# jsourati/nn-active-learning

Measured on AMD Instinct MI355X. Metric: patches/sec Fisher-scored (32^3, 2-class), higher is better.
Workload: dtype f32 (fp32 operands split into 16-bit pieces on the 16-bit MFMA, fp32 accumulate: fp16 pairs - 22-23 bits kept per operand, three products - in the conv under the head (forward + backward), in dec1's forward launch and in the other backward launches; bf16 triples - all 24 bits, exact, six products -

## Files before the change

include/alq.h:

```cpp
#ifndef ALQ_H
#define ALQ_H

#include <stddef.h>
#include <stdint.h>

#ifdef __cplusplus
extern "C" {
#endif

typedef struct alq_ctx alq_ctx;
typedef struct alq_model alq_model;

enum { ALQ_OK = 0, ALQ_EINVAL = -1, ALQ_EHIP = -2, ALQ_ENOMEM = -3, ALQ_EUNSUPPORTED = -4 };

enum { ALQ_CONV = 0, ALQ_CONVT = 1, ALQ_POOL = 2, ALQ_FC = 3 };

typedef struct {
    int32_t type;
    int32_t cout;
    int32_t k[3];
    int32_t s[3];
    int32_t relu;
    int32_t skip_src;
} alq_layer_t;
// ... 164 lines not shown
int alq_segment_min(alq_ctx *ctx, const int32_t *d_labels, const int64_t dims[3], int32_t n_labels, const int64_t *d_inds,
                    const double *d_scores, int64_t n, double *d_table);

size_t alq_cc_work_bytes(const int64_t dims[3]);
int alq_cc_label(alq_ctx *ctx, const uint8_t *d_seg, const int64_t dims[3], int connectivity, int select_zero, int32_t *d_labels);
int alq_cc_keep_largest(alq_ctx *ctx, const uint8_t *d_seg, const int64_t dims[3], int connectivity, int skip_origin, uint8_t *d_out,
                        int64_t *d_info, void *d_work);
int alq_fill_holes(alq_ctx *ctx, const uint8_t *d_seg, const int64_t dims[3], uint8_t *d_out, int64_t *d_info, void *d_work);

typedef struct alq_dcrf_params {
    float sdims_smooth[2];
    float sdims_app[2];
    float schan;
    float compat_smooth, compat_app;
    int32_t niter;
} alq_dcrf_params;
size_t alq_dcrf_work_bytes(const int64_t dims[3]);
int alq_dcrf2d(alq_ctx *ctx, const float *d_post, const float *d_img, const int64_t dims[3], const alq_dcrf_params *par,
               float *d_q1, uint8_t *d_map, void *d_work);

int alq_llfc_grads(alq_ctx *ctx, const float *d_feat, const float *d_post, const int32_t *d_labels, int n, int d, int c,
                   float *d_out);
size_t alq_llfc_hess_max_bytes(void);
int alq_llfc_hess(alq_ctx *ctx, const float *d_feat_one, const float *d_post_one, int d, int c, double *d_H);
int alq_llfc_if_path(int d, int c);
size_t alq_llfc_if_work_bytes(int n_pool, int c);
int alq_llfc_stoch_if(alq_ctx *ctx, const float *d_pool_feat, const float *d_pool_post, const int32_t *d_pool_labels, int n_pool,
                      const float *d_tr_feat, const float *d_tr_post, int n_tr, const int32_t *d_draws, int T, double scale, int d,
                      int c, int path, float *d_V, void *d_work);

int alq_aopt_tile(void);
int alq_aopt_max_workgroups(void);
size_t alq_aopt_work_bytes(int64_t n, int L);
int alq_aopt_svec(alq_ctx *ctx, const double *d_A, int64_t n, int L, double *d_V);
int alq_aopt_stats(alq_ctx *ctx, const double *d_V, const double *d_q, int64_t n, int m, const double *h_kvec,
                   const double *h_R, double mu, double obj, double *d_out, void *d_work);
int alq_aopt_direction(alq_ctx *ctx, const double *d_V, const double *d_q, int64_t n, int m, const double *h_kvec,
                       const double *h_R, const double *h_c_r, const double *h_c_1, double ratio, double mu, double obj,
                       double *d_dq, double *d_out, void *d_work);
int alq_aopt_linesearch(alq_ctx *ctx, const double *d_q, const double *d_dq, int64_t n, const double *h_alpha, int J,
                        double *d_out, void *d_work);
int alq_aopt_update(alq_ctx *ctx, double *d_q, const double *d_dq, const double *d_V, int64_t n, int m, double alpha,
                    double *d_out, void *d_work);

typedef struct {
    int32_t layer;
    int32_t pad;
    int64_t idx;
    double delta;
} alq_flip_t;
int alq_ref64_scores(alq_ctx *ctx, const alq_layer_t *layers, int n_layers, const int32_t in_dims[4],
                     const double *const *h_dW, const double *const *h_db, const float *d_x, const int64_t *d_rows, int N,
                     const alq_flip_t *d_flips, int flips_per_sample, double eps, int cand_cap,
                     double *d_logits, double *d_S, double *d_rms, alq_flip_t *d_cand, double *d_cand_key, int32_t *d_cand_count);

int alq_prof_enable(alq_ctx *ctx, int on);
int alq_prof_reset(alq_ctx *ctx);
int alq_prof_num_classes(void);
const char *alq_prof_class_name(int cls);
int alq_prof_read(alq_ctx *ctx, int cls, double *ms, int64_t *launches, double *flops);

int alq_model_debug_copy(alq_model *m, int layer_idx, int what, int N, float *d_out,
                         int64_t *elems_out);

int alq_debug_set_stamp_buffer(void *d_buf);
int alq_debug_set(int key, int value);
enum {
    ALQ_INFO_SUBNORMALS_OK = 0,
    ALQ_INFO_C3D_FWD = 1,
    ALQ_INFO_C3D_BWD = 2,
    ALQ_INFO_C3D_ONE_ACC = 3,
    ALQ_INFO_FLIP_OVERFLOW = 5,
    ALQ_INFO_F16_DERIVED = 6,
    ALQ_INFO_T3D_FWD = 7,
    ALQ_INFO_T3D_BWD = 8,
    ALQ_INFO_E3D_BWD = 9,
    ALQ_INFO_D3D_FWD = 10,
    ALQ_INFO_D3D_BWD = 11,
    ALQ_INFO_F3D_FWD = 12,
    ALQ_INFO_C3D_BWD_FORM = 13,
    ALQ_INFO_HOST_PACK_ELEMS = 14,
    ALQ_INFO_LSUM = 15,
    ALQ_INFO_DCP_FORM = 16,
    ALQ_INFO_E3D_BWD_FORM = 17
};
int alq_model_engine_info(alq_model *m, int what);

int alq_synth_patches(alq_ctx *ctx, uint64_t seed, int64_t first_id, int64_t n,
                      int64_t elems_per_patch, float *d_out);

#ifdef __cplusplus
}
#endif
#endif
```

nn-active-learning_amd/csrc/alq_internal.h:

```cpp
#pragma once
#include <hip/hip_runtime.h>

#include <cstdint>
#include <cstdio>
#include <memory>
#include <string>
#include <vector>

#include "alq.h"
#include "engine_switches.h"

namespace alq {

void set_error(const char *fmt, ...);

#define ALQ_HIP(expr)                                                                     \
    do {                                                                                  \
        hipError_t e_ = (expr);                                                           \
        if (e_ != hipSuccess) {                                                           \
            ::alq::set_error("%s:%d: %s -> %s", __FILE__, __LINE__, #expr,               \
                             hipGetErrorString(e_));                                      \
            return ALQ_EHIP;                                                              \
        }                                                                                 \
    } while (0)
// ... 142 lines not shown
int igemm_launch(alq_ctx *ctx, const IgemmPlan &plan, const View &in, const View &out,
                 const float *bias, int relu, int accumulate, int N, int prof_cls);

struct Igemm2Args {
    const float *in;
    float *out;
    const float *W;
    const float *bias;
    const float *mask;
    float *osumA, *osumB;
    int mask_cs, mask_c0, mask_from, split;
    int in_cs, in_c0, Ci, ID, IH, IW;
    int out_cs, out_c0, Co, OD, OH, OW;
    int MD, MH, MW;
    int sm, so, ooffz, ooffy, ooffx;
    int PT, TZ, TY, TX, HZ, HY, HX, rows;
    int minz, miny, minx;
    int ntaps, nchunks;
    int tilesZ, tilesY, tilesX;
    int N, relu, accumulate;
    int t0, tsz, tsy, tsx, tnx, tny;
    int dbg_repeat, dbg_flags;
    unsigned long long *dbg;
    const int *tdesc;
    const int *sdesc;
    int tpg;
    int in_bytes;
    int in_pstride, out_pstride;
    float f16_sc = 0.f, f16_inv = 0.f, f16_bias_sc = 0.f;
    const unsigned *f16_bound = nullptr;
    int f16_wexp = 0;
};

struct Igemm2Plan {
    Igemm2Args a;
    bool ok = false;
    bool wres = false;
    int NTW = 1;
    int wgs_per_cu = 1;
    size_t lds_bytes = 0;
    double flops_per_patch = 0;
    std::vector<float> h_W;
    float *d_W = nullptr;
    std::vector<int> h_tdesc, h_sdesc;
    int *d_tdesc = nullptr, *d_sdesc = nullptr;
};

struct Igemm2Fuse {
    const float *mask = nullptr;
    int mask_cs = 0, mask_c0 = 0, mask_from = 0;
    int mask_to = 1 << 30;
    float *osumA = nullptr, *osumB = nullptr;
    int split = 0;
    int store_from = 0;
    int mask_split = 0;
    long long mask_delta = 0;
    const unsigned char *mask_bits = nullptr;
    unsigned char *sign_out = nullptr;
    const unsigned *in_bits = nullptr;
    const float *in_vec = nullptr;
    float in_vec_amax = 0.f;
    const unsigned *in_vec16 = nullptr;
    unsigned *out_amax = nullptr;
    int amax_from = 0;
    const unsigned *in_amax = nullptr, *in_amax2 = nullptr;
    float in_bound = 0.f;
    const float *fc_W = nullptr;
    long long fc_F = 0;
    float *fc_part = nullptr;
    unsigned *fc_bits = nullptr;
    unsigned *flip_cnt = nullptr, *flip_list = nullptr;
    int flip_cap = 0;
    float flip_l1 = 0.f;
    bool flip_bias_nonzero = false;
};

extern unsigned long long *g_igemm2_dbg;
extern int g_dbg_knobs[ALQ_NKNOBS];
inline bool two_slot_allowed() { return !g_dbg_knobs[KNOB_NO_V3] && !g_dbg_knobs[KNOB_NO_V4]; }
extern int g_dcp_last_form;
extern int g_no_f16x2;
extern int g_no_fixed;
extern int g_no_xcd_order;
int igemm2_build_plan(const IgemmPlan &p1, Igemm2Plan *p2);
void igemm2_pack_weights(Igemm2Plan *p2, const std::vector<float> &Bmat);
int igemm2_launch(alq_ctx *ctx, const Igemm2Plan &plan, const View &in, const View &out, const float *bias,
                  int relu, int accumulate, int N, int prof_cls, const Igemm2Fuse *fuse);

struct Igemm3Plan {
    bool ok = false;
    bool wres = false;
    int NTW = 1;
    int wgs_per_cu = 1;
    size_t lds_bytes = 0;
    std::vector<unsigned short> h_W;
    void *d_W = nullptr;
    std::vector<unsigned short> h_W16;
    void *d_W16 = nullptr;
    int w16_exp = 0;
};
int igemm3_build_plan(const Igemm2Plan &p2, Igemm3Plan *p3);
void igemm3_pack_weights(const Igemm2Plan &p2, Igemm3Plan *p3, const std::vector<float> &Bmat);
void igemm3_pack_weights_f16(const Igemm2Plan &p2, Igemm3Plan *p3, const std::vector<float> &Bmat);
int igemm3_launch(alq_ctx *ctx, const Igemm2Plan &p2, const Igemm3Plan &plan, const View &in, const View &out,
                  const float *bias, int relu, int accumulate, int N, int prof_cls, const Igemm2Fuse *fuse);

struct Igemm4Args {
    const float *in;
    float *out;
    const void *W;
    const float *bias;
    const float *mask;
    float *osumA, *osumB;
    const int *tdesc;
    const int *sdesc;
    const int *pdesc;
    const int *ttab;
    const int *vdesc;
    int in_cs, in_c0, out_cs, out_c0, Co;
    int mask_cs, mask_c0, mask_from, mask_to, split;
    int N, PT, tpg, rows;
    int PX, PYX, PZ;
    int smz, smy, smx;
    int soz, soy, sox, OD, OH, OW;
    int MD, MH, MW;
    int nph, ngr, NP;
    int nslots, plane_bytes;
    int in_pstride, out_pstride, in_bytes;
    int relu, accumulate, pair, store_from;
    int cls_ok;
    int in_split_ch, in_delta, out_split, out_delta, mask_split, mask_delta;
    int tt_ints, pd_off, td_off, wbytes, abytes;
    int dbg_repeat;
    unsigned long long *dbg;
    const unsigned *src_bits;
    int bits_pstride, bits_bytes;
    const float *fc_W;
    float *fc_part;
    unsigned char *fc_bits;
    int fc_F;
    int f16_ein;
    int f16_ew;
    const unsigned *in_amax, *in_amax2;
    unsigned *out_amax;
    int amax_from;
    int wp;
    int src_presplit;
    int xcd_order;
    int zreuse;
    float flip_tau;
    int flip_cap;
    unsigned *flip_cnt;
    unsigned *flip_list;
    const unsigned char *mask_bits;
    unsigned char *sign_out;
};

struct G4Geom {
    int kind = 0;
    int cls[3] = {0, 0, 0};
    int ID = 1, IH = 1, IW = 1, Ci = 0;
    int OD = 1, OH = 1, OW = 1, Co = 0;
    int k[3] = {1, 1, 1}, s[3] = {1, 1, 1}, lo[3] = {0, 0, 0};
    bool flipped = false;
    double flops_per_patch = 0;
};
// ... 350 lines not shown
```

nn-active-learning_amd/csrc/d3d.hip:

```cpp
#include "f16_pair.h"
#include "sweep_common.h"

#include <algorithm>
#include <cmath>
#include <cstdlib>
#include <cstring>
#include <vector>

namespace alq {

struct D3Args {
    const float *inA, *inB;
    const unsigned *amaxA, *amaxB;
    const unsigned short *Whi;
    const unsigned short *Wlo;
    const float *bias;
    float *out;
    unsigned char *sg;
    float *osum;
    int e_w;
    int relu;
    int N;
};

constexpr int D3_KG = 18 * 16;
constexpr int D3_ROWB = 4 * D3_KG;
constexpr int D3_SLOT = 2 * D3_ROWB;
constexpr int D3_PLANE = 18 * D3_SLOT;
constexpr int D3_STRIP = 2 * D3_PLANE;

#ifndef D3_PIPE
#define D3_PIPE 2
#endif
#ifndef D3_START
#define D3_START 1
#endif

struct D3Row { f32x4 a, b; };

__global__ __launch_bounds__(256) __attribute__((amdgpu_waves_per_eu(1, 1))) void d3d_fwd_kernel(const D3Args a) {
    extern __shared__ __attribute__((aligned(16))) char d3lds[];
    const int lane = threadIdx.x & 63, wave = __builtin_amdgcn_readfirstlane((int)(threadIdx.x >> 6));
    char *strip = d3lds;
    for (int i = threadIdx.x; i < D3_STRIP / 16; i += 256) reinterpret_cast<i32x4 *>(strip)[i] = i32x4{0, 0, 0, 0};
    __syncthreads();
    const int n = lane & 15, kg = lane >> 4;
    f16x8 wh[27], wl[27];
#pragma unroll
    for (int c = 0; c < 27; ++c) {
        wh[c] = *reinterpret_cast<const f16x8 *>(a.Whi + ((size_t)c * 64 + lane) * 8);
        wl[c] = *reinterpret_cast<const f16x8 *>(a.Wlo + ((size_t)c * 64 + lane) * 8);
    }
#pragma unroll
    for (int c = 0; c < 27; ++c) asm volatile("" : "+a"(wh[c]), "+a"(wl[c]));
    f32x4 bias4 = *reinterpret_cast<const f32x4 *>(a.bias + 4 * kg);
    asm volatile("" : "+v"(bias4));
    const float relu_floor = a.relu ? 0.f : -__builtin_inff();

    typedef const unsigned __attribute__((address_space(4))) *cu32p;
    const cu32p amaxA_c = (cu32p)(unsigned long long)a.amaxA, amaxB_c = (cu32p)(unsigned long long)a.amaxB;
    auto patch_exp = [&](int p) __attribute__((always_inline)) {
        const unsigned fa = amaxA_c[p], fb = amaxB_c[p];
        return sw_patch_exp(fa > fb ? fa : fb);
    };

    const __amdgpu_buffer_rsrc_t ia_rsrc = sw_rsrc(a.inA, (unsigned long long)a.N * 4096 * 64);
    const __amdgpu_buffer_rsrc_t ib_rsrc = sw_rsrc(a.inB, (unsigned long long)a.N * 4096 * 64);
    const __amdgpu_buffer_rsrc_t o_rsrc = sw_rsrc(a.out, (unsigned long long)a.N * 4096 * 64);
    const __amdgpu_buffer_rsrc_t s_rsrc = sw_rsrc(a.sg, a.sg ? (unsigned long long)a.N * 4096 * 4 : 0ull);
    const __amdgpu_buffer_rsrc_t u_rsrc = sw_rsrc(a.osum, a.osum ? (unsigned long long)a.N * 4096 * 4 : 0ull);

    const int sx = lane >> 2, cq = lane & 3;
    char *const w_base = strip + (4 * wave + 1) * D3_SLOT + (cq >> 1) * D3_KG + (sx + 1) * 16 + (cq & 1) * 8;
    const unsigned ldA = (unsigned)lane * 16u;
    const char *const f_base = strip + 4 * wave * D3_SLOT + kg * D3_KG + n * 16;
    const unsigned e_out = (unsigned)n * 64u + (unsigned)kg * 16u, e_sg = (unsigned)n * 4u + (unsigned)kg;
    const unsigned e_sum = kg == 0 ? (unsigned)n * 4u : SW_OOB;

    SW_PATCH_ORDER(a.N);

    D3Row RA[4];
    auto fetch = [&](int q) __attribute__((always_inline)) {
        const unsigned row0 = ((unsigned)patch_of(q >> 4) * 16u + (unsigned)(q & 15)) * 16u + 4u * (unsigned)wave;
#pragma unroll
        for (int r = 0; r < 4; ++r) {
            RA[r].a = __builtin_bit_cast(f32x4, __builtin_amdgcn_raw_buffer_load_b128(ia_rsrc, (int)ldA, sw_s((row0 + r) * 1024u), 0));
            RA[r].b = __builtin_bit_cast(f32x4, __builtin_amdgcn_raw_buffer_load_b128(ib_rsrc, (int)ldA, sw_s((row0 + r) * 1024u), 0));
        }
    };
    auto stage_unit = [&](auto U, int img, float sc, float sc11) __attribute__((always_inline)) {
        constexpr int u = decltype(U)::value, r = u >> 1, h = u & 1;
        char *dst = w_base + img * D3_PLANE + r * D3_SLOT + h * 2 * D3_KG;
        const f32x4 g = h ? RA[r].b : RA[r].a;
        const f16x2 h01 = __builtin_convertvector(f32x2{g.x * sc, g.y * sc}, f16x2), h23 = __builtin_convertvector(f32x2{g.z * sc, g.w * sc}, f16x2);
        const f16x2 l01 = __builtin_convertvector(f32x2{__builtin_fmaf((float)h01.x, -2048.f, g.x * sc11), __builtin_fmaf((float)h01.y, -2048.f, g.y * sc11)}, f16x2);
        const f16x2 l23 = __builtin_convertvector(f32x2{__builtin_fmaf((float)h23.x, -2048.f, g.z * sc11), __builtin_fmaf((float)h23.y, -2048.f, g.w * sc11)}, f16x2);
        *reinterpret_cast<i32x2 *>(dst) = i32x2{__builtin_bit_cast(int, h01), __builtin_bit_cast(int, h23)};
        *reinterpret_cast<i32x2 *>(dst + D3_ROWB) = i32x2{__builtin_bit_cast(int, l01), __builtin_bit_cast(int, l23)};
    };

    f32x4 acc[3][4], acx[3][4];
#pragma unroll
    for (int st = 0; st < 3; ++st)
#pragma unroll
        for (int ry = 0; ry < 4; ++ry) { acc[st][ry] = f32x4{0.f, 0.f, 0.f, 0.f}; acx[st][ry] = f32x4{0.f, 0.f, 0.f, 0.f}; }
    f32x4 okeep[2];
    okeep[0] = okeep[1] = f32x4{0.f, 0.f, 0.f, 0.f};

    auto epi_row = [&](auto ST, auto RY, int p, int zo, bool tv, float inv) __attribute__((always_inline)) {
        constexpr int st = decltype(ST)::value, ry = decltype(RY)::value;
        const unsigned vrow = (unsigned)sw_s((((unsigned)p * 16u + (unsigned)(tv ? zo : 0)) * 16u + (unsigned)(4 * wave + ry)) * 16u);
        const f32x4 c = acc[st][ry], cx = acx[st][ry];
        if (!D3_START) { acc[st][ry] = f32x4{0.f, 0.f, 0.f, 0.f}; acx[st][ry] = f32x4{0.f, 0.f, 0.f, 0.f}; }
        const float v0 = __builtin_fmaxf(__builtin_fmaf(__builtin_fmaf(cx.x, 0x1p-11f, c.x), inv, bias4.x), relu_floor);
        const float v1 = __builtin_fmaxf(__builtin_fmaf(__builtin_fmaf(cx.y, 0x1p-11f, c.y), inv, bias4.y), relu_floor);
        const float v2 = __builtin_fmaxf(__builtin_fmaf(__builtin_fmaf(cx.z, 0x1p-11f, c.z), inv, bias4.z), relu_floor);
        const float v3 = __builtin_fmaxf(__builtin_fmaf(__builtin_fmaf(cx.w, 0x1p-11f, c.w), inv, bias4.w), relu_floor);
        const f32x4 o = f32x4{v0, v1, v2, v3};
        okeep[ry & 1] = o;
        __builtin_amdgcn_raw_buffer_store_b128(__builtin_bit_cast(i32x4, o), o_rsrc, (int)(tv ? e_out : SW_OOB), (int)(vrow * 64u), 0);
        ALQ_STORE_HOLD("v"(o));
        const unsigned bits = (v0 > 0.f ? 1u : 0u) | (v1 > 0.f ? 2u : 0u) | (v2 > 0.f ? 4u : 0u) | (v3 > 0.f ? 8u : 0u);
        __builtin_amdgcn_raw_buffer_store_b8((unsigned char)bits, s_rsrc, (int)(tv ? e_sg : SW_OOB), (int)(vrow * 4u), 0);
        float s_ = (v0 + v1) + (v2 + v3);
        s_ += __shfl_xor(s_, 16, 64);
        s_ += __shfl_xor(s_, 32, 64);
        __builtin_amdgcn_raw_buffer_store_b32(__builtin_bit_cast(int, s_), u_rsrc, (int)(tv ? e_sum : SW_OOB), (int)(vrow * 4u), 0);
    };

    auto step = [&](auto JJ, int i, int s) __attribute__((always_inline)) {
        constexpr int J = decltype(JJ)::value;
        constexpr int S0 = (J + 1) % 3, S1 = J, S2 = (J + 2) % 3;
        __builtin_amdgcn_sched_barrier(0);
        const int q = 16 * i + s;
        const int p = patch_of(i);
        const float inv = __builtin_ldexpf(1.f, -(patch_exp(p) + a.e_w));
        const int pn = patch_of((q + 1) >> 4);
        const int cen = patch_exp(pn);
        const bool nv = ((q + 1) >> 4) < npw;
        const float sc = nv ? __builtin_ldexpf(1.f, cen) : 0.f, sc11 = nv ? __builtin_ldexpf(1.f, cen + 11) : 0.f;
        const int img = q & 1;
        asm volatile("s_waitcnt lgkmcnt(0)\n\ts_barrier" ::: "memory");
        const char *fb = f_base + img * D3_PLANE;
        f16x8 Fh[2][3], Fl[2][3];
        auto frag = [&](auto R, f16x8 *fh, f16x8 *fl) __attribute__((always_inline)) {
            constexpr int r = decltype(R)::value;
#pragma unroll
            for (int dx = 0; dx < 3; ++dx) {
                fh[dx] = *reinterpret_cast<const f16x8 *>(fb + r * D3_SLOT + dx * 16);
                fl[dx] = *reinterpret_cast<const f16x8 *>(fb + r * D3_SLOT + dx * 16 + D3_ROWB);
            }
        };
        frag(IC<0>{}, Fh[0], Fl[0]);
        auto block = [&](auto R) __attribute__((always_inline)) {
            constexpr int r = decltype(R)::value;
            __builtin_amdgcn_sched_barrier(0);
            if constexpr (r + 1 < 6) frag(IC<r + 1>{}, Fh[(r + 1) % 2], Fl[(r + 1) % 2]);
            if constexpr (r == 0) epi_row(IC<S0>{}, IC<3>{}, p, s - 2, s >= 2, inv);
            if constexpr (r == 1) { stage_unit(IC<0>{}, img ^ 1, sc, sc11); stage_unit(IC<1>{}, img ^ 1, sc, sc11); stage_unit(IC<2>{}, img ^ 1, sc, sc11); stage_unit(IC<3>{}, img ^ 1, sc, sc11); }
            if constexpr (r == 2) { stage_unit(IC<4>{}, img ^ 1, sc, sc11); stage_unit(IC<5>{}, img ^ 1, sc, sc11); stage_unit(IC<6>{}, img ^ 1, sc, sc11); stage_unit(IC<7>{}, img ^ 1, sc, sc11); }
            if constexpr (r == 3) {
                fetch(q + 2);
                epi_row(IC<S2>{}, IC<0>{}, p, s - 1, s >= 1, inv);
            }
            if constexpr (r == 4) epi_row(IC<S2>{}, IC<1>{}, p, s - 1, s >= 1, inv);
            if constexpr (r == 5) epi_row(IC<S2>{}, IC<2>{}, p, s - 1, s >= 1, inv);
            int nm = 0;
#pragma unroll
            for (int dx = 0; dx < 3; ++dx) {
                const f16x8 xh = Fh[r % 2][dx], xl = Fl[r % 2][dx];
#pragma unroll
                for (int dy = 0; dy < 3; ++dy) {
                    const int ry = r - dy;
                    if (ry < 0 || ry > 3) continue;
#pragma unroll
                    for (int dz = 0; dz < 3; ++dz) {
                        const int st = dz == 0 ? S0 : (dz == 1 ? S1 : S2);
                        const int tap = (dz * 3 + dy) * 3 + dx;
                        const bool first = D3_START && dz == 0 && dy == 0 && dx == 0;
                        const f32x4 zero = f32x4{0.f, 0.f, 0.f, 0.f};
                        acx[st][ry] = __builtin_amdgcn_mfma_f32_16x16x32_f16(wl[tap], xh, first ? zero : acx[st][ry], 0, 0, 0);
                        acc[st][ry] = __builtin_amdgcn_mfma_f32_16x16x32_f16(wh[tap], xh, first ? zero : acc[st][ry], 0, 0, 0);
                        acx[st][ry] = __builtin_amdgcn_mfma_f32_16x16x32_f16(wh[tap], xl, acx[st][ry], 0, 0, 0);
                        nm += 3;
                    }
                }
            }
            (void)nm;
#pragma unroll
            for (int m = 0; m < 27 * ((r == 0 || r == 5) ? 1 : ((r == 1 || r == 4) ? 2 : 3)); ++m) {
                __builtin_amdgcn_sched_group_barrier(0x008, 1, 0);
                __builtin_amdgcn_sched_group_barrier(SW_FILL_MASK, D3_PIPE, 0);
            }
        };
        block(IC<0>{}); block(IC<1>{}); block(IC<2>{}); block(IC<3>{}); block(IC<4>{}); block(IC<5>{});
        __builtin_amdgcn_sched_barrier(0);
        const f32x4 k0 = okeep[0], k1 = okeep[1];
        asm volatile("" :: "v"(k0), "v"(k1));
    };

    if (npw > 0) {
        {
            fetch(0);
            const int ce = patch_exp(patch_of(0));
            const float sc = __builtin_ldexpf(1.f, ce), sc11 = __builtin_ldexpf(1.f, ce + 11);
            stage_unit(IC<0>{}, 0, sc, sc11); stage_unit(IC<1>{}, 0, sc, sc11); stage_unit(IC<2>{}, 0, sc, sc11); stage_unit(IC<3>{}, 0, sc, sc11);
            stage_unit(IC<4>{}, 0, sc, sc11); stage_unit(IC<5>{}, 0, sc, sc11); stage_unit(IC<6>{}, 0, sc, sc11); stage_unit(IC<7>{}, 0, sc, sc11);
            __builtin_amdgcn_sched_barrier(0);
            fetch(1);
        }
        for (int i = 0; i < npw; ++i) {
            for (int k = 0; k < 5; ++k) {
                step(IC<0>{}, i, 3 * k);
                step(IC<1>{}, i, 3 * k + 1);
                step(IC<2>{}, i, 3 * k + 2);
            }
            step(IC<0>{}, i, 15);
            __builtin_amdgcn_sched_barrier(0);
            const int p = patch_of(i);
            const float inv = __builtin_ldexpf(1.f, -(patch_exp(p) + a.e_w));
            epi_row(IC<2>{}, IC<3>{}, p, 14, true, inv);
            epi_row(IC<0>{}, IC<0>{}, p, 15, true, inv);
            epi_row(IC<0>{}, IC<1>{}, p, 15, true, inv);
            epi_row(IC<0>{}, IC<2>{}, p, 15, true, inv);
            epi_row(IC<0>{}, IC<3>{}, p, 15, true, inv);
#pragma unroll
            for (int ry = 0; ry < 4; ++ry) { acc[0][ry] = f32x4{0.f, 0.f, 0.f, 0.f}; acx[0][ry] = f32x4{0.f, 0.f, 0.f, 0.f}; }
            __builtin_amdgcn_sched_barrier(0);
            asm volatile("s_nop 7" :: "v"(okeep[0]), "v"(okeep[1]) : "memory");
        }
    }
}

struct D3BArgs {
    const float *dout;
    const unsigned short *Whi;
    const unsigned short *Wlo;
    float *dinA, *dinB;
    float *sumB;
    float scale, scale11, inv;
    int N;
};
constexpr int DB_KG = 18 * 16;
constexpr int DB_ROWB = 2 * DB_KG;
constexpr int DB_SLOT = 2 * DB_ROWB;
constexpr int DB_PLANE = 19 * DB_SLOT;
constexpr int DB_STRIP = 2 * DB_PLANE;

__global__ __launch_bounds__(256) __attribute__((amdgpu_waves_per_eu(1, 1))) void d3d_bwd_kernel(const D3BArgs a) {
    extern __shared__ __attribute__((aligned(16))) char d3lds[];
    const int lane = threadIdx.x & 63, wave = __builtin_amdgcn_readfirstlane((int)(threadIdx.x >> 6));
    const int cb = wave & 1, rg = wave >> 1;
    char *strip = d3lds;
    for (int i = threadIdx.x; i < DB_STRIP / 16; i += 256) reinterpret_cast<i32x4 *>(strip)[i] = i32x4{0, 0, 0, 0};
    __syncthreads();
    const int n = lane & 15, kg = lane >> 4;
    f16x8 wh[15], wl[15];
#pragma unroll
    for (int c = 0; c < 15; ++c) {
        wh[c] = *reinterpret_cast<const f16x8 *>(a.Whi + ((size_t)(cb * 15 + c) * 64 + lane) * 8);
        wl[c] = *reinterpret_cast<const f16x8 *>(a.Wlo + ((size_t)(cb * 15 + c) * 64 + lane) * 8);
    }
#pragma unroll
    for (int c = 0; c < 15; ++c) asm volatile("" : "+a"(wh[c]), "+a"(wl[c]));

    const __amdgpu_buffer_rsrc_t i_rsrc = sw_rsrc(a.dout, (unsigned long long)a.N * 4096 * 64);
    const __amdgpu_buffer_rsrc_t o_rsrc = sw_rsrc(cb ? a.dinB : a.dinA, (unsigned long long)a.N * 4096 * 64);
    const __amdgpu_buffer_rsrc_t u_rsrc = sw_rsrc(a.sumB, a.sumB ? (unsigned long long)a.N * 4096 * 4 : 0ull);

    const int sx = lane >> 2, cq = lane & 3;
    char *const w_base = strip + (4 * wave + 1) * DB_SLOT + (cq >> 1) * DB_KG + (sx + 1) * 16 + (cq & 1) * 8;
    const unsigned ldA = (unsigned)lane * 16u;
    const char *const f01 = strip + 8 * rg * DB_SLOT + (kg & 1) * DB_KG + (n + (kg >> 1)) * 16;
    const char *const f22 = strip + 8 * rg * DB_SLOT + (kg >> 1) * DB_SLOT + (kg & 1) * DB_KG + (n + 2) * 16;
    const unsigned e_out = (unsigned)n * 64u + (unsigned)kg * 16u;
    const unsigned e_sum = (kg == 0 && cb == 1) ? (unsigned)n * 4u : SW_OOB;

    SW_PATCH_ORDER(a.N);

    f32x4 RA[4];
    auto fetch = [&](int q) __attribute__((always_inline)) {
        const unsigned row0 = ((unsigned)patch_of(q >> 4) * 16u + (unsigned)(q & 15)) * 16u + 4u * (unsigned)wave;
#pragma unroll
        for (int r = 0; r < 4; ++r)
            RA[r] = __builtin_bit_cast(f32x4, __builtin_amdgcn_raw_buffer_load_b128(i_rsrc, (int)ldA, sw_s((row0 + r) * 1024u), 0));
    };
    auto stage_unit = [&](auto U, int img, float sc, float sc11) __attribute__((always_inline)) {
        constexpr int r = decltype(U)::value;
        char *dst = w_base + img * DB_PLANE + r * DB_SLOT;
        const f32x4 g = RA[r];
        const f16x2 h01 = __builtin_convertvector(f32x2{g.x * sc, g.y * sc}, f16x2), h23 = __builtin_convertvector(f32x2{g.z * sc, g.w * sc}, f16x2);
        const f16x2 l01 = __builtin_convertvector(f32x2{__builtin_fmaf((float)h01.x, -2048.f, g.x * sc11), __builtin_fmaf((float)h01.y, -2048.f, g.y * sc11)}, f16x2);
        const f16x2 l23 = __builtin_convertvector(f32x2{__builtin_fmaf((float)h23.x, -2048.f, g.z * sc11), __builtin_fmaf((float)h23.y, -2048.f, g.w * sc11)}, f16x2);
        *reinterpret_cast<i32x2 *>(dst) = i32x2{__builtin_bit_cast(int, h01), __builtin_bit_cast(int, h23)};
        *reinterpret_cast<i32x2 *>(dst + DB_ROWB) = i32x2{__builtin_bit_cast(int, l01), __builtin_bit_cast(int, l23)};
    };

    f32x4 acc[3][8], acx[3][8];
#pragma unroll
    for (int st = 0; st < 3; ++st)
#pragma unroll
        for (int ry = 0; ry < 8; ++ry) { acc[st][ry] = f32x4{0.f, 0.f, 0.f, 0.f}; acx[st][ry] = f32x4{0.f, 0.f, 0.f, 0.f}; }
    f32x4 okeep[2];
    okeep[0] = okeep[1] = f32x4{0.f, 0.f, 0.f, 0.f};

    auto epi_row = [&](auto ST, auto RY, int p, int zo, bool tv) __attribute__((always_inline)) {
        constexpr int st = decltype(ST)::value, ry = decltype(RY)::value;
        const unsigned vrow = (unsigned)sw_s((((unsigned)p * 16u + (unsigned)(tv ? zo : 0)) * 16u + (unsigned)(8 * rg + ry)) * 16u);
        const f32x4 c = acc[st][ry], cx = acx[st][ry];
        if (!D3_START) { acc[st][ry] = f32x4{0.f, 0.f, 0.f, 0.f}; acx[st][ry] = f32x4{0.f, 0.f, 0.f, 0.f}; }
        const float v0 = __builtin_fmaf(cx.x, 0x1p-11f, c.x) * a.inv, v1 = __builtin_fmaf(cx.y, 0x1p-11f, c.y) * a.inv;
        const float v2 = __builtin_fmaf(cx.z, 0x1p-11f, c.z) * a.inv, v3 = __builtin_fmaf(cx.w, 0x1p-11f, c.w) * a.inv;
        const f32x4 o = f32x4{v0, v1, v2, v3};
        okeep[ry & 1] = o;
        __builtin_amdgcn_raw_buffer_store_b128(__builtin_bit_cast(i32x4, o), o_rsrc, (int)(tv ? e_out : SW_OOB), (int)(vrow * 64u), 0);
        ALQ_STORE_HOLD("v"(o));
        float s_ = (v0 + v1) + (v2 + v3);
        s_ += __shfl_xor(s_, 16, 64);
        s_ += __shfl_xor(s_, 32, 64);
        __builtin_amdgcn_raw_buffer_store_b32(__builtin_bit_cast(int, s_), u_rsrc, (int)(tv ? e_sum : SW_OOB), (int)(vrow * 4u), 0);
    };

    auto step = [&](auto JJ, int i, int s) __attribute__((always_inline)) {
        constexpr int J = decltype(JJ)::value;
        constexpr int S0 = (J + 1) % 3, S1 = J, S2 = (J + 2) % 3;
        __builtin_amdgcn_sched_barrier(0);
        const int q = 16 * i + s;
        const int p = patch_of(i);
        const bool nv = ((q + 1) >> 4) < npw;
        const float sc = nv ? a.scale : 0.f, sc11 = nv ? a.scale11 : 0.f;
        const int img = q & 1;
        asm volatile("s_waitcnt lgkmcnt(0)\n\ts_barrier" ::: "memory");
        const char *fa = f01 + img * DB_PLANE, *fb = f22 + img * DB_PLANE;
        f16x8 Fh[2][2], Fl[2][2];
        auto frag = [&](auto R, f16x8 *fh, f16x8 *fl) __attribute__((always_inline)) {
            constexpr int r = decltype(R)::value;
            fh[0] = *reinterpret_cast<const f16x8 *>(fa + r * DB_SLOT);
            fl[0] = *reinterpret_cast<const f16x8 *>(fa + r * DB_SLOT + DB_ROWB);
            fh[1] = *reinterpret_cast<const f16x8 *>(fb + r * DB_SLOT);
            fl[1] = *reinterpret_cast<const f16x8 *>(fb + r * DB_SLOT + DB_ROWB);
        };
        frag(IC<0>{}, Fh[0], Fl[0]);
        auto mm = [&](auto ST, auto RY, auto KS, const f16x8 &xh, const f16x8 &xl) __attribute__((always_inline)) {
            constexpr int st = decltype(ST)::value, ry = decltype(RY)::value, ks = decltype(KS)::value;
            constexpr bool first = D3_START && ks == 0;
            const f32x4 zero = f32x4{0.f, 0.f, 0.f, 0.f};
            acx[st][ry] = __builtin_amdgcn_mfma_f32_16x16x32_f16(wl[ks], xh, first ? zero : acx[st][ry], 0, 0, 0);
            acc[st][ry] = __builtin_amdgcn_mfma_f32_16x16x32_f16(wh[ks], xh, first ? zero : acc[st][ry], 0, 0, 0);
            acx[st][ry] = __builtin_amdgcn_mfma_f32_16x16x32_f16(wh[ks], xl, acx[st][ry], 0, 0, 0);
        };
        auto block = [&](auto R) __attribute__((always_inline)) {
            constexpr int r = decltype(R)::value;
            __builtin_amdgcn_sched_barrier(0);
            if constexpr (r + 1 < 10) frag(IC<r + 1>{}, Fh[(r + 1) % 2], Fl[(r + 1) % 2]);
            if constexpr (r == 0) epi_row(IC<S0>{}, IC<7>{}, p, s - 2, s >= 2);
            if constexpr (r == 2) { stage_unit(IC<0>{}, img ^ 1, sc, sc11); stage_unit(IC<1>{}, img ^ 1, sc, sc11); }
            if constexpr (r == 3) { stage_unit(IC<2>{}, img ^ 1, sc, sc11); stage_unit(IC<3>{}, img ^ 1, sc, sc11); }
            if constexpr (r == 4) fetch(q + 2);
            if constexpr (r >= 3) epi_row(IC<S2>{}, IC<r - 3>{}, p, s - 1, s >= 1);
            const f16x8 ph = Fh[r % 2][0], pl = Fl[r % 2][0], qh = Fh[r % 2][1], ql = Fl[r % 2][1];
#define D3B_ALLDZ(RYV, PIV, XH, XL)                                                   \
            mm(IC<S0>{}, IC<RYV>{}, IC<0 * 5 + PIV>{}, XH, XL);                 \
            mm(IC<S1>{}, IC<RYV>{}, IC<1 * 5 + PIV>{}, XH, XL);                 \
            mm(IC<S2>{}, IC<RYV>{}, IC<2 * 5 + PIV>{}, XH, XL);
            if constexpr (r <= 7) { D3B_ALLDZ((r <= 7 ? r : 0), 0, ph, pl) }
            if constexpr (r >= 1 && r <= 8) { D3B_ALLDZ((r >= 1 && r <= 8 ? r - 1 : 0), 1, ph, pl) }
            if constexpr (r >= 2) { D3B_ALLDZ((r >= 2 ? r - 2 : 0), 2, ph, pl) }
            if constexpr (r <= 7) { D3B_ALLDZ((r <= 7 ? r : 0), 3, qh, ql) }
            if constexpr (r >= 2) { D3B_ALLDZ((r >= 2 ? r - 2 : 0), 4, qh, ql) }
#undef D3B_ALLDZ
#pragma unroll
            for (int m = 0; m < 9 * ((r == 0 || r == 9) ? 2 : ((r == 1 || r == 8) ? 3 : 5)); ++m) {
                __builtin_amdgcn_sched_group_barrier(0x008, 1, 0);
                __builtin_amdgcn_sched_group_barrier(SW_FILL_MASK, D3_PIPE, 0);
            }
        };
        block(IC<0>{}); block(IC<1>{}); block(IC<2>{}); block(IC<3>{}); block(IC<4>{});
        block(IC<5>{}); block(IC<6>{}); block(IC<7>{}); block(IC<8>{}); block(IC<9>{});
        __builtin_amdgcn_sched_barrier(0);
        const f32x4 k0 = okeep[0], k1 = okeep[1];
        asm volatile("" :: "v"(k0), "v"(k1));
    };

    if (npw > 0) {
        {
            fetch(0);
            stage_unit(IC<0>{}, 0, a.scale, a.scale11); stage_unit(IC<1>{}, 0, a.scale, a.scale11);
            stage_unit(IC<2>{}, 0, a.scale, a.scale11); stage_unit(IC<3>{}, 0, a.scale, a.scale11);
            __builtin_amdgcn_sched_barrier(0);
            fetch(1);
        }
        for (int i = 0; i < npw; ++i) {
            for (int k = 0; k < 5; ++k) {
                step(IC<0>{}, i, 3 * k);
                step(IC<1>{}, i, 3 * k + 1);
                step(IC<2>{}, i, 3 * k + 2);
            }
            step(IC<0>{}, i, 15);
            __builtin_amdgcn_sched_barrier(0);
            const int p = patch_of(i);
            epi_row(IC<2>{}, IC<7>{}, p, 14, true);
            epi_row(IC<0>{}, IC<0>{}, p, 15, true); epi_row(IC<0>{}, IC<1>{}, p, 15, true);
            epi_row(IC<0>{}, IC<2>{}, p, 15, true); epi_row(IC<0>{}, IC<3>{}, p, 15, true);
            epi_row(IC<0>{}, IC<4>{}, p, 15, true); epi_row(IC<0>{}, IC<5>{}, p, 15, true);
            epi_row(IC<0>{}, IC<6>{}, p, 15, true); epi_row(IC<0>{}, IC<7>{}, p, 15, true);
#pragma unroll
            for (int ry = 0; ry < 8; ++ry) { acc[0][ry] = f32x4{0.f, 0.f, 0.f, 0.f}; acx[0][ry] = f32x4{0.f, 0.f, 0.f, 0.f}; }
            __builtin_amdgcn_sched_barrier(0);
            asm volatile("s_nop 7" :: "v"(okeep[0]), "v"(okeep[1]) : "memory");
        }
    }
}

int d3d_build(const View &in, const View &out, const int k[3], const int lo[3], const int s[3], D3dPlan *plan) {
    plan->ok = false;
    if (getenv("ALQ_NO_D3D")) return ALQ_OK;
    if (!is_conv3_same(k, lo, s)) return ALQ_OK;
    if (!(in.D == 16 && in.H == 16 && in.W == 16 && out.D == 16 && out.H == 16 && out.W == 16 && in.C == 32 && in.split == 16 && in.cs == 16 && in.c0 == 0 &&
          out.C == 16 && out.cs == 16 && out.c0 == 0 && out.split == 0)) return ALQ_OK;
    plan->flops_per_patch = 2.0 * 27 * 32 * 16 * 4096.0;
    plan->ok = true;
    return ALQ_OK;
}

void d3d_pack(D3dPlan *plan, const float *W) {
    plan->w_exp = f16_pair_exp(W, (size_t)27 * 32 * 16);
    plan->h_Whi.assign((size_t)27 * 64 * 8, 0);
    plan->h_Wlo.assign((size_t)27 * 64 * 8, 0);
    for (int tap = 0; tap < 27; ++tap)
        for (int lane = 0; lane < 64; ++lane) {
            const int co = lane & 15, kg = lane >> 4;
            for (int c = 0; c < 8; ++c) {
                const float w = W[((size_t)tap * 32 + 8 * kg + c) * 16 + co];
                const size_t o = ((size_t)tap * 64 + lane) * 8 + c;
                f16_pair_split(w, plan->w_exp, 11, &plan->h_Whi[o], &plan->h_Wlo[o]);
            }
        }
}

void d3d_bwd_pack(D3dPlan *plan, const float *W) {
    plan->h_Bhi.assign((size_t)2 * 15 * 64 * 8, 0);
    plan->h_Blo.assign((size_t)2 * 15 * 64 * 8, 0);
    for (int cb = 0; cb < 2; ++cb)
        for (int dz = 0; dz < 3; ++dz)
            for (int pi = 0; pi < 5; ++pi)
                for (int lane = 0; lane < 64; ++lane) {
                    const int r = lane & 15, kg = lane >> 4, h = kg >> 1;
                    int dy, dx;
                    bool any = true;
                    if (pi < 3) { dy = pi; dx = h; } else if (pi == 3) { dy = h; dx = 2; } else { dy = 2; dx = 2; any = h == 0; }
                    for (int c = 0; c < 8; ++c) {
                        const int co = 8 * (kg & 1) + c, ci = 16 * cb + r;
                        const int tap = ((2 - dz) * 3 + (2 - dy)) * 3 + (2 - dx);
                        const float w = any ? W[((size_t)tap * 32 + ci) * 16 + co] : 0.f;
                        const size_t o = ((size_t)((cb * 3 + dz) * 5 + pi) * 64 + lane) * 8 + c;
                        f16_pair_split(w, plan->w_exp, 11, &plan->h_Bhi[o], &plan->h_Blo[o]);
                    }
                }
}

int d3d_bwd_launch(alq_ctx *ctx, const D3dPlan &plan, int N, const float *dout, float in_bound, float *dinA, float *dinB, float *sumB) {
    ALQ_REQUIRE(plan.ok && plan.d_Bhi && plan.d_Blo, ALQ_EINVAL, "d3d: backward weights not set");
    ALQ_REQUIRE(dout && dinA && dinB && in_bound > 0.f, ALQ_EINVAL, "d3d: missing argument");
    SWEEP_REQUIRE_PATCHES(N, "d3d");
    if (N <= 0) return ALQ_OK;
    const int e_in = f16_pair_exp(&in_bound, 1);
    D3BArgs a;
    a.dout = dout; a.Whi = reinterpret_cast<const unsigned short *>(plan.d_Bhi); a.Wlo = reinterpret_cast<const unsigned short *>(plan.d_Blo);
    a.dinA = dinA; a.dinB = dinB; a.sumB = sumB;
    a.scale = std::ldexp(1.f, e_in); a.scale11 = std::ldexp(1.f, e_in + 11); a.inv = std::ldexp(1.f, -(e_in + plan.w_exp)); a.N = N;
    ProfScope ps(ctx, PROF_IGEMM_F16, plan.flops_per_patch * N);
    return sweep_launch(ctx, d3d_bwd_kernel, sweep_grid(ctx, N, 1), 256, DB_STRIP, a);
}

int d3d_fwd_launch(alq_ctx *ctx, const D3dPlan &plan, int N, const float *inA, const float *inB, const unsigned *amaxA, const unsigned *amaxB,
                   const float *bias, int relu, float *out, unsigned char *sg, float *osum) {
    ALQ_REQUIRE(plan.ok && plan.d_Whi && plan.d_Wlo, ALQ_EINVAL, "d3d: weights not set");
    ALQ_REQUIRE(inA && inB && amaxA && amaxB && bias && out, ALQ_EINVAL, "d3d: missing argument");
    SWEEP_REQUIRE_PATCHES(N, "d3d");
    if (N <= 0) return ALQ_OK;
    D3Args a;
    a.inA = inA; a.inB = inB; a.amaxA = amaxA; a.amaxB = amaxB;
    a.Whi = reinterpret_cast<const unsigned short *>(plan.d_Whi); a.Wlo = reinterpret_cast<const unsigned short *>(plan.d_Wlo);
    a.bias = bias; a.out = out; a.sg = sg; a.osum = osum; a.e_w = plan.w_exp; a.relu = relu; a.N = N;
    ProfScope ps(ctx, PROF_IGEMM_F16, plan.flops_per_patch * N);
    return sweep_launch(ctx, d3d_fwd_kernel, sweep_grid(ctx, N, 1), 256, D3_STRIP, a);
}

}
```

nn-active-learning_amd/csrc/e3d.hip:

```cpp
#include "f16_pair.h"
#include "sweep_common.h"

#include <algorithm>
#include <cmath>
#include <cstdlib>
#include <cstring>
#include <vector>

namespace alq {

struct E3Args {
    const float *skip;
    const float *dpool;
    const unsigned char *am2;
    const unsigned char *sg2;
    const unsigned short *Whi;
    const unsigned short *Wlo;
    const unsigned char *am1;
    const unsigned char *sg1;
    float *dsum2;
    float *dsum1;
    float scale, inv;
    int N;
};
// ... 131 lines not shown
                const E3RowB &rb = RB[r];
                const int i = 3 * wave + r, pi = i >> 1;
                const int zz = z0 - 1 + pi, yy = 2 * t - 1 + (i & 1);
                const bool rv = live && zz >= 0 && zz < 16 && yy >= 0 && yy < 16;
                const float scr = rv ? a.scale : 0.f;
                const unsigned x4 = rb.am ^ (lanepar4 ^ ((unsigned)((((zz & 1) * 2 + (yy & 1)) * 2)) * 0x01010101u));
                float g0 = ra.sk.x + (((x4 & 0xffu) == 0u) ? rb.dp.x : 0.f);
                float g1 = ra.sk.y + (((x4 & 0xff00u) == 0u) ? rb.dp.y : 0.f);
                float g2 = ra.sk.z + (((x4 & 0xff0000u) == 0u) ? rb.dp.z : 0.f);
                float g3 = ra.sk.w + (((x4 & 0xff000000u) == 0u) ? rb.dp.w : 0.f);
                unsigned k0 = (unsigned)__builtin_amdgcn_sbfe((int)ra.sg, 0, 1), k1 = (unsigned)__builtin_amdgcn_sbfe((int)ra.sg, 1, 1);
                unsigned k2 = (unsigned)__builtin_amdgcn_sbfe((int)ra.sg, 2, 1), k3 = (unsigned)__builtin_amdgcn_sbfe((int)ra.sg, 3, 1);
                asm("" : "+v"(k0), "+v"(k1), "+v"(k2), "+v"(k3));
                g0 = __builtin_bit_cast(float, __builtin_bit_cast(unsigned, g0) & k0); g1 = __builtin_bit_cast(float, __builtin_bit_cast(unsigned, g1) & k1);
                g2 = __builtin_bit_cast(float, __builtin_bit_cast(unsigned, g2) & k2); g3 = __builtin_bit_cast(float, __builtin_bit_cast(unsigned, g3) & k3);
                {
                    float s_ = (g0 + g1) + (g2 + g3);
                    s_ += __builtin_bit_cast(float, __builtin_amdgcn_mov_dpp(__builtin_bit_cast(int, s_), 0xB1, 0xf, 0xf, true));
                    s_ += __builtin_bit_cast(float, __builtin_amdgcn_mov_dpp(__builtin_bit_cast(int, s_), 0x4E, 0xf, 0xf, true));
                    const bool own = rv && pi >= 1 && pi <= 4;
                    const unsigned row = ((unsigned)p * 16u + (unsigned)clampi(zz)) * 16u + (unsigned)clampi(yy);
                    __builtin_amdgcn_raw_buffer_store_b32(__builtin_bit_cast(int, s_), d2_rsrc, (int)(own ? st2 : SW_OOB), sw_s(row * 64u), 0);
                }
                const float x0 = g0 * scr, x1 = g1 * scr, x2 = g2 * scr, x3 = g3 * scr;
                const f16x2 h01 = __builtin_convertvector(f32x2{x0, x1}, f16x2), h23 = __builtin_convertvector(f32x2{x2, x3}, f16x2);
                const float sc11 = scr * 2048.f;
                const f16x2 l01 = __builtin_convertvector(f32x2{__builtin_fmaf((float)h01.x, -2048.f, g0 * sc11), __builtin_fmaf((float)h01.y, -2048.f, g1 * sc11)}, f16x2);
                const f16x2 l23 = __builtin_convertvector(f32x2{__builtin_fmaf((float)h23.x, -2048.f, g2 * sc11), __builtin_fmaf((float)h23.y, -2048.f, g3 * sc11)}, f16x2);
                char *dst = strip + (live ? pi * E3_PLANE + ((yy + 6) % 6) * E3_SLOT : E3_STRIP) + w_off;
                *reinterpret_cast<i32x2 *>(dst) = i32x2{__builtin_bit_cast(int, h01), __builtin_bit_cast(int, h23)};
                *reinterpret_cast<i32x2 *>(dst + E3_ROWB) = i32x2{__builtin_bit_cast(int, l01), __builtin_bit_cast(int, l23)};
            }
            fetchB(S + 1, RB);
            fetchA(S + 2, RA[b]);
            asm volatile("s_waitcnt lgkmcnt(0)\n\ts_barrier" ::: "memory");
            f32x4 c = f32x4{0.f, 0.f, 0.f, 0.f}, cl = f32x4{0.f, 0.f, 0.f, 0.f};
#pragma unroll
            for (int dy = 0; dy < 3; ++dy) {
                const int s0 = ((2 * t + 3 + dy) % 6) * E3_SLOT, s1 = ((2 * t + 4 + dy) % 6) * E3_SLOT;
                const int rowo = (ry ? s1 : s0) + f_off;
#pragma unroll
                for (int dz = 0; dz < 3; ++dz) {
                    const char *src = strip + dz * E3_PLANE + rowo;
#pragma unroll
                    for (int s = 0; s < 2; ++s) {
                        const f16x8 xh = *reinterpret_cast<const f16x8 *>(src + s * 64);
                        const f16x8 xl = *reinterpret_cast<const f16x8 *>(src + s * 64 + E3_ROWB);
                        const f16x8 wlo = *reinterpret_cast<const f16x8 *>(wl + ((dz * 3 + dy) * 2 + s) * 1024);
                        const f16x8 whi = wh[dz * 3 + dy][s];
                        cl = __builtin_amdgcn_mfma_f32_16x16x32_f16(wlo, xh, cl, 0, 0, 0);
                        cl = __builtin_amdgcn_mfma_f32_16x16x32_f16(whi, xl, cl, 0, 0, 0);
                        c = __builtin_amdgcn_mfma_f32_16x16x32_f16(whi, xh, c, 0, 0, 0);
                    }
                }
            }
            const float r0 = __builtin_fmaf(cl.x, 0x1p-11f, c.x) * a.inv, r1 = __builtin_fmaf(cl.y, 0x1p-11f, c.y) * a.inv;
            const float r2 = __builtin_fmaf(cl.z, 0x1p-11f, c.z) * a.inv, r3 = __builtin_fmaf(cl.w, 0x1p-11f, c.w) * a.inv;
            unsigned m0 = (unsigned)__builtin_amdgcn_sbfe((int)sg1b, 0, 1), m1 = (unsigned)__builtin_amdgcn_sbfe((int)sg1b, 1, 1);
            unsigned m2 = (unsigned)__builtin_amdgcn_sbfe((int)sg1b, 2, 1), m3 = (unsigned)__builtin_amdgcn_sbfe((int)sg1b, 3, 1);
            asm("" : "+v"(m0), "+v"(m1), "+v"(m2), "+v"(m3));
            const float v0 = __builtin_bit_cast(float, __builtin_bit_cast(unsigned, r0) & m0), v1 = __builtin_bit_cast(float, __builtin_bit_cast(unsigned, r1) & m1);
            const float v2 = __builtin_bit_cast(float, __builtin_bit_cast(unsigned, r2) & m2), v3 = __builtin_bit_cast(float, __builtin_bit_cast(unsigned, r3) & m3);
            float sw[8];
#pragma unroll
            for (int w = 0; w < 8; ++w)
                sw[w] = ((((am1w & 255u) == (unsigned)w) ? v0 : 0.f) + ((((am1w >> 8) & 255u) == (unsigned)w) ? v1 : 0.f)) +
                        (((((am1w >> 16) & 255u) == (unsigned)w) ? v2 : 0.f) + (((am1w >> 24) == (unsigned)w) ? v3 : 0.f));
            f32x4 mine;
            {
                const float g0 = __shfl_xor(hi ? sw[0] : sw[4], 16, 64), g1 = __shfl_xor(hi ? sw[1] : sw[5], 16, 64);
                const float g2 = __shfl_xor(hi ? sw[2] : sw[6], 16, 64), g3 = __shfl_xor(hi ? sw[3] : sw[7], 16, 64);
                mine = f32x4{(hi ? sw[4] : sw[0]) + g0, (hi ? sw[5] : sw[1]) + g1, (hi ? sw[6] : sw[2]) + g2, (hi ? sw[7] : sw[3]) + g3};
            }
            const f32x2 n0 = f32x2{old0.x + mine.x, old0.y + mine.y}, n1 = f32x2{old1.x + mine.z, old1.y + mine.w};
            __builtin_amdgcn_raw_buffer_store_b64(__builtin_bit_cast(i32x2, n0), d1_rsrc, (int)(tv ? e_d1 : SW_OOB), (int)d1row, 0);
            __builtin_amdgcn_raw_buffer_store_b64(__builtin_bit_cast(i32x2, n1), d1_rsrc, (int)(tv ? e_d1 + 128u : SW_OOB), (int)d1row, 0);
        }
    }
}

constexpr int E3Z_IMG = 18 * E3_SLOT;
constexpr int E3Z_ZERO = 4 * E3Z_IMG;
constexpr int E3Z_SINK = 5 * E3Z_IMG;
constexpr int E3Z_LDS = E3_WLO + E3Z_SINK + E3_SLOT;
static_assert(E3Z_IMG % 16 == 0 && E3Z_LDS <= 160 * 1024, "e3d plane sweep: LDS layout");

struct E3ZRowB { f32x4 dp; unsigned am; };

__global__ __launch_bounds__(512) void e3d_bwdz_kernel(const E3Args a) {
    extern __shared__ __attribute__((aligned(16))) char e3lds[];
    {
        const i32x4 *src = reinterpret_cast<const i32x4 *>(a.Wlo);
        i32x4 *dst = reinterpret_cast<i32x4 *>(e3lds);
        for (int i = threadIdx.x; i < E3_WLO / 16; i += 512) dst[i] = src[i];
        for (int i = threadIdx.x; i < (E3Z_LDS - E3_WLO) / 16; i += 512) dst[E3_WLO / 16 + i] = i32x4{0, 0, 0, 0};
    }
    __syncthreads();
    const int lane = threadIdx.x & 63, wave = __builtin_amdgcn_readfirstlane((int)(threadIdx.x >> 6));
    char *strip = e3lds + E3_WLO;
    const int n = lane & 15, kg = lane >> 4, ry = n >> 3, j = n & 7;
    f16x8 wh[9][2];
#pragma unroll
    for (int c = 0; c < 9; ++c)
#pragma unroll
        for (int s = 0; s < 2; ++s) wh[c][s] = *reinterpret_cast<const f16x8 *>(a.Whi + ((size_t)(c * 2 + s) * 64 + lane) * 8);
#pragma unroll
    for (int c = 0; c < 9; ++c)
#pragma unroll
        for (int s = 0; s < 2; ++s) asm volatile("" : "+v"(wh[c][s]));
    const char *wl = e3lds + lane * 16;

    const __amdgpu_buffer_rsrc_t sk_rsrc = sw_rsrc(a.skip, (unsigned long long)a.N * 4096 * 64);
    const __amdgpu_buffer_rsrc_t dp_rsrc = sw_rsrc(a.dpool, (unsigned long long)a.N * 512 * 64);
    const __amdgpu_buffer_rsrc_t a2_rsrc = sw_rsrc(a.am2, (unsigned long long)a.N * 512 * 16);
    const __amdgpu_buffer_rsrc_t s2_rsrc = sw_rsrc(a.sg2, (unsigned long long)a.N * 4096 * 4);
    const __amdgpu_buffer_rsrc_t a1_rsrc = sw_rsrc(a.am1, (unsigned long long)a.N * 4096 * 8);
    const __amdgpu_buffer_rsrc_t s1_rsrc = sw_rsrc(a.sg1, (unsigned long long)a.N * 4096 * 2);
    const __amdgpu_buffer_rsrc_t d2_rsrc = sw_rsrc(a.dsum2, (unsigned long long)a.N * 4096 * 4);
    const __amdgpu_buffer_rsrc_t d1_rsrc = sw_rsrc(a.dsum1, (unsigned long long)a.N * 32768 * 4);

    const int sx = lane >> 2, cq = lane & 3;
    const int w_off = (sx + 1) * 32 + cq * 8 + (2 * wave + 1) * E3_SLOT;
    const unsigned ldA = (unsigned)lane * 16u, ldS = (unsigned)lane;
    const unsigned ldP = (unsigned)(sx >> 1) * 64u + (unsigned)cq * 16u, ldM = (unsigned)(sx >> 1) * 16u + (unsigned)cq * 4u;
    const unsigned lanepar4 = (unsigned)(sx & 1) * 0x01010101u;
    const unsigned st2 = cq == 0 ? (unsigned)sx * 4u : SW_OOB;
    const int f_off = (2 * j + (kg >> 1)) * 32 + (kg & 1) * 16 + (2 * wave + ry) * E3_SLOT;
    const bool hi = (kg & 1) != 0;
    const unsigned e_am = (unsigned)(ry * 16 + 2 * j + (kg >> 1)) * 8u + (unsigned)(kg & 1) * 4u;
    const unsigned e_sg = (unsigned)(ry * 16 + 2 * j + (kg >> 1)) * 2u + (unsigned)(kg & 1);
    const unsigned e_d1 = (unsigned)(hi ? 32 * 128 : 0) + (unsigned)(2 * ry) * 128u + (unsigned)(2 * (2 * j + (kg >> 1))) * 4u;

    const int G = (int)gridDim.x, b0 = (int)blockIdx.x;
    const int nunits = a.N > b0 ? (a.N - b0 + G - 1) / G : 0;
    const int T = nunits * 16;

    auto plane = [&](int m, int *p, int *z) __attribute__((always_inline)) {
        const int mc = m < 0 ? 0 : (m < T ? m : T - 1);
        *p = b0 + (mc >> 4) * G;
        *z = mc & 15;
    };
    auto fetchA = [&](int m, E3RowA *R) __attribute__((always_inline)) {
        int p, z;
        plane(m, &p, &z);
        const unsigned row = ((unsigned)p * 16u + (unsigned)z) * 16u + (unsigned)(2 * wave);
        const int so_sk = sw_s(row * 1024u), so_sg = sw_s(row * 64u);
#pragma unroll
        for (int r = 0; r < 2; ++r) {
            R[r].sk = __builtin_bit_cast(f32x4, __builtin_amdgcn_raw_buffer_load_b128(sk_rsrc, (int)(ldA + (unsigned)r * 1024u), so_sk, 0));
            R[r].sg = (unsigned)(unsigned char)__builtin_amdgcn_raw_buffer_load_b8(s2_rsrc, (int)(ldS + (unsigned)r * 64u), so_sg, 0);
        }
    };
    auto fetchB = [&](int m, E3ZRowB *R) __attribute__((always_inline)) {
        int p, z;
        plane(m, &p, &z);
        const unsigned prow = ((unsigned)p * 8u + (unsigned)(z >> 1)) * 8u + (unsigned)wave;
        R->dp = __builtin_bit_cast(f32x4, __builtin_amdgcn_raw_buffer_load_b128(dp_rsrc, (int)ldP, sw_s(prow * 512u), 0));
        R->am = (unsigned)__builtin_amdgcn_raw_buffer_load_b32(a2_rsrc, (int)ldM, sw_s(prow * 128u), 0);
    };

    E3RowA RA[2][2];
    E3ZRowB RB;
    RB.dp = f32x4{0.f, 0.f, 0.f, 0.f}; RB.am = 0u;
#pragma unroll
    for (int i = 0; i < 2; ++i)
#pragma unroll
        for (int b = 0; b < 2; ++b) { RA[b][i].sk = f32x4{0.f, 0.f, 0.f, 0.f}; RA[b][i].sg = 0u; }

    if (T > 0)
    for (int s0 = -2; s0 < T + 2; s0 += 2) {
#pragma unroll
        for (int b = 0; b < 2; ++b) {
            __builtin_amdgcn_sched_barrier(0);
            const int s = s0 + b;
            const bool live = s0 >= 0 && s < T;
            const bool tv = s >= 2;
            int p, z, po, zo;
            plane(s, &p, &z);
            plane(s - 2, &po, &zo);
            asm volatile("s_waitcnt lgkmcnt(0)\n\ts_barrier" ::: "memory");
            const unsigned trow = ((unsigned)po * 16u + (unsigned)zo) * 16u + (unsigned)(2 * wave);
            const unsigned am1w = (unsigned)__builtin_amdgcn_raw_buffer_load_b32(a1_rsrc, (int)e_am, sw_s(trow * 128u), 0);
            const unsigned sg1b = (unsigned)(unsigned char)__builtin_amdgcn_raw_buffer_load_b8(s1_rsrc, (int)e_sg, sw_s(trow * 32u), 0);
            const unsigned d1row = (unsigned)sw_s((((unsigned)po * 32u + (unsigned)(2 * zo)) * 32u + (unsigned)(4 * wave)) * 128u);
            const f32x2 old0 = __builtin_bit_cast(f32x2, __builtin_amdgcn_raw_buffer_load_b64(d1_rsrc, (int)e_d1, (int)d1row, 0));
            const f32x2 old1 = __builtin_bit_cast(f32x2, __builtin_amdgcn_raw_buffer_load_b64(d1_rsrc, (int)(e_d1 + 128u), (int)d1row, 0));
            const unsigned srow = ((unsigned)p * 16u + (unsigned)z) * 16u + (unsigned)(2 * wave);
            const int so_d2 = sw_s(srow * 64u);
            char *img = strip + sw_s(live ? (unsigned)(s & 3) * (unsigned)E3Z_IMG : (unsigned)(E3Z_SINK - (2 * wave + 1) * E3_SLOT)) + w_off;
            const float scr = a.scale;
#pragma unroll
            for (int r = 0; r < 2; ++r) {
                const E3RowA &ra = RA[b][r];
                const unsigned x4 = RB.am ^ (lanepar4 ^ ((unsigned)((((z & 1) * 2 + r) * 2)) * 0x01010101u));
                float g0 = ra.sk.x + (((x4 & 0xffu) == 0u) ? RB.dp.x : 0.f);
                float g1 = ra.sk.y + (((x4 & 0xff00u) == 0u) ? RB.dp.y : 0.f);
                float g2 = ra.sk.z + (((x4 & 0xff0000u) == 0u) ? RB.dp.z : 0.f);
                float g3 = ra.sk.w + (((x4 & 0xff000000u) == 0u) ? RB.dp.w : 0.f);
                unsigned k0 = (unsigned)__builtin_amdgcn_sbfe((int)ra.sg, 0, 1), k1 = (unsigned)__builtin_amdgcn_sbfe((int)ra.sg, 1, 1);
                unsigned k2 = (unsigned)__builtin_amdgcn_sbfe((int)ra.sg, 2, 1), k3 = (unsigned)__builtin_amdgcn_sbfe((int)ra.sg, 3, 1);
                asm("" : "+v"(k0), "+v"(k1), "+v"(k2), "+v"(k3));
                g0 = __builtin_bit_cast(float, __builtin_bit_cast(unsigned, g0) & k0); g1 = __builtin_bit_cast(float, __builtin_bit_cast(unsigned, g1) & k1);
                g2 = __builtin_bit_cast(float, __builtin_bit_cast(unsigned, g2) & k2); g3 = __builtin_bit_cast(float, __builtin_bit_cast(unsigned, g3) & k3);
                {
                    float s_ = (g0 + g1) + (g2 + g3);
                    s_ += __builtin_bit_cast(float, __builtin_amdgcn_mov_dpp(__builtin_bit_cast(int, s_), 0xB1, 0xf, 0xf, true));
                    s_ += __builtin_bit_cast(float, __builtin_amdgcn_mov_dpp(__builtin_bit_cast(int, s_), 0x4E, 0xf, 0xf, true));
                    __builtin_amdgcn_raw_buffer_store_b32(__builtin_bit_cast(int, s_), d2_rsrc, (int)(live ? st2 + (unsigned)r * 64u : SW_OOB), so_d2, 0);
                }
                const float x0 = g0 * scr, x1 = g1 * scr, x2 = g2 * scr, x3 = g3 * scr;
                const f16x2 h01 = __builtin_convertvector(f32x2{x0, x1}, f16x2), h23 = __builtin_convertvector(f32x2{x2, x3}, f16x2);
                const float sc11 = scr * 2048.f;
                const f16x2 l01 = __builtin_convertvector(f32x2{__builtin_fmaf((float)h01.x, -2048.f, g0 * sc11), __builtin_fmaf((float)h01.y, -2048.f, g1 * sc11)}, f16x2);
                const f16x2 l23 = __builtin_convertvector(f32x2{__builtin_fmaf((float)h23.x, -2048.f, g2 * sc11), __builtin_fmaf((float)h23.y, -2048.f, g3 * sc11)}, f16x2);
                char *dst = img + (live ? r * E3_SLOT : 0);
                *reinterpret_cast<i32x2 *>(dst) = i32x2{__builtin_bit_cast(int, h01), __builtin_bit_cast(int, h23)};
                *reinterpret_cast<i32x2 *>(dst + E3_ROWB) = i32x2{__builtin_bit_cast(int, l01), __builtin_bit_cast(int, l23)};
            }
            fetchB(s + 1, &RB);
            fetchA(s + 2, RA[b]);
            const int io[3] = {sw_s(zo == 0 ? (unsigned)E3Z_ZERO : (unsigned)((s + 1) & 3) * (unsigned)E3Z_IMG), sw_s((unsigned)((s + 2) & 3) * (unsigned)E3Z_IMG),
                               sw_s(zo == 15 ? (unsigned)E3Z_ZERO : (unsigned)((s + 3) & 3) * (unsigned)E3Z_IMG)};
            f32x4 c = f32x4{0.f, 0.f, 0.f, 0.f}, cl = f32x4{0.f, 0.f, 0.f, 0.f};
#pragma unroll
            for (int dy = 0; dy < 3; ++dy) {
#pragma unroll
                for (int dz = 0; dz < 3; ++dz) {
                    const char *src = strip + io[dz] + f_off + dy * E3_SLOT;
#pragma unroll
                    for (int s2 = 0; s2 < 2; ++s2) {
                        const f16x8 xh = *reinterpret_cast<const f16x8 *>(src + s2 * 64);
                        const f16x8 xl = *reinterpret_cast<const f16x8 *>(src + s2 * 64 + E3_ROWB);
                        const f16x8 wlo = *reinterpret_cast<const f16x8 *>(wl + ((dz * 3 + dy) * 2 + s2) * 1024);
                        const f16x8 whi = wh[dz * 3 + dy][s2];
                        cl = __builtin_amdgcn_mfma_f32_16x16x32_f16(wlo, xh, cl, 0, 0, 0);
                        cl = __builtin_amdgcn_mfma_f32_16x16x32_f16(whi, xl, cl, 0, 0, 0);
                        c = __builtin_amdgcn_mfma_f32_16x16x32_f16(whi, xh, c, 0, 0, 0);
                    }
                }
            }
            const float r0 = __builtin_fmaf(cl.x, 0x1p-11f, c.x) * a.inv, r1 = __builtin_fmaf(cl.y, 0x1p-11f, c.y) * a.inv;
            const float r2 = __builtin_fmaf(cl.z, 0x1p-11f, c.z) * a.inv, r3 = __builtin_fmaf(cl.w, 0x1p-11f, c.w) * a.inv;
            unsigned m0 = (unsigned)__builtin_amdgcn_sbfe((int)sg1b, 0, 1), m1 = (unsigned)__builtin_amdgcn_sbfe((int)sg1b, 1, 1);
            unsigned m2 = (unsigned)__builtin_amdgcn_sbfe((int)sg1b, 2, 1), m3 = (unsigned)__builtin_amdgcn_sbfe((int)sg1b, 3, 1);
            asm("" : "+v"(m0), "+v"(m1), "+v"(m2), "+v"(m3));
            const float v0 = __builtin_bit_cast(float, __builtin_bit_cast(unsigned, r0) & m0), v1 = __builtin_bit_cast(float, __builtin_bit_cast(unsigned, r1) & m1);
            const float v2 = __builtin_bit_cast(float, __builtin_bit_cast(unsigned, r2) & m2), v3 = __builtin_bit_cast(float, __builtin_bit_cast(unsigned, r3) & m3);
            float sw[8];
#pragma unroll
            for (int w = 0; w < 8; ++w)
                sw[w] = ((((am1w & 255u) == (unsigned)w) ? v0 : 0.f) + ((((am1w >> 8) & 255u) == (unsigned)w) ? v1 : 0.f)) +
                        (((((am1w >> 16) & 255u) == (unsigned)w) ? v2 : 0.f) + (((am1w >> 24) == (unsigned)w) ? v3 : 0.f));
            f32x4 mine;
            {
                const float g0 = __shfl_xor(hi ? sw[0] : sw[4], 16, 64), g1 = __shfl_xor(hi ? sw[1] : sw[5], 16, 64);
                const float g2 = __shfl_xor(hi ? sw[2] : sw[6], 16, 64), g3 = __shfl_xor(hi ? sw[3] : sw[7], 16, 64);
                mine = f32x4{(hi ? sw[4] : sw[0]) + g0, (hi ? sw[5] : sw[1]) + g1, (hi ? sw[6] : sw[2]) + g2, (hi ? sw[7] : sw[3]) + g3};
            }
            const f32x2 n0 = f32x2{old0.x + mine.x, old0.y + mine.y}, n1 = f32x2{old1.x + mine.z, old1.y + mine.w};
            __builtin_amdgcn_raw_buffer_store_b64(__builtin_bit_cast(i32x2, n0), d1_rsrc, (int)(tv ? e_d1 : SW_OOB), (int)d1row, 0);
            __builtin_amdgcn_raw_buffer_store_b64(__builtin_bit_cast(i32x2, n1), d1_rsrc, (int)(tv ? e_d1 + 128u : SW_OOB), (int)d1row, 0);
        }
    }
}

int e3d_build(const View &in, const View &out, const int k[3], const int lo[3], const int s[3], E3dPlan *plan) {
    plan->ok = false;
    if (getenv("ALQ_NO_E3D")) return ALQ_OK;
    if (!is_conv3_same(k, lo, s)) return ALQ_OK;
    if (!(in.D == 16 && in.H == 16 && in.W == 16 && out.D == 16 && out.H == 16 && out.W == 16 && in.C == 8 && out.C == 16 && in.split == 0 && out.split == 0)) return ALQ_OK;
    plan->flops_per_patch = 2.0 * 27 * 8 * 16 * 4096.0;
    plan->ok = true;
    return ALQ_OK;
}

void e3d_pack(E3dPlan *plan, const float *W) {
    plan->w_exp = f16_pair_exp(W, (size_t)27 * 8 * 16);
    plan->h_Whi.assign((size_t)9 * 2 * 64 * 8, 0);
    plan->h_Wlo.assign((size_t)9 * 2 * 64 * 8, 0);
    for (int dz = 0; dz < 3; ++dz)
        for (int dy = 0; dy < 3; ++dy)
            for (int s = 0; s < 2; ++s)
                for (int lane = 0; lane < 64; ++lane) {
                    const int r = lane & 15, kg = lane >> 4, px = r >> 3, ci = r & 7, q = 2 * s + (kg >> 1);
                    const int tz = 2 - dz, ty = 2 - dy, tx = 2 - q + px;
                    for (int c = 0; c < 8; ++c) {
                        const int co = 8 * (kg & 1) + c;
                        const float w = (tx >= 0 && tx <= 2) ? W[((size_t)((tz * 3 + ty) * 3 + tx) * 8 + ci) * 16 + co] : 0.f;
                        const size_t o = ((size_t)((dz * 3 + dy) * 2 + s) * 64 + lane) * 8 + c;
                        f16_pair_split(w, plan->w_exp, 11, &plan->h_Whi[o], &plan->h_Wlo[o]);
                    }
                }
}

int e3d_bwd_launch(alq_ctx *ctx, const E3dPlan &plan, int N, const float *skip, const float *dpool, const unsigned char *am2, const unsigned char *sg2,
                   const unsigned char *am1, const unsigned char *sg1, float *dsum2, float *dsum1, float in_bound, bool rows) {
    ALQ_REQUIRE(plan.ok && plan.d_Whi && plan.d_Wlo, ALQ_EINVAL, "e3d: weights not set");
    ALQ_REQUIRE(skip && dpool && am2 && sg2 && am1 && sg1 && dsum2 && dsum1 && in_bound > 0.f, ALQ_EINVAL, "e3d: missing argument");
    SWEEP_REQUIRE_PATCHES(N, "e3d");
    if (N <= 0) return ALQ_OK;
    const int e_in = f16_pair_exp(&in_bound, 1);
    E3Args a;
    a.skip = skip; a.dpool = dpool; a.am2 = am2; a.sg2 = sg2; a.Whi = reinterpret_cast<const unsigned short *>(plan.d_Whi);
    a.Wlo = reinterpret_cast<const unsigned short *>(plan.d_Wlo); a.am1 = am1; a.sg1 = sg1; a.dsum2 = dsum2; a.dsum1 = dsum1;
    a.scale = std::ldexp(1.f, e_in); a.inv = std::ldexp(1.f, -(e_in + plan.w_exp)); a.N = N;
    ProfScope ps(ctx, PROF_IGEMM_F16, plan.flops_per_patch * N);
    if (!rows) {
        unsigned g = sweep_grid(ctx, N, 1);
        if (g_dbg_knobs[KNOB_E3D_GRID_CAP] > 0) g = std::min<unsigned>(g, (unsigned)g_dbg_knobs[KNOB_E3D_GRID_CAP]);
        return sweep_launch(ctx, e3d_bwdz_kernel, g, 512, E3Z_LDS, a);
    }
    return sweep_launch(ctx, e3d_bwd_kernel, sweep_grid(ctx, (long long)N * 4, 2), 256, E3_WLO + E3_STRIP + E3_SINK, a);
}

}
```

nn-active-learning_amd/csrc/engine_switches.h:

```cpp
#ifndef ALQ_ENGINE_SWITCHES_H
#define ALQ_ENGINE_SWITCHES_H
#include <cstddef>
#include <cstdlib>

namespace alq {

enum Knob {
    KNOB_REPEAT = 0,
    KNOB_FLAGS = 1,
    KNOB_NO_BWD_FUSE = 2,
    KNOB_NO_FWD_FUSE = 3,
    KNOB_NO_V3 = 4,
    KNOB_NO_V4 = 5,
    KNOB_NO_POOL_FIRST = 6,
    KNOB_NO_CONV_POOL = 7,
    KNOB_DCP_NARROW = 8,
    KNOB_E3D_GRID_CAP = 9,
    ALQ_NKNOBS = 10
};

struct EngineSwitches {
    int knobs[ALQ_NKNOBS] = {0, 0, 0, 0, 0, 0, 0, 0, 0, 0};
    int disable_v2 = 0;
    int disable_v3 = 0;
    int disable_v4 = 0;
    int no_fcgemm = 0;
    int no_split = 0;
    int no_wide2d_rule = 0;
    int no_v3_f16 = 0;
    int no_v3_f16_fwd = 0;
    int no_co_split = 0;
    int no_co_split_f16 = 0;
    int no_class_tiles = 0;
    int no_fc_bits = 0;
    int no_fc_fuse = 0;
    int no_fc_f16 = 0;
    int no_fc_f16_fwd = 0;
    int f16_derived_mask = 0;
    int has_f16_derived_mask = 0;
    int no_f16x2 = 0;
    int no_xcd_order = 0;
    int no_fixed = 0;
    int no_bound16 = 0;
    int no_flipfix = 0;
    int no_presplit = 0;
    int no_signs = 0;
    int no_signs0 = 0;
    int f16_fwd_mask = -1;
    int no_f16_derived = 0;
    int no_light_kernels = 0;
    int no_c3d = 0;
    int c3_bwd_rows = 7;
    int no_e3d = 0;
    int e3d_rows = 0;
    int no_d3d = 0;
    int no_d3b = 0;
    int no_f3d = 0;
    int no_t3d = 0;
};

enum SwitchRule {
    SW_PRESENT,
    SW_FIRST_IS_1,
    SW_ATOI_EQ,
    SW_INT,
    SW_ROWS
};

struct SwitchRow {
    const char *env;
    size_t member;
    SwitchRule rule;
    int arg;
};

#define ALQ_SW(env, member, rule, arg) {env, offsetof(EngineSwitches, member), rule, arg}
inline const SwitchRow kSwitchTable[] = {
    ALQ_SW("ALQ_DEBUG_REPEAT", knobs[KNOB_REPEAT], SW_INT, 0),
    ALQ_SW("ALQ_DEBUG_FLAGS", knobs[KNOB_FLAGS], SW_INT, 0),
    ALQ_SW("ALQ_NO_BWD_FUSE", knobs[KNOB_NO_BWD_FUSE], SW_INT, 0),
    ALQ_SW("ALQ_NO_FWD_FUSE", knobs[KNOB_NO_FWD_FUSE], SW_INT, 0),
    ALQ_SW("ALQ_NO_V3", knobs[KNOB_NO_V3], SW_INT, 0),
    ALQ_SW("ALQ_NO_V4", knobs[KNOB_NO_V4], SW_INT, 0),
    ALQ_SW("ALQ_NO_POOL_FIRST", knobs[KNOB_NO_POOL_FIRST], SW_INT, 0),
    ALQ_SW("ALQ_NO_CONV_POOL", knobs[KNOB_NO_CONV_POOL], SW_INT, 0),
    ALQ_SW("ALQ_DCP_NARROW", knobs[KNOB_DCP_NARROW], SW_INT, 0),
    ALQ_SW("ALQ_E3D_GRID_CAP", knobs[KNOB_E3D_GRID_CAP], SW_INT, 0),
    ALQ_SW("ALQ_DISABLE_V2", disable_v2, SW_FIRST_IS_1, 0),
    ALQ_SW("ALQ_DISABLE_V3", disable_v3, SW_FIRST_IS_1, 0),
    ALQ_SW("ALQ_DISABLE_V4", disable_v4, SW_PRESENT, 0),
    ALQ_SW("ALQ_NO_FCGEMM", no_fcgemm, SW_PRESENT, 0),
    ALQ_SW("ALQ_NO_SPLIT", no_split, SW_PRESENT, 0),
    ALQ_SW("ALQ_NO_WIDE2D_RULE", no_wide2d_rule, SW_PRESENT, 0),
    ALQ_SW("ALQ_NO_V3_F16", no_v3_f16, SW_PRESENT, 0),
    ALQ_SW("ALQ_NO_V3_F16_FWD", no_v3_f16_fwd, SW_PRESENT, 0),
    ALQ_SW("ALQ_NO_CO_SPLIT", no_co_split, SW_PRESENT, 0),
    ALQ_SW("ALQ_NO_CO_SPLIT_F16", no_co_split_f16, SW_PRESENT, 0),
    ALQ_SW("ALQ_NO_CLASS_TILES", no_class_tiles, SW_PRESENT, 0),
    ALQ_SW("ALQ_NO_FC_BITS", no_fc_bits, SW_PRESENT, 0),
    ALQ_SW("ALQ_NO_FC_FUSE", no_fc_fuse, SW_PRESENT, 0),
    ALQ_SW("ALQ_NO_FC_F16", no_fc_f16, SW_PRESENT, 0),
    ALQ_SW("ALQ_NO_FC_F16_FWD", no_fc_f16_fwd, SW_PRESENT, 0),
    ALQ_SW("ALQ_F16_DERIVED_MASK", f16_derived_mask, SW_INT, 0),
    ALQ_SW("ALQ_F16_DERIVED_MASK", has_f16_derived_mask, SW_PRESENT, 0),
    ALQ_SW("ALQ_NO_F16X2", no_f16x2, SW_PRESENT, 0),
    ALQ_SW("ALQ_NO_XCD_ORDER", no_xcd_order, SW_PRESENT, 0),
    ALQ_SW("ALQ_NO_FIXED", no_fixed, SW_PRESENT, 0),
    ALQ_SW("ALQ_NO_BOUND16", no_bound16, SW_PRESENT, 0),
    ALQ_SW("ALQ_NO_FLIPFIX", no_flipfix, SW_PRESENT, 0),
    ALQ_SW("ALQ_NO_PRESPLIT", no_presplit, SW_PRESENT, 0),
    ALQ_SW("ALQ_NO_SIGNS", no_signs, SW_PRESENT, 0),
    ALQ_SW("ALQ_NO_SIGNS0", no_signs0, SW_PRESENT, 0),
    ALQ_SW("ALQ_F16_FWD_MASK", f16_fwd_mask, SW_INT, 0),
    ALQ_SW("ALQ_F16_DERIVED", no_f16_derived, SW_ATOI_EQ, 0),
    ALQ_SW("ALQ_NO_F16_DERIVED", no_f16_derived, SW_ATOI_EQ, 1),
    ALQ_SW("ALQ_NO_LIGHT_KERNELS", no_light_kernels, SW_PRESENT, 0),
    ALQ_SW("ALQ_NO_C3D", no_c3d, SW_PRESENT, 0),
    ALQ_SW("ALQ_C3D_BWD_ROWS", c3_bwd_rows, SW_ROWS, 0),
    ALQ_SW("ALQ_NO_E3D", no_e3d, SW_PRESENT, 0),
    ALQ_SW("ALQ_E3D_ROWS", e3d_rows, SW_ATOI_EQ, 1),
    ALQ_SW("ALQ_NO_D3D", no_d3d, SW_PRESENT, 0),
    ALQ_SW("ALQ_NO_D3D_BWD", no_d3b, SW_PRESENT, 0),
    ALQ_SW("ALQ_NO_F3D", no_f3d, SW_PRESENT, 0),
    ALQ_SW("ALQ_NO_T3D", no_t3d, SW_PRESENT, 0),
};
#undef ALQ_SW
inline const int kNumSwitchRows = (int)(sizeof(kSwitchTable) / sizeof(kSwitchTable[0]));

inline int &switch_member(EngineSwitches &sw, const SwitchRow &row) {
    return *reinterpret_cast<int *>(reinterpret_cast<char *>(&sw) + row.member);
}

inline EngineSwitches read_engine_switches() {
    EngineSwitches sw;
    for (const SwitchRow &row : kSwitchTable) {
        const char *v = std::getenv(row.env);
        int &dst = switch_member(sw, row);
        switch (row.rule) {
            case SW_PRESENT:    if (v) dst = 1; break;
            case SW_FIRST_IS_1: if (v && v[0] == '1') dst = 1; break;
            case SW_ATOI_EQ:    if (v && std::atoi(v) == row.arg) dst = 1; break;
            case SW_INT:        if (v) dst = std::atoi(v); break;
            case SW_ROWS:       dst = (v && std::atoi(v) == 4) ? 4 : ((v && std::atoi(v) == 8) ? 8 : 7); break;
        }
    }
    return sw;
}

}
#endif
```

nn-active-learning_amd/csrc/igemm2.hip:

```cpp
#include "alq_internal.h"

#include <algorithm>
#include <cmath>
#include <cstring>

namespace alq {

typedef float f32x4 __attribute__((ext_vector_type(4)));
typedef float f32x2 __attribute__((ext_vector_type(2)));

#ifdef ALQ_STAMPS
#define STAMP(var) asm volatile("s_memtime %0\n\ts_waitcnt lgkmcnt(0)" : "=s"(var)::"memory")
#define PHASE_END(idx)                         \
    do {                                       \
        unsigned long long t_now_;             \
        STAMP(t_now_);                         \
        ph[idx] += t_now_ - t_last;            \
        t_last = t_now_;                       \
    } while (0)
#else
#define PHASE_END(idx) do {} while (0)
#endif

constexpr int I2_CBP = 12;
// ... 400 lines not shown
    a.split = 1 << 30;
    {
        const int dimsI[3] = {a.ID, a.IH, a.IW}, dimsM[3] = {a.MD, a.MH, a.MW};
        const int T[3] = {a.TZ, a.TY, a.TX}, tiles[3] = {a.tilesZ, a.tilesY, a.tilesX};
        const int mins[3] = {a.minz, a.miny, a.minx}, H[3] = {a.HZ, a.HY, a.HX};
        auto cls_of = [&](int d, int t) { return (t == 0 ? 1 : 0) | (t == tiles[d] - 1 ? 2 : 0); };
        auto valid1 = [&](int d, int t, int h) {
            const int c = t * T[d] * a.sm + mins[d] + h;
            return c >= 0 && c < dimsI[d];
        };
        for (int d = 0; d < 3; ++d)
            for (int t = 1; t + 1 < tiles[d]; ++t)
                for (int h = 0; h < H[d]; ++h)
                    if (!valid1(d, t, h)) return ALQ_OK;
        a.tpg = a.tilesZ * a.tilesY * a.tilesX;
        a.in_pstride = a.PT * a.ID * a.IH * a.IW;
        a.out_pstride = a.PT * a.OD * a.OH * a.OW;
        p2->h_tdesc.assign((size_t)a.tpg * 8, 0);
        for (int tz = 0; tz < a.tilesZ; ++tz)
            for (int ty = 0; ty < a.tilesY; ++ty)
                for (int tx = 0; tx < a.tilesX; ++tx) {
                    int *td = &p2->h_tdesc[(((size_t)tz * a.tilesY + ty) * a.tilesX + tx) * 8];
                    const int mz0 = tz * a.TZ, my0 = ty * a.TY, mx0 = tx * a.TX;
                    const int z0 = mz0 * a.sm + a.minz, y0 = my0 * a.sm + a.miny, x0 = mx0 * a.sm + a.minx;
                    td[0] = (z0 * a.IH + y0) * a.IW + x0;
                    td[1] = ((mz0 * a.so + a.ooffz) * a.OH + my0 * a.so + a.ooffy) * a.OW + mx0 * a.so + a.ooffx;
                    const int cls = cls_of(0, tz) | (cls_of(1, ty) << 2) | (cls_of(2, tx) << 4);
                    const bool full = a.rows == 256 && mz0 + a.TZ <= a.MD && my0 + a.TY <= a.MH && mx0 + a.TX <= a.MW;
                    td[2] = cls | (full ? 256 : 0);
                    td[3] = mz0; td[4] = my0; td[5] = mx0;
                }
        (void)dimsM;
        auto rep = [&](int d, int c) { return (c & 1) ? 0 : ((c & 2) ? tiles[d] - 1 : (tiles[d] > 2 ? 1 : 0)); };
        p2->h_sdesc.assign((size_t)nhv * 4, 0);
        for (int pt = 0; pt < a.PT; ++pt)
            for (int hz = 0; hz < a.HZ; ++hz)
                for (int hy = 0; hy < a.HY; ++hy)
                    for (int hx = 0; hx < a.HX; ++hx) {
                        const int hv = ((pt * a.HZ + hz) * a.HY + hy) * a.HX + hx;
                        int *sd = &p2->h_sdesc[(size_t)hv * 4];
                        sd[0] = ((pt * a.ID + hz) * a.IH + hy) * a.IW + hx;
                        unsigned long long m = 0;
                        for (int c = 0; c < 64; ++c) {
                            const int cz = c & 3, cy = (c >> 2) & 3, cx = (c >> 4) & 3;
                            if (valid1(0, rep(0, cz), hz) && valid1(1, rep(1, cy), hy) && valid1(2, rep(2, cx), hx))
                                m |= 1ull << c;
                        }
                        sd[1] = (int)(unsigned)(m & 0xffffffffull);
                        sd[2] = (int)(unsigned)(m >> 32);
                        sd[3] = (pt << 24) | (hz << 16) | (hy << 8) | hx;
                    }
    }
    p2->NTW = p1.NTW;
    p2->wres = wres;
    p2->lds_bytes = lds;
    int max_wgs = 2;
    if (const char *e = getenv("ALQ_MAX_WGS")) max_wgs = atoi(e);
    p2->wgs_per_cu = std::max<int>(1, std::min<int>(max_wgs, (int)((160 * 1024) / (lds + 512))));
    p2->flops_per_patch = p1.flops_per_patch;
    p2->ok = true;
    return ALQ_OK;
}

void igemm2_pack_weights(Igemm2Plan *p2, const std::vector<float> &Bmat) {
    const Igemm2Args &a = p2->a;
    const int NTW = p2->NTW, Ci = a.Ci, Co = a.Co;
    p2->h_W.assign((size_t)a.nchunks * a.ntaps * NTW * 128, 0.f);
    for (int ch = 0; ch < a.nchunks; ++ch)
        for (int tp = 0; tp < a.ntaps; ++tp)
            for (int nt = 0; nt < NTW; ++nt)
                for (int lane = 0; lane < 64; ++lane)
                    for (int s = 0; s < 2; ++s) {
                        const int c = ch * 8 + 2 * (lane >> 4) + s;
                        const int co = nt * 16 + (lane & 15);
                        if (co < Co)
                            p2->h_W[((((size_t)ch * a.ntaps + tp) * NTW + nt) * 64 + lane) * 2 + s] =
                                Bmat[((size_t)tp * Ci + c) * Co + co];
                    }
}

unsigned long long *g_igemm2_dbg = nullptr;
int g_no_f16x2 = 0;
int g_no_xcd_order = 0;
int g_no_fixed = 0;
int g_dbg_knobs[ALQ_NKNOBS] = {0, 0, 0, 0, 0, 0, 0, 0, 0, 0};

template <int NTW, bool WRES, int GEO, bool SUMS>
static int launch2_s(alq_ctx *ctx, const Igemm2Plan &plan, const Igemm2Args &a, unsigned grid) {
    auto kfn = igemm2_kernel<NTW, WRES, GEO, SUMS>;
    if (plan.lds_bytes > 64 * 1024)
        ALQ_HIP(hipFuncSetAttribute(reinterpret_cast<const void *>(kfn), hipFuncAttributeMaxDynamicSharedMemorySize,
                                    (int)plan.lds_bytes));
    hipLaunchKernelGGL(kfn, dim3(grid), dim3(256), plan.lds_bytes, ctx->stream, a);
    ALQ_HIP(hipGetLastError());
    return ALQ_OK;
}

template <int NTW, bool WRES, int GEO>
static int launch2_t(alq_ctx *ctx, const Igemm2Plan &plan, const Igemm2Args &a, unsigned grid) {
    return (a.osumA || a.osumB) ? launch2_s<NTW, WRES, GEO, true>(ctx, plan, a, grid)
                                : launch2_s<NTW, WRES, GEO, false>(ctx, plan, a, grid);
}

int igemm2_launch(alq_ctx *ctx, const Igemm2Plan &plan, const View &in, const View &out, const float *bias, int relu,
                  int accumulate, int N, int prof_cls, const Igemm2Fuse *fuse) {
    Igemm2Args a = plan.a;
    ALQ_REQUIRE(in.C == a.Ci && in.D == a.ID && in.H == a.IH && in.W == a.IW, ALQ_EINVAL,
                "igemm2: input view does not match plan");
    ALQ_REQUIRE(out.C == a.Co && out.D == a.OD && out.H == a.OH && out.W == a.OW, ALQ_EINVAL,
                "igemm2: output view does not match plan");
    ALQ_REQUIRE(plan.d_W != nullptr, ALQ_EINVAL, "igemm2: weights not set");
    ALQ_REQUIRE((long long)N * in.vox() * in.cs < (1LL << 29) && (long long)N * out.vox() * out.cs < (1LL << 29),
                ALQ_EUNSUPPORTED, "igemm2: tensor exceeds the 32-bit byte-offset range (lower the batch)");
    ALQ_REQUIRE(in.cs % 4 == 0 && in.c0 % 4 == 0 && out.cs % 4 == 0 && out.c0 % 4 == 0, ALQ_EUNSUPPORTED,
                "igemm2: channel slice not 16-byte aligned");
    if (fuse) ALQ_REQUIRE(fuse->split % 4 == 0 && fuse->mask_cs % 4 == 0 && fuse->mask_c0 % 4 == 0 && fuse->mask_from % 4 == 0, ALQ_EUNSUPPORTED,
                          "igemm2: fused epilogue needs 4-channel aligned slices");
    a.in = in.p; a.in_cs = in.cs; a.in_c0 = in.c0;
    a.out = out.p; a.out_cs = out.cs; a.out_c0 = out.c0;
    a.W = plan.d_W; a.bias = bias; a.relu = relu; a.accumulate = accumulate; a.N = N;
    a.in_bytes = (int)((long long)N * in.vox() * in.cs * 4);
    a.dbg = nullptr;
    if (g_igemm2_dbg) {
        static int want = -2;
        if (want == -2) { const char *e = getenv("ALQ_STAMP_ONLY"); want = e ? atoi(e) : -1; }
        static int ordinal = 0;
        static unsigned long long *last = nullptr;
        if (last != g_igemm2_dbg) { last = g_igemm2_dbg; ordinal = 0; }
        if (want < 0 || ordinal == want) a.dbg = g_igemm2_dbg;
        ++ordinal;
    }
    a.dbg_repeat = g_dbg_knobs[KNOB_REPEAT];
    a.dbg_flags = g_dbg_knobs[KNOB_FLAGS];
    if (fuse) {
        a.mask = fuse->mask; a.mask_cs = fuse->mask_cs; a.mask_c0 = fuse->mask_c0; a.mask_from = fuse->mask_from;
        a.osumA = fuse->osumA; a.osumB = fuse->osumB;
        a.split = fuse->split > 0 ? fuse->split : (1 << 30);
    }
    const int pgroups = (N + a.PT - 1) / a.PT;
    const long long total = (long long)pgroups * a.tilesZ * a.tilesY * a.tilesX;
    const unsigned grid = (unsigned)std::min<long long>(total, 256LL * plan.wgs_per_cu);
    ProfScope ps(ctx, prof_cls, plan.flops_per_patch * N);
    int geo = 0;
    if (a.ntaps == 27 && a.tnx == 3 && a.tny == 3 && a.HY == 6 && a.HX == 18) {
        const int SX = I2_CBP, SY = 18 * I2_CBP, SZ = 6 * 18 * I2_CBP;
        if (a.t0 == 0 && a.tsx == SX && a.tsy == SY && a.tsz == SZ) geo = 1;
        if (a.t0 == 2 * (SX + SY + SZ) && a.tsx == -SX && a.tsy == -SY && a.tsz == -SZ) geo = 2;
    }
#define ALQ_L2(NT)                                                                                       \
    case NT:                                                                                             \
        if (geo == 1) return plan.wres ? launch2_t<NT, true, 1>(ctx, plan, a, grid) : launch2_t<NT, false, 1>(ctx, plan, a, grid); \
        if (geo == 2) return plan.wres ? launch2_t<NT, true, 2>(ctx, plan, a, grid) : launch2_t<NT, false, 2>(ctx, plan, a, grid); \
        return plan.wres ? launch2_t<NT, true, 0>(ctx, plan, a, grid) : launch2_t<NT, false, 0>(ctx, plan, a, grid)
    switch (plan.NTW) { ALQ_L2(1); ALQ_L2(2); ALQ_L2(3); }
#undef ALQ_L2
    set_error("igemm2: NTW=%d unsupported", plan.NTW);
    return ALQ_EUNSUPPORTED;
}

}
```

nn-active-learning_amd/csrc/model.hip:

```cpp
#include <algorithm>
#include <cmath>
#include <cstring>
#include <string>

#include "model_types.h"

namespace alq {

static void same_pads(int in, int k, int s, int *out, int *lo) {
    *out = (in + s - 1) / s;
    int total = (*out - 1) * s + k - in;
    if (total < 0) total = 0;
    *lo = total / 2;
}

}

using namespace alq;

static int g_knob_override[ALQ_NKNOBS] = {-1, -1, -1, -1, -1, -1, -1, -1, -1, -1};

static void apply_knobs(const alq_model *m) {
    for (int k = 0; k < ALQ_NKNOBS; ++k) g_dbg_knobs[k] = g_knob_override[k] >= 0 ? g_knob_override[k] : m->sw.knobs[k];
    g_no_f16x2 = m->sw.no_f16x2;
    g_no_xcd_order = m->sw.no_xcd_order;
    g_no_fixed = m->sw.no_fixed;
}

static int gemm_build(const EngineSwitches &sw, const ConvDesc &d, int max_batch, Gemm *g, const G4Geom *g4 = nullptr) {
    ALQ_TRY(igemm_build_plan(d, max_batch, &g->p1));
    if (g4 && !sw.disable_v4) {
        G4Geom gg = *g4;
        gg.flops_per_patch = g->p1.flops_per_patch;
        ALQ_TRY(igemm4_build_plan(gg, max_batch, &g->p4));
    }
    ALQ_TRY(igemm2_build_plan(g->p1, &g->p2));
    ALQ_TRY(direct_build_plan(g->p1, &g->pd));
    if (sw.disable_v2) { g->p2.ok = false; g->pd.ok = false; }
    ALQ_TRY(igemm3_build_plan(g->p2, &g->p3));
    if (d.ID == 1 && d.IH == 1 && d.IW == 1 && d.tz.size() == 1 && d.sm == 1 && d.so == 1 && !sw.no_fcgemm)
        ALQ_TRY(fcgemm_build_plan(d.Ci, d.Co, &g->pfc));
    if (sw.disable_v3) g->p3.ok = false;
    return ALQ_OK;
}

int prepare_call(alq_model *m, bool fisher) {
    m->last.call_fisher = fisher;
    apply_knobs(m);
    if (!two_slot_allowed()) ALQ_TRY(refresh_fallback_forms(m));
    return ALQ_OK;
}

enum GemmRoute { ROUTE_DIRECT, ROUTE_FCGEMM, ROUTE_IGEMM4, ROUTE_IGEMM3, ROUTE_IGEMM2, ROUTE_IGEMM };
static GemmRoute gemm_route(const Gemm &g, const View &in, const View &out, int accumulate, const Igemm2Fuse *fuse) {
    if (g.pd.ok && !accumulate && !(fuse && (fuse->mask || fuse->osumB || fuse->split))) return ROUTE_DIRECT;
    if (g.pfc.ok && !accumulate && !fuse && two_slot_allowed()) return ROUTE_FCGEMM;
    const bool split_view = in.split != 0 || out.split != 0;
    if (g.p4.ok && (two_slot_allowed() || split_view)) return ROUTE_IGEMM4;
    if (g.p3.ok && !g_dbg_knobs[KNOB_NO_V3]) return ROUTE_IGEMM3;
    return g.p2.ok ? ROUTE_IGEMM2 : ROUTE_IGEMM;
}

int gemm_launch(alq_ctx *ctx, const Gemm &g, const View &in, const View &out, const float *bias, int relu,
                int accumulate, int N, int cls, const Igemm2Fuse *fuse, bool *fused, float fc_in_bound) {
    const GemmRoute route = gemm_route(g, in, out, accumulate, fuse);
    ALQ_REQUIRE(route <= ROUTE_FCGEMM || g.p4.ok || (in.split == 0 && out.split == 0), ALQ_EUNSUPPORTED, "split concat view without a two-slot plan");
    if (fused) *fused = fuse != nullptr && route != ROUTE_FCGEMM && route != ROUTE_IGEMM;
    const int cls3 = cls == PROF_IGEMM_BWD ? PROF_IGEMM3_BWD : PROF_IGEMM3_FWD;
    switch (route) {
        case ROUTE_DIRECT: return direct_launch(ctx, g.pd, in, out, bias, relu, N, fuse ? fuse->osumA : nullptr, PROF_DIRECT);
        case ROUTE_FCGEMM:
            return fcgemm_launch(ctx, g.pfc, in, out, bias, relu, N, cls3, (g_no_f16x2 || bias || relu) ? 0.f : fc_in_bound,
                                 (cls == PROF_IGEMM_FWD && !g_no_f16x2) ? g.fc_row_amax : nullptr);
        case ROUTE_IGEMM4: return igemm4_launch(ctx, g.p4, in, out, bias, relu, accumulate, N, cls3, fuse);
        case ROUTE_IGEMM3: return igemm3_launch(ctx, g.p2, g.p3, in, out, bias, relu, accumulate, N, cls3, fuse);
        case ROUTE_IGEMM2: return igemm2_launch(ctx, g.p2, in, out, bias, relu, accumulate, N, cls, fuse);
        case ROUTE_IGEMM: break;
    }
    return igemm_launch(ctx, g.p1, in, out, bias, relu, accumulate, N, cls);
}

static void enum_taps(const int k[3], std::vector<int> *tz, std::vector<int> *ty, std::vector<int> *tx) {
    for (int z = 0; z < k[0]; ++z)
        for (int y = 0; y < k[1]; ++y)
            for (int x = 0; x < k[2]; ++x) {
                tz->push_back(z); ty->push_back(y); tx->push_back(x);
            }
}

static int build_model(alq_model *m, const alq_layer_t *specs, int n_layers) {
    const EngineSwitches &sw = m->sw;
    m->layers.resize(n_layers);
    struct Shp { int D, H, W, C; };
    std::vector<Shp> outs(n_layers);
    Shp cur = {m->in_dims[0], m->in_dims[1], m->in_dims[2], m->in_dims[3]};
    bool flat = false;
    int pidx = 0;
    std::vector<int> src_of(n_layers, -1);
    std::vector<int> dest_of(n_layers, -1);
    for (int i = 0; i < n_layers; ++i) {
        Layer &ly = m->layers[i];
        ly.spec = specs[i];
        const alq_layer_t &sp = ly.spec;
        Shp in = cur;
        if (sp.skip_src >= 0) {
            ALQ_REQUIRE(sp.skip_src < i - 1, ALQ_EUNSUPPORTED, "layer %d: skip source %d must be an earlier, non-adjacent layer", i, sp.skip_src);
            ALQ_REQUIRE(dest_of[sp.skip_src] < 0, ALQ_EUNSUPPORTED, "layer %d feeds more than one concat", sp.skip_src);
            const Shp &s = outs[sp.skip_src];
            ALQ_REQUIRE(!flat && s.D == cur.D && s.H == cur.H && s.W == cur.W, ALQ_EUNSUPPORTED,
// ... 411 lines not shown
    const int nl = (int)m->layers.size();
    ALQ_TRY(m->dalloc(&m->bound_all, (size_t)nl * m->max_batch));
    for (int k = 0; k < nl; ++k) m->layers[k].bound_fwd = m->bound_all + (size_t)k * m->max_batch;
    return ALQ_OK;
}

static int ensure_amax_tiles(alq_model *m, size_t len) {
    if (len <= m->amax_tiles_len) return ALQ_OK;
    ALQ_TRY(m->dalloc(&m->amax_tiles, (size_t)m->max_batch * len));
    m->amax_tiles_len = len;
    return ALQ_OK;
}

static FwdBoundsArgs fwd_bounds_args(const alq_model *m) {
    const int nl = (int)m->layers.size();
    FwdBoundsArgs ba;
    ba.nl = nl;
    for (int k = 0; k < nl && k < 16; ++k) {
        const Layer &lk = m->layers[k];
        const bool par = lk.pidx >= 0 && lk.spec.type != ALQ_FC;
        ba.L[k] = par ? lk.out_l1 : 1.f;
        ba.B[k] = par ? lk.out_bmax : 0.f;
        ba.src2[k] = lk.spec.skip_src;
    }
    return ba;
}


static bool dcp_applies(const alq_model *m, int i, const DropSpec *drop) {
    if (i != 0 || m->layers.size() < 2) return false;
    const Layer &ly = m->layers[0], &nx = m->layers[1];
    const alq_layer_t &sp = ly.spec;
    const View &in = ly.in;
    return ly.spec.type == ALQ_CONV && nx.spec.type == ALQ_POOL && ly.fwd[0].pd.ok && ly.fwd[0].pd.d_W && in.C == 1 && in.cs == 1 &&
           sp.cout == 8 && sp.k[0] == 3 && sp.k[1] == 3 && sp.k[2] == 3 && ly.lo[0] == 1 && ly.lo[1] == 1 && ly.lo[2] == 1 &&
           nx.spec.k[0] == 2 && nx.spec.k[1] == 2 && nx.spec.k[2] == 2 && nx.lo[0] == 0 && nx.lo[1] == 0 && nx.lo[2] == 0 &&
           in.D % 2 == 0 && in.H % 2 == 0 && in.W % 2 == 0 && nx.out.D * 2 == in.D && nx.out.H * 2 == in.H &&
           nx.out.W * 2 == in.W && ((ly.out.cs | ly.out.c0 | nx.out.cs | nx.out.c0) & 3) == 0 && !g_dbg_knobs[KNOB_NO_CONV_POOL] &&
           !(drop && (drop->on(0) || drop->on(1)));
}

static bool flipfix_applies(const alq_model *m, const Layer &ly, const Layer &nx, const View &in, const Igemm2Fuse &fz, bool with_sums) {
    const alq_layer_t &sp = ly.spec;
    return with_sums && fz.fc_bits && fz.in_amax && !g_no_f16x2 && !m->sw.no_flipfix && ly.d_W32 && ly.fwd_l1 > 0.f &&
           sp.s[0] == 1 && sp.s[1] == 1 && sp.s[2] == 1 && in.c0 == 0 && nx.F % 64 == 0 &&
           ((in.split == 0 && in.cs == in.C) || (in.split > 0 && in.cs == in.split && in.C == 2 * in.split));
}

static bool c3d_fwd_applies(const alq_model *m, const Layer &ly, const Layer &nx, const Igemm2Fuse &fz) {
    return ly.c3f.ok && ly.c3f.d_W && nx.c3_part && fz.in_amax && fz.in_amax2 && !g_no_f16x2 && !m->sw.no_c3d;
}

static bool d3d_fwd_applies(const alq_model *m, int i, const View &in, const Igemm2Fuse *fuse, const std::vector<char> &prod, bool with_sums,
                            bool light, const DropSpec *drop) {
    const Layer &ly = m->layers[i];
    return fuse && ly.d3f.ok && ly.d3f.d_Whi && !m->sw.no_d3d && fuse->in_amax && fuse->in_amax2 && !prod[i] && !g_no_f16x2 && two_slot_allowed() &&
           ((with_sums && fuse->osumA) || (light && !m->sw.no_light_kernels)) && in.split == 16 && !(drop && drop->on(i));
}

static bool f3d_fwd_applies(const alq_model *m, int i, const View &in, const Igemm2Fuse *fuse, const std::vector<char> &prod,
                            const std::vector<char> &cons, bool with_sums, bool light, const DropSpec *drop) {
    const Layer &ly = m->layers[i];
    const Layer *nx = i + 1 < (int)m->layers.size() ? &m->layers[i + 1] : nullptr;
    return fuse && ly.f3f.ok && ly.f3f.d_Whi && !m->sw.no_f3d && cons[i] == 2 && fuse->in_amax && !fuse->in_amax2 && !prod[i] && !g_no_f16x2 && two_slot_allowed() &&
           ((with_sums && fuse->osumA) || (light && !m->sw.no_light_kernels)) && ly.spec.relu && in.split == 0 && !(drop && (drop->on(i) || drop->on(i + 1))) && nx && nx->spec.type == ALQ_POOL &&
           nx->spec.k[0] == 2 && nx->spec.k[1] == 2 && nx->spec.k[2] == 2 && nx->lo[0] == 0 && nx->lo[1] == 0 && nx->lo[2] == 0 && nx->out.D == 8 && nx->out.H == 8 &&
           nx->out.W == 8 && nx->out.C == 16 && nx->out.cs == 16 && nx->out.c0 == 0 && !nx->out.split && nx->argmax && !prod[i + 1];
}

static bool t3d_fwd_applies(const alq_model *m, int i, const std::vector<char> &prod, const std::vector<char> &cons, bool with_sums,
                            const DropSpec *drop) {
    const Layer &ly = m->layers[i];
    return ly.t3f.ok && ly.t3f.d_W && !m->sw.no_t3d && !g_dbg_knobs[KNOB_NO_FWD_FUSE] && two_slot_allowed() && !cons[i] && !ly.spec.relu &&
           !(drop && drop->on(i)) && (!with_sums || ly.osum) && !(ly.t3f.kind == 8 && prod[i]);
}

int run_forward(alq_model *m, const float *d_x, int N, bool with_sums, bool keep_all, const DropSpec *drop) {
    alq_ctx *ctx = m->ctx;
    const int nl = (int)m->layers.size();
    bool skip_next = false;
    bool fc_head_fused = false;
    bool c3_head = false;
    m->last.fwd = {};
    const bool no16 = g_no_f16x2 != 0;
    std::vector<char> prod(nl, 0), cons(nl, 0);
    const bool light = !with_sums && !keep_all;
    if ((with_sums || light) && !no16 && !g_dbg_knobs[KNOB_NO_FWD_FUSE] && two_slot_allowed()) {
        auto prod_ok = [&](int p) {
            if (p < 0) return false;
            const Layer &l = m->layers[p];
            if (p == 0 && dcp_applies(m, 0, drop)) return true;
            if (!l.osum) return false;
            if (l.spec.type == ALQ_CONV) return l.fwd[0].p4.ok && !l.fwd[0].pd.ok && !l.fwd[0].pfc.ok && l.fwd[0].p4.a.PT == 1;
            if (l.spec.type == ALQ_CONVT) return l.fwd_all.ok && l.fwd_all.a.PT == 1;
            return false;
        };
        size_t need = 0;
        for (int j = 1; j < nl; ++j) {
            const Layer &l = m->layers[j];
            if (l.dense_head) continue;
            const Igemm4Plan *pl = l.spec.type == ALQ_CONV ? &l.fwd[0].p4 : (l.spec.type == ALQ_CONVT ? &l.fwd_all : nullptr);
            if (!pl || !pl->ok || !pl->d_W16 || pl->multi || pl->a.PT != 1 || !l.osum) continue;
            if (l.spec.type == ALQ_CONV && (l.fwd[0].pd.ok || l.fwd[0].pfc.ok)) continue;
            const int s_ = l.spec.skip_src;
            if (m->sw.f16_fwd_mask < 0 && !m->sw.no_f16_derived && nl <= 16 && ((m->f16_fwd_derived >> j) & 1) && l.spec.type == ALQ_CONV && dcp_applies(m, 0, drop) &&
                (s_ >= 0) == (l.in.split != 0) && !(drop && drop->layers)) {
                cons[j] = 2;
                prod[0] = 1;
                continue;
            }
            if (!(j == nl - 2 && m->layers[nl - 1].fc_part2 && l.spec.type == ALQ_CONV) && m->sw.f16_fwd_mask < 0) continue;
            if (l.spec.type == ALQ_CONVT && !pl->fic) continue;
            if (!prod_ok(j - 1) || (s_ >= 0 && !prod_ok(s_))) continue;
            if ((s_ >= 0) != (l.in.split != 0)) continue;
            if (m->sw.f16_fwd_mask >= 0 && !((m->sw.f16_fwd_mask >> j) & 1)) continue;
            cons[j] = 1; prod[j - 1] = 1;
            if (s_ >= 0) prod[s_] = 1;
        }
        for (int p = 0; p < nl; ++p) {
            if (!prod[p]) continue;
            Layer &l = m->layers[p];
            if (!l.amax_fwd) ALQ_TRY(m->dalloc(&l.amax_fwd, (size_t)m->max_batch));
            if (l.spec.type == ALQ_CONV && !(p == 0 && dcp_applies(m, 0, drop))) need = std::max(need, (size_t)l.fwd[0].p4.a.tpg * 4);
            if (l.spec.type == ALQ_CONVT) need = std::max(need, (size_t)l.fwd_all.a.tpg * (l.fwd_all.multi ? l.fwd_all.a.ngr : 1) * 4);
            if (l.spec.type == ALQ_CONVT && l.t3f.ok) need = std::max(need, (size_t)16);
        }
        ALQ_TRY(ensure_amax_tiles(m, need));
    }
    bool any_derived = false;
    for (int j = 0; j < nl; ++j) any_derived = any_derived || cons[j] == 2;
    m->last.fwd.f16_derived = any_derived;
    if (any_derived) ALQ_TRY(ensure_bounds(m));
    const bool v3f16 = m->v3_fwd_f16 && (with_sums || light) && !no16 && !drop && !any_derived && !dcp_applies(m, 0, drop) && nl <= 16 &&
                       !g_dbg_knobs[KNOB_NO_FWD_FUSE] && two_slot_allowed() && m->layers[0].in.split == 0 && m->layers[0].in.cs == m->layers[0].in.C;
    if (v3f16) {
        if (!m->in_amax) ALQ_TRY(m->dalloc(&m->in_amax, (size_t)m->max_batch));
        ALQ_TRY(ensure_bounds(m));
        ALQ_TRY(k_rowmax_abs(ctx, d_x, N, (long long)m->layers[0].in.vox() * m->layers[0].in.C, m->in_amax));
        FwdBoundsArgs ba = fwd_bounds_args(m);
        ba.from_input = 1;
        ALQ_TRY(k_fwd_bounds(ctx, m->in_amax, N, m->max_batch, ba, m->bound_all));
    }
    auto take_amax = [&](Igemm2Fuse &fz, int j) {
        if (!cons[j]) return;
        const bool dv = cons[j] == 2;
        fz.in_amax = dv ? m->layers[j - 1].bound_fwd : m->layers[j - 1].amax_fwd;
        if (m->layers[j].spec.skip_src >= 0) {
            const Layer &sl = m->layers[m->layers[j].spec.skip_src];
            fz.in_amax2 = dv ? sl.bound_fwd : sl.amax_fwd;
        }
    };
    for (Layer &l : m->layers) l.signs_ready = false;
    for (int i = 0; i < nl; ++i) {
        Layer &ly = m->layers[i];
        ALQ_REQUIRE(ly.pidx < 0 || ly.weights_set, ALQ_EINVAL, "weights of parameterised layer %d not set", ly.pidx);
        if (ly.dense_head) break;
        if (skip_next) { skip_next = false; continue; }
        View in = ly.in;
        if (i == 0) in.p = const_cast<float *>(d_x);
        Igemm2Fuse fz;
        fz.osumA = with_sums ? ly.osum : nullptr;
        const bool head_conv = i + 2 == nl && m->layers[nl - 1].fc_part2 && ly.spec.type == ALQ_CONV;
        const bool light_here = light && (prod[i] || cons[i] || head_conv);
        const Igemm2Fuse *fuse = ((with_sums || light_here) && ly.osum && !g_dbg_knobs[KNOB_NO_FWD_FUSE]) ? &fz : nullptr;
        bool fused = false;
        switch (ly.spec.type) {
            case ALQ_CONV: {
                Layer *nx = i + 1 < nl ? &m->layers[i + 1] : nullptr;
                const alq_layer_t &sp = ly.spec;
                if (dcp_applies(m, i, drop)) {
                    if (prod[i]) ALQ_HIP(hipMemsetAsync(ly.amax_fwd, 0, (size_t)N * sizeof(unsigned), ctx->stream));
                    const bool sg_here = with_sums && !m->sw.no_signs && !m->sw.no_signs0 && sp.relu && ly.out.sg != nullptr;
                    ALQ_TRY(direct_conv_pool_launch(ctx, ly.fwd[0].pd.d_W, in, ly.out, nx->out, ly.d_bias, sp.relu, nx->argmax,
                                                    with_sums ? ly.osum : nullptr, with_sums ? nx->osum : nullptr, N,
                                                    ly.fwd[0].pd.flops_per_patch, prod[i] ? ly.amax_fwd : nullptr,
                                                    sg_here ? ly.out.sg : nullptr, (sg_here && nx->out.sg) ? nx->out.sg : nullptr));
                    m->last.fwd.dcp = g_dcp_last_form;
                    ly.signs_ready = sg_here;
                    nx->signs_ready = sg_here && nx->out.sg != nullptr;
                    if (any_derived)
                        ALQ_TRY(k_fwd_bounds(ctx, ly.amax_fwd, N, m->max_batch, fwd_bounds_args(m), m->bound_all));
                    fused = true;
                    skip_next = true;
                    break;
                }
                if (fuse && nx && i + 2 == nl && nx->fc_part2 && two_slot_allowed()) {
                    fz.fc_W = nx->fc_wv; fz.fc_F = nx->F; fz.fc_part = nx->fc_part2; fz.fc_bits = with_sums ? nx->fc_maskbits : nullptr;
                    take_amax(fz, i);
                    const bool flipfix = flipfix_applies(m, ly, *nx, in, fz, with_sums);
                    if (flipfix) {
                        if (!m->flip_list) {
                            m->flip_cap = flip_list_len(m->max_batch);
                            ALQ_TRY(m->dalloc(&m->flip_cnt, (size_t)flip_segments(m->max_batch)));
                            ALQ_TRY(m->dalloc(&m->flip_list, (size_t)m->flip_cap));
                            ALQ_TRY(m->dalloc(&m->flip_overflow, (size_t)1));
                            ALQ_HIP(hipMemsetAsync(m->flip_overflow, 0, sizeof(unsigned), ctx->stream));
                        }
                        fz.flip_cnt = m->flip_cnt; fz.flip_list = m->flip_list; fz.flip_cap = m->flip_cap; fz.flip_l1 = ly.fwd_l1; fz.flip_bias_nonzero = ly.out_bmax > 0.f;
                    }
                    c3_head = c3d_fwd_applies(m, ly, *nx, fz);
                    if (c3_head)
                        ALQ_TRY(c3d_fwd_launch(ctx, ly.c3f, in, ly.d_bias, N, fz.in_amax, fz.in_amax2, nx->fc_wv, nx->c3_part,
                                               with_sums ? nx->c3_asum : nullptr, reinterpret_cast<unsigned char *>(fz.fc_bits),
                                               flipfix ? std::ldexp(ly.fwd_l1, -24) : 0.f));
                    else
                        ALQ_TRY(igemm4_launch(ctx, ly.fwd[0].p4, in, ly.out, ly.d_bias, ly.spec.relu, 0, N, PROF_IGEMM3_FWD, &fz));
                    if (flipfix)
                        ALQ_TRY(k_flip_fix(ctx, m->flip_list, m->flip_cnt, m->flip_cap, N, in.p, in.split ? in.p + in.delta : nullptr,
                                           in.split ? in.split : in.C, in.split ? in.C - in.split : 0, in.D, in.H, in.W, sp.k[0], sp.k[1], sp.k[2],
                                           ly.lo[0], ly.lo[1], ly.lo[2], ly.d_W32, ly.d_bias, sp.cout,
                                           reinterpret_cast<unsigned char *>(nx->fc_maskbits), nx->F, m->flip_overflow));
                    fused = true;
                    fc_head_fused = true;
                    m->last.fwd.head_fused = true;
                    m->last.fwd.c3 = c3_head;
                    break;
                }
                if (fuse) take_amax(fz, i);
                if (d3d_fwd_applies(m, i, in, fuse, prod, with_sums, light, drop)) {
                    const bool sgd = with_sums && !m->sw.no_signs && ly.spec.relu && ly.out.sg;
                    ALQ_TRY(d3d_fwd_launch(ctx, ly.d3f, N, in.p, in.p + in.delta, fz.in_amax, fz.in_amax2, ly.d_bias, ly.spec.relu ? 1 : 0, ly.out.p,
                                           sgd ? ly.out.sg : nullptr, fz.osumA));
                    ly.signs_ready = sgd;
                    fused = true;
                    m->last.fwd.d3f = 1;
                    break;
                }
                if (f3d_fwd_applies(m, i, in, fuse, prod, cons, with_sums, light, drop)) {
                    const bool sgd = with_sums && !m->sw.no_signs && ly.out.sg;
                    ALQ_TRY(f3d_fwd_launch(ctx, ly.f3f, N, in.p, fz.in_amax, ly.d_bias, ly.out.p, sgd ? ly.out.sg : nullptr, fz.osumA, nx->out.p, nx->argmax,
                                           with_sums ? nx->osum : nullptr));
                    ly.signs_ready = sgd;
                    nx->signs_ready = false;
                    fused = true;
                    skip_next = true;
                    m->last.fwd.f3f = 1;
                    break;
                }
                if (fuse && prod[i]) fz.out_amax = m->amax_tiles;
                if (!ly.fwd_co.empty() && !prod[i] && !cons[i] && two_slot_allowed()) {
                    Igemm2Fuse sz;
                    const bool s16 = v3f16 && i >= 1 && in.split == 0 && ly.spec.skip_src < 0 && !m->sw.no_co_split_f16;
                    if (s16) sz.in_amax = m->layers[i - 1].bound_fwd;
                    for (size_t j = 0; j < ly.fwd_co.size(); ++j) {
                        View oj = ly.out;
                        oj.c0 = ly.out.c0 + (int)j * ly.fwd_co_w;
                        oj.C = ly.fwd_co_w;
                        bool f1 = false;
                        ALQ_TRY(gemm_launch(ctx, ly.fwd_co[j], in, oj, ly.d_bias + j * ly.fwd_co_w, ly.spec.relu, 0, N, PROF_IGEMM_FWD, s16 ? &sz : nullptr, &f1));
                    }
                    fused = false;
                    ly.signs_ready = false;
                    break;
                }
                const bool sg_here = with_sums && fuse && !m->sw.no_signs && ly.spec.relu && ly.out.sg && gemm_route(ly.fwd[0], in, ly.out, 0, fuse) == ROUTE_IGEMM4;
                if (sg_here) fz.sign_out = ly.out.sg;
                {
                    Igemm2Fuse hz;
                    const Igemm2Fuse *fu = fuse;
                    if (v3f16 && !ly.fwd[0].p4.ok && !ly.fwd[0].pd.ok && !ly.fwd[0].pfc.ok && ly.fwd[0].p3.ok && ly.fwd[0].p3.d_W16 && ly.fwd[0].p2.a.PT == 1 &&
                        in.split == 0 && ly.spec.skip_src < 0) {
                        if (fuse) hz = *fuse;
                        hz.in_amax = i == 0 ? m->in_amax : m->layers[i - 1].bound_fwd;
                        hz.in_amax2 = nullptr;
                        fu = &hz;
                    }
                    bool f2 = false;
                    ALQ_TRY(gemm_launch(ctx, ly.fwd[0], in, ly.out, ly.d_bias, ly.spec.relu, 0, N, PROF_IGEMM_FWD, fu, &f2));
                    fused = fuse ? f2 : false;
                }
                ly.signs_ready = sg_here;
                if (fuse && prod[i]) ALQ_TRY(k_rowmax_u32(ctx, m->amax_tiles, ly.fwd[0].p4.a.tpg * 4, N, ly.amax_fwd));
                break;
            }
            case ALQ_CONVT: {
                if (t3d_fwd_applies(m, i, prod, cons, with_sums, drop)) {
                    const bool want_amax = prod[i] != 0;
                    ALQ_TRY(t3d_fwd_launch(ctx, ly.t3f, in, ly.out, ly.d_bias, N, with_sums ? ly.osum : nullptr, want_amax ? m->amax_tiles : nullptr));
                    if (want_amax) ALQ_TRY(k_rowmax_u32(ctx, m->amax_tiles, 16, N, ly.amax_fwd));
                    ly.signs_ready = false;
                    fused = true;
                    m->last.fwd.t3f += 1;
                    break;
                }
                if (ly.fwd_all.ok && two_slot_allowed()) {
                    const bool want_amax = fuse && prod[i];
                    if (fuse) take_amax(fz, i);
                    if (want_amax) fz.out_amax = m->amax_tiles;
                    const bool sg_here = with_sums && fuse && !m->sw.no_signs && ly.spec.relu && ly.out.sg;
                    if (sg_here) fz.sign_out = ly.out.sg;
                    ALQ_TRY(igemm4_launch(ctx, ly.fwd_all, in, ly.out, ly.d_bias, ly.spec.relu, 0, N, PROF_IGEMM3_FWD, fuse));
                    ly.signs_ready = sg_here;
                    if (want_amax)
                        ALQ_TRY(k_rowmax_u32(ctx, m->amax_tiles, ly.fwd_all.a.tpg * (ly.fwd_all.multi ? ly.fwd_all.a.ngr : 1) * 4, N, ly.amax_fwd));
                    fused = fuse != nullptr;
                    break;
                }
                bool all = true;
                for (auto &p : ly.fwd) {
                    bool f1 = false;
                    ALQ_TRY(gemm_launch(ctx, p, in, ly.out, ly.d_bias, ly.spec.relu, 0, N, PROF_IGEMM_FWD, fuse, &f1));
                    all = all && f1;
                }
                fused = all;
                break;
            }
            case ALQ_POOL:
                ALQ_TRY(k_pool_fwd(ctx, in, ly.out, ly.argmax, ly.spec.k, ly.lo, N, with_sums ? ly.osum : nullptr, &fused));
// ... 212 lines not shown
                const bool can = prev_param && prev->out.cs == prev->out.C;
                ALQ_TRY(k_fc_small_bwd(ctx, ly.dout.p, ly.spec.cout, ly.d_Wp, ly.F, N, ly.din.p,
                                       (can && prev->spec.relu) ? prev->out.p : nullptr, can ? prev->dsum : nullptr,
                                       can ? prev->out.C : 0, &fused));
            } else {
                ALQ_TRY(gemm_launch(ctx, ly.bwd, ly.dout, flat_view(ly.din), nullptr, 0, 0, N, PROF_IGEMM_BWD, nullptr, nullptr,
                                    (ly.dout_bound > 0.f && !m->sw.no_bound16) ? ly.dout_bound : 0.f));
            }
        } else {
            Igemm2Fuse fz;
            const Igemm2Fuse *fuse = nullptr;
            if (prev_param && !g_dbg_knobs[KNOB_NO_BWD_FUSE]) {
                const int Cs = ly.spec.skip_src >= 0 ? m->layers[ly.spec.skip_src].out.C : 0;
                if (prev->spec.relu) {
                    fz.mask = prev->out.p; fz.mask_cs = prev->out.cs; fz.mask_c0 = prev->out.c0; fz.mask_from = Cs;
                    if (prev->signs_ready) fz.mask_bits = prev->out.sg;
                }
                if (Cs > 0) { fz.split = Cs; fz.osumB = prev->dsum; } else { fz.osumA = prev->dsum; }
                if (Cs > 0 && (two_slot_allowed() || ly.din.split) && ly.bwd.p4.ok) {
                    Layer &sl = m->layers[ly.spec.skip_src];
                    const bool next_pool = ly.spec.skip_src + 1 < nl && pool_first_ok(m->layers[ly.spec.skip_src + 1], sl);
                    const bool sliced = sl.out.p == prev->out.p && sl.out.cs == prev->out.cs && prev->out.c0 == sl.out.c0 + Cs;
                    const bool splitv = ly.in.split == Cs && sl.out.p == ly.in.p;
                    if (next_pool && (sliced || splitv) && (Cs & 3) == 0) {
                        fz.mask = sl.out.p; fz.mask_cs = sl.out.cs; fz.mask_c0 = sl.out.c0; fz.mask_from = 0;
                        fz.mask_bits = (sl.signs_ready && (!prev->spec.relu || prev->signs_ready)) ? sl.out.sg : nullptr;
                        if (splitv) { fz.mask_split = Cs; fz.mask_delta = ly.in.delta; }
                        if (!prev->spec.relu) fz.mask_to = Cs;
                        fz.osumA = sl.dsum; fz.store_from = Cs;
                        sl.dsum_partial = true;
                    }
                }
                fuse = &fz;
            }
            if (ly.dout_bits) {
                fz.in_bits = ly.dout_bits; fz.in_vec = ly.dout_vec; fz.in_vec_amax = ly.dout_vec_amax;
                fz.in_vec16 = m->sw.no_presplit ? nullptr : ly.dout_vec16;
                const unsigned short *vec16c = ly.dout_vec16c;
                ly.dout_bits = nullptr; ly.dout_vec = nullptr; ly.dout_vec16 = nullptr; ly.dout_vec16c = nullptr;
                const bool honoured = fuse != nullptr;
                const bool c3 = c3d_bwd_applies(m, ly, vec16c, fuse, acc);
                m->last.bwd.c3_bwd = c3;
                if (c3) {
                    int ex = 0;
                    (void)std::frexp(fz.in_vec_amax, &ex);
                    ALQ_TRY(c3d_bwd_launch(ctx, ly.c3b, N, reinterpret_cast<const unsigned char *>(fz.in_bits), vec16c, 14 - ex, fz.mask_bits,
                                           ly.din.p + ly.din.delta, fz.osumA, fz.osumB, m->sw.c3_bwd_rows));
                } else {
                    ALQ_TRY(igemm4_launch(ctx, ly.bwd.p4, ly.dout, ly.din, nullptr, 0, acc, N, PROF_IGEMM3_BWD, &fz));
                }
                fused = honoured;
            } else {
                const bool p4_here = fuse && two_slot_allowed() && ly.bwd.p4.ok && !ly.bwd.p4.multi && ly.bwd.p4.a.PT == 1 && !g_no_f16x2;
                bool hand = false;
                if (p4_here && prev_param && !acc && !(prev->dout_bound > 0.f && !m->sw.no_bound16) && prev->pidx > 0 && prev->bwd.p4.ok && !prev->bwd.p4.multi && prev->bwd.p4.a.PT == 1 &&
                    prev->bwd.p4.d_W16 && !prev->dout.split &&
                    ((prev->bwd.p4.NTW == 1 && prev->bwd.p4.fic) || prev->bwd.p4.NTW == 2)) {
                    const size_t len = (size_t)ly.bwd.p4.a.tpg * 4;
                    if (!m->amax_a) { ALQ_TRY(m->dalloc(&m->amax_a, (size_t)m->max_batch)); ALQ_TRY(m->dalloc(&m->amax_b, (size_t)m->max_batch)); }
                    ALQ_TRY(ensure_amax_tiles(m, len));
                    fz.out_amax = m->amax_tiles;
                    fz.amax_from = fz.split > 0 && fz.split < (1 << 29) ? fz.split : 0;
                    hand = true;
                }
                if (p4_here && !acc && ly.dout_amax) fz.in_amax = ly.dout_amax;
                if (p4_here && !acc && !fz.in_amax && ly.dout_bound > 0.f && !m->sw.no_bound16) fz.in_bound = ly.dout_bound;
                if (!fuse && !acc && two_slot_allowed() && ly.bwd.p4.ok && !ly.bwd.p4.multi && ly.bwd.p4.a.PT == 1 && !g_no_f16x2 && !ly.dout_amax &&
                    ly.dout_bound > 0.f && !m->sw.no_bound16 && !g_dbg_knobs[KNOB_NO_BWD_FUSE]) {
                    fz = Igemm2Fuse();
                    fz.in_bound = ly.dout_bound;
                    fuse = &fz;
                }
                if (!ly.bwd.p4.ok && ly.bwd.p3.ok && ly.bwd.p3.d_W16 && !acc && !g_no_f16x2 && ly.dout_bound > 0.f && !m->sw.no_bound16 && !g_dbg_knobs[KNOB_NO_BWD_FUSE] &&
                    two_slot_allowed() && !ly.bwd.pd.ok && !ly.bwd.pfc.ok) {
                    if (!fuse) { fz = Igemm2Fuse(); fuse = &fz; }
                    fz.in_bound = ly.dout_bound;
                }
                const unsigned *mine = ly.dout_amax;
                ly.dout_amax = nullptr;
                if (t3d_bwd_applies(m, ly, fuse, acc, hand, prev_param)) {
                    ALQ_TRY(t3d_bwd_launch(ctx, ly.t3b, ly.dout, ly.din, N, fz.in_bound, fz.mask ? fz.mask_bits : nullptr, fz.osumA));
                    fused = true;
                    m->last.bwd.t3b += 1;
                } else if (d3d_bwd_applies(m, ly, fuse, acc, hand)) {
                    ALQ_TRY(d3d_bwd_launch(ctx, ly.d3f, N, ly.dout.p, fz.in_bound, ly.din.p, ly.din.p + ly.din.delta, fz.osumB));
                    fused = true;
                    m->last.bwd.d3b = 1;
                } else
                ALQ_TRY(gemm_launch(ctx, ly.bwd, ly.dout, ly.din, nullptr, 0, acc, N, PROF_IGEMM_BWD, fuse, &fused));
                if (hand) {
                    unsigned *dst = mine == m->amax_a ? m->amax_b : m->amax_a;
                    ALQ_TRY(k_rowmax_u32(ctx, m->amax_tiles, ly.bwd.p4.a.tpg * 4, N, dst));
                    prev->dout_amax = dst;
                }
            }
        }
        if (prev_param && fused) prev->delta_ready = true;
    }
    return ALQ_OK;
}

int make_drop(const alq_model *m, float keep_prob, uint64_t seed, int64_t first_sample, const int32_t *h_layers, int n_layers,
              DropSpec *d) {
    ALQ_REQUIRE(keep_prob > 0.f && keep_prob <= 1.f, ALQ_EINVAL, "keep_prob %g outside (0, 1]", (double)keep_prob);
    ALQ_REQUIRE(n_layers == 0 || h_layers, ALQ_EINVAL, "dropout layer list missing");
    d->keep_prob = keep_prob; d->seed = seed; d->first_sample = first_sample; d->layers = 0;
    for (int i = 0; i < n_layers; ++i) {
        ALQ_REQUIRE(h_layers[i] >= 0 && h_layers[i] < (int)m->layers.size() && h_layers[i] < 64, ALQ_EINVAL, "dropout layer %d", h_layers[i]);
        d->layers |= 1ull << h_layers[i];
    }
    return ALQ_OK;
}

extern "C" {

int alq_model_out_voxels(const alq_model *m) { return m ? (int)m->V : ALQ_EINVAL; }

int alq_model_set_aleatoric(alq_model *m, int on) {
    ALQ_REQUIRE(m, ALQ_EINVAL, "alq_model_set_aleatoric: null model");
    ALQ_REQUIRE(m->dense && m->nclass >= 3, ALQ_EUNSUPPORTED,
                "alq_model_set_aleatoric: a log-variance channel needs a 1x1 conv head of 3 .. 8 channels (2 .. 7 classes beside it)");
    if (on && !m->au) {
        ALQ_HIP(hipSetDevice(m->ctx->device));
        ALQ_TRY(m->dalloc(&m->au, (size_t)m->max_batch * m->V));
    }
    m->aleatoric = on != 0;
    return ALQ_OK;
}

int alq_forward_au(alq_model *m, const float *d_x, int N, float keep_prob, uint64_t seed, int64_t first_sample,
                   const int32_t *h_drop_layers, int n_drop_layers, float *d_post, int64_t *d_pred, float *d_au, float *d_logits) {
    ALQ_REQUIRE(m && d_x && d_au, ALQ_EINVAL, "alq_forward_au: null argument");
    ALQ_REQUIRE(m->aleatoric, ALQ_EUNSUPPORTED, "alq_forward_au: the model has no log-variance channel (alq_model_set_aleatoric)");
    ALQ_REQUIRE(N >= 0 && N <= m->max_batch, ALQ_EINVAL, "alq_forward_au: N=%d exceeds max_batch=%d", N, m->max_batch);
    if (N == 0) return ALQ_OK;
    ALQ_HIP(hipSetDevice(m->ctx->device));
    DropSpec ds;
    ALQ_TRY(make_drop(m, keep_prob, seed, first_sample, h_drop_layers, n_drop_layers, &ds));
    ALQ_TRY(prepare_call(m, false));
    ALQ_TRY(run_forward(m, d_x, N, false, true, &ds));
    return dense_forward_head(m, d_x, N, d_post, d_pred, false, d_au, d_logits);
}

int alq_forward_dropout(alq_model *m, const float *d_x, int N, float keep_prob, uint64_t seed, int64_t first_sample,
                        const int32_t *h_drop_layers, int n_drop_layers, float *d_post, int64_t *d_pred) {
    ALQ_REQUIRE(m && d_x, ALQ_EINVAL, "alq_forward_dropout: null argument");
    ALQ_REQUIRE(N >= 0 && N <= m->max_batch, ALQ_EINVAL, "alq_forward_dropout: N=%d exceeds max_batch=%d", N, m->max_batch);
    if (N == 0) return ALQ_OK;
    ALQ_HIP(hipSetDevice(m->ctx->device));
    DropSpec ds;
    ALQ_TRY(make_drop(m, keep_prob, seed, first_sample, h_drop_layers, n_drop_layers, &ds));
    ALQ_TRY(prepare_call(m, false));
    ALQ_TRY(run_forward(m, d_x, N, false, true, &ds));
    if (m->dense) return dense_forward_head(m, d_x, N, d_post, d_pred, false);
    ALQ_TRY(k_softmax(m->ctx, m->logits, m->nclass, N, d_post ? d_post : m->post, d_pred));
    return ALQ_OK;
}

int alq_model_create(alq_ctx *ctx, const alq_layer_t *layers, int n_layers, const int32_t in_dims[4],
                     int max_batch, alq_model **out) {
    ALQ_REQUIRE(ctx && layers && in_dims && out, ALQ_EINVAL, "alq_model_create: null argument");
    ALQ_REQUIRE(n_layers >= 1 && n_layers <= 64 && max_batch >= 1, ALQ_EINVAL, "alq_model_create: bad sizes");
    ALQ_HIP(hipSetDevice(ctx->device));
    alq_model *m = new alq_model();
    m->ctx = ctx;
    m->max_batch = max_batch;
    m->sw = read_engine_switches();
    for (int i = 0; i < 4; ++i) m->in_dims[i] = in_dims[i];
    m->epp = (int64_t)in_dims[0] * in_dims[1] * in_dims[2] * in_dims[3];
    const int rc = build_model(m, layers, n_layers);
// ... 153 lines not shown
            ALQ_HIP(hipStreamSynchronize(m->ctx->stream));
            return ALQ_OK;
        }
        const FcGemmPlan &pl = what <= 7 ? ly.fwd[0].pfc : ly.bwd.pfc;
        const void *src = (what & 1) ? pl.d_W16 : pl.d_W;
        ALQ_REQUIRE(pl.ok && src, ALQ_EUNSUPPORTED, "layer %d: this form is not packed", layer_idx);
        const int64_t e = (int64_t)pl.K * pl.N * ((what & 1) ? 2 : 3) / 2;
        if (elems_out) *elems_out = e;
        ALQ_HIP(hipMemcpyAsync(d_out, src, (size_t)e * 4, hipMemcpyDeviceToDevice, m->ctx->stream));
        return ALQ_OK;
    }
    if (what >= 11 && what <= 13) {
        if (what == 11) {
            ALQ_REQUIRE(ly.osum && m->last.call_fisher, ALQ_EUNSUPPORTED, "layer %d: no channel sums of its output in the last pass", layer_idx);
            if (elems_out) *elems_out = (int64_t)N * ly.out.vox();
            ALQ_HIP(hipMemcpyAsync(d_out, ly.osum, (size_t)N * ly.out.vox() * sizeof(float), hipMemcpyDeviceToDevice, m->ctx->stream));
            return ALQ_OK;
        }
        if (what == 12) {
            const View &v = ly.out;
            ALQ_REQUIRE(v.sg && ly.signs_ready && ((v.C | v.cs | v.c0) & 3) == 0 && ((int64_t)N * v.vox() * v.cs) % 16 == 0, ALQ_EUNSUPPORTED,
                        "layer %d: no sign field of its output in the last pass", layer_idx);
            if (elems_out) *elems_out = (int64_t)N * v.vox() * v.cs / 16;
            ALQ_HIP(hipMemcpyAsync(d_out, v.sg, (size_t)N * v.vox() * v.cs / 4, hipMemcpyDeviceToDevice, m->ctx->stream));
            return ALQ_OK;
        }
        ALQ_REQUIRE(ly.spec.type == ALQ_POOL && ly.argmax && ((int64_t)N * ly.out.vox() * ly.out.C) % 4 == 0, ALQ_EUNSUPPORTED, "layer %d has no arg-max field", layer_idx);
        if (elems_out) *elems_out = (int64_t)N * ly.out.vox() * ly.out.C / 4;
        ALQ_HIP(hipMemcpyAsync(d_out, ly.argmax, (size_t)N * ly.out.vox() * ly.out.C, hipMemcpyDeviceToDevice, m->ctx->stream));
        return ALQ_OK;
    }
    if (what == 0 || what == 1) {
        const Layer &head = m->layers.back();
        ALQ_REQUIRE(!(layer_idx + 2 == (int)m->layers.size() && head.spec.type == ALQ_FC &&
                      (what == 0 ? m->last.fwd.head_fused
                                 : (m->last.call_fisher && head.fc_maskbits != nullptr && two_slot_allowed()))),
                    ALQ_EUNSUPPORTED, "layer %d: this tensor is not materialised in a Fisher pass (fc head fused into the layer: "
                    "create the model under ALQ_NO_FC_BITS=1 to keep it)", layer_idx);
        const View &v = what == 0 ? ly.out : ly.dout;
        if (elems_out) *elems_out = (int64_t)N * v.elems();
        return debug_view_copy(m->ctx, v, N, d_out);
    }
    ALQ_REQUIRE(ly.pidx >= 0 && !ly.dense_head && (what == 2 || what == 3), ALQ_EINVAL, "layer has no channel-sum fields");
    const bool isfc = ly.spec.type == ALQ_FC;
    const int64_t e = (int64_t)N * (isfc ? 1 : (what == 2 ? ly.in.vox() : ly.out.vox()));
    if (elems_out) *elems_out = e;
    ALQ_HIP(hipMemcpyAsync(d_out, what == 2 ? ly.asum : ly.dsum, e * sizeof(float), hipMemcpyDeviceToDevice,
                           m->ctx->stream));
    return ALQ_OK;
}

int alq_model_engine_info(alq_model *m, int what) {
    ALQ_REQUIRE(m, ALQ_EINVAL, "alq_model_engine_info: bad argument");
    switch (what) {
        case ALQ_INFO_SUBNORMALS_OK:
            ALQ_HIP(hipSetDevice(m->ctx->device));
            return c3d_subnormals_ok(m->ctx);
        case ALQ_INFO_C3D_FWD: return m->last.fwd.c3 ? 1 : 0;
        case ALQ_INFO_C3D_BWD: return m->last.bwd.c3_bwd ? 1 : 0;
        case ALQ_INFO_C3D_ONE_ACC:
            for (const Layer &ly : m->layers)
                if (ly.c3f.ok) return ly.c3f.oneacc;
            return 0;
        case ALQ_INFO_FLIP_OVERFLOW: {
            ALQ_HIP(hipSetDevice(m->ctx->device));
            if (!m->flip_overflow) return 0;
            unsigned h = 0;
            ALQ_HIP(hipMemcpyAsync(&h, m->flip_overflow, sizeof(unsigned), hipMemcpyDeviceToHost, m->ctx->stream));
            ALQ_HIP(hipStreamSynchronize(m->ctx->stream));
            return h > 0x7fffffffu ? 0x7fffffff : (int)h;
        }
        case ALQ_INFO_F16_DERIVED: return m->last.fwd.f16_derived ? 1 : 0;
        case ALQ_INFO_T3D_FWD: return m->last.fwd.t3f;
        case ALQ_INFO_T3D_BWD: return m->last.bwd.t3b;
        case ALQ_INFO_E3D_BWD: return m->last.bwd.e3b;
        case ALQ_INFO_D3D_FWD: return m->last.fwd.d3f;
        case ALQ_INFO_D3D_BWD: return m->last.bwd.d3b;
        case ALQ_INFO_F3D_FWD: return m->last.fwd.f3f;
        case ALQ_INFO_C3D_BWD_FORM: return m->last.bwd.c3_bwd ? m->sw.c3_bwd_rows : 0;
        case ALQ_INFO_HOST_PACK_ELEMS: return m->host_pack_elems > 0x7fffffffll ? 0x7fffffff : (int)m->host_pack_elems;
        case ALQ_INFO_LSUM: return m->last.lsum;
        case ALQ_INFO_DCP_FORM: return m->last.fwd.dcp;
        case ALQ_INFO_E3D_BWD_FORM: return m->last.bwd.e3b_form;
        default: break;
    }
    set_error("alq_model_engine_info: bad argument");
    return ALQ_EINVAL;
}

int alq_debug_set(int key, int value) {
    ALQ_REQUIRE(key >= 0 && key < ALQ_NKNOBS, ALQ_EINVAL, "alq_debug_set: bad key");
    g_knob_override[key] = value > 0 ? value : -1;
    g_dbg_knobs[key] = value;
    return ALQ_OK;
}

int alq_debug_set_stamp_buffer(void *d_buf) {
    g_igemm2_dbg = reinterpret_cast<unsigned long long *>(d_buf);
    return ALQ_OK;
}

}
```

nn-active-learning_amd/csrc/model_types.h:

```cpp
#pragma once
#include <algorithm>

#include "alq_internal.h"

namespace alq {

struct Layer {
    alq_layer_t spec;
    int pidx = -1;
    View in, out;
    View din, dout;
    int lo[3] = {0, 0, 0};
    bool dense_fc_small = false;
    bool dense_head = false;
    int64_t F = 0;
    int64_t w_elems = 0, b_elems = 0;
    float *d_bias = nullptr;
    float *d_Wp = nullptr;
    std::vector<Gemm> fwd;
    std::vector<Gemm> fwd_co;
    int fwd_co_w = 0;
    Igemm4Plan fwd_all;
    Gemm bwd;
    bool has_bwd = false;
    bool weights_set = false;
    float *d_Wres = nullptr;
    bool fallback_stale = false;
    uint8_t *argmax = nullptr;
    float *asum = nullptr, *dsum = nullptr;
    double *ls_field = nullptr;
    float *osum = nullptr;
    bool delta_ready = false;
    bool signs_ready = false;
    bool dsum_partial = false;
    float *fc_partials = nullptr;
    unsigned *fc_maskbits = nullptr;
    float *fc_wv = nullptr;
    unsigned *fc_wv16 = nullptr;
    float fc_wv_amax = 0.f;
    const unsigned *dout_amax = nullptr;
    unsigned *amax_fwd = nullptr;
    float dout_vec_amax = 0.f;
    double bwd_l1 = 0;
    float dout_bound = 0.f;
    float *d_W32 = nullptr;
    float fwd_l1 = 0.f;
    float out_l1 = 0.f, out_bmax = 0.f;
    unsigned *bound_fwd = nullptr;
    float *fc_part2 = nullptr;
    int fc_slices2 = 0;
    C3dPlan c3f, c3b;
    D3dPlan d3f;
    F3dPlan f3f;
    E3dPlan e3b;
    T3dPlan t3f, t3b;
    float *c3_part = nullptr, *c3_asum = nullptr;
    unsigned short *fc_wv16c = nullptr;
    const unsigned short *dout_vec16c = nullptr;
    const unsigned *dout_bits = nullptr;
    const float *dout_vec = nullptr;
    const unsigned *dout_vec16 = nullptr;
    int fc_slices = 0;
    bool out_is_skip_src = false;
    std::vector<std::vector<int>> class_taps;
    std::vector<float> hv_hW;
    int hv_src = 0;
    bool hv_stale = false;
    float *hv_W = nullptr;
    double *hv_A = nullptr, *hv_D = nullptr, *hv_Ra = nullptr, *hv_Rd = nullptr;
};

}

struct PassInfo {
    struct Fwd {
        bool head_fused = false;
        bool c3 = false;
        int t3f = 0;
        int d3f = 0;
        int f3f = 0;
        int dcp = 0;
        bool f16_derived = false;
    } fwd;
    struct Bwd {
        bool c3_bwd = false;
        int t3b = 0;
        int e3b = 0;
        int e3b_form = 0;
        int d3b = 0;
    } bwd;
    int lsum = 0;
    bool call_fisher = false;
};

struct alq_model {
    alq_ctx *ctx = nullptr;
    int max_batch = 0;
    alq::EngineSwitches sw;
    PassInfo last;
    unsigned *amax_a = nullptr, *amax_b = nullptr, *amax_tiles = nullptr;
    unsigned *flip_cnt = nullptr, *flip_list = nullptr;
    int flip_cap = 0;
    unsigned *bound_all = nullptr;
    unsigned *in_amax = nullptr;
    bool v3_fwd_f16 = false;
    unsigned *flip_overflow = nullptr;
    size_t amax_tiles_len = 0;
    int in_dims[4] = {1, 1, 1, 1};
    int nclass = 0;
    bool dense = false;
    int64_t V = 1;
    bool aleatoric = false;
    float *au = nullptr;
    double *dh_part = nullptr;
    int L = 0;
    std::vector<alq::Layer> layers;
    std::vector<void *> allocs;
    float *logits = nullptr, *dlogits = nullptr, *post = nullptr;
    double *S = nullptr, *sizes = nullptr, *Apart = nullptr;
    double *Spart = nullptr;
    int *nslab = nullptr;
    int nslab_max = 1;
    float *wg_partial = nullptr;
    size_t wg_partial_len = 0;
    double *gn_partial = nullptr;
    size_t gn_partial_len = 0;
    double *df_scratch = nullptr;
    double *ls_part = nullptr;
    std::vector<int> ls_nslab;
    int ls_nslab_max = 0;
    float *x_stage = nullptr;
    int64_t epp = 0;
    int f16_fwd_derived = 0;
    int64_t host_pack_elems = 0;
    void *d_wscal = nullptr;
    bool hv_ready = false;
    double *hv_part = nullptr;
    double *hv_p64 = nullptr;

    template <typename T>
    int dalloc(T **p, size_t count) {
        void *q = nullptr;
        const size_t bytes = std::max<size_t>(count * sizeof(T), 256);
        if (hipMalloc(&q, bytes) != hipSuccess) {
            alq::set_error("hipMalloc of %zu bytes failed", bytes);
            return ALQ_ENOMEM;
        }
        allocs.push_back(q);
        *p = reinterpret_cast<T *>(q);
        return ALQ_OK;
    }
};

template <typename T, typename D>
int ensure(alq_model *m, D **d, size_t count) {
    T *p = static_cast<T *>(*d);
    if (!p) ALQ_TRY(m->dalloc(&p, count));
    *d = p;
    return ALQ_OK;
}

template <typename T, typename D>
int upload(alq_model *m, D **d, const std::vector<T> &h) {
    ALQ_TRY(ensure<T>(m, d, h.size()));
    ALQ_HIP(hipMemcpyAsync(*d, h.data(), h.size() * sizeof(T), hipMemcpyHostToDevice, m->ctx->stream));
    return ALQ_OK;
}

template <typename T, typename D>
int upload_release(alq_model *m, D **d, std::vector<T> *h) {
    ALQ_TRY(upload(m, d, *h));
    ALQ_HIP(hipStreamSynchronize(m->ctx->stream));
    std::vector<T>().swap(*h);
// ... 27 lines not shown
```

nn-active-learning_amd/csrc/sweep_common.h:

```cpp
#ifndef ALQ_SWEEP_COMMON_H
#define ALQ_SWEEP_COMMON_H
#include "alq_internal.h"

#include <algorithm>

namespace alq {

typedef float f32x4 __attribute__((ext_vector_type(4)));
typedef float f32x2 __attribute__((ext_vector_type(2)));
typedef int i32x4 __attribute__((ext_vector_type(4)));
typedef int i32x2 __attribute__((ext_vector_type(2)));
typedef __bf16 bf16x2 __attribute__((ext_vector_type(2)));
typedef __bf16 bf16x8 __attribute__((ext_vector_type(8)));
typedef _Float16 f16x8 __attribute__((ext_vector_type(8)));
typedef _Float16 f16x2 __attribute__((ext_vector_type(2)));

__device__ inline __amdgpu_buffer_rsrc_t sw_rsrc(const void *base, unsigned long long bytes) {
    return __builtin_amdgcn_make_buffer_rsrc(const_cast<void *>(base), 0, (int)(unsigned)bytes, 0x00020000);
}
constexpr unsigned SW_OOB = 0xffffff00u;

__device__ inline int sw_s(unsigned v) { return __builtin_amdgcn_readfirstlane((int)v); }

template <int V> struct IC { static constexpr int value = V; };

constexpr int SW_FILL_MASK = 0x096;

__device__ inline int sw_patch_exp(unsigned fm) {
    const int ex = (int)((fm >> 23) & 255u) - 126;
    const int ce = 14 - ex;
    return fm ? (ce < 96 ? ce : 96) : 0;
}

#define SW_XCD_DEAL(N)                                                                                         \
    const int G8 = (int)gridDim.x >> 3, xcd = (int)blockIdx.x & 7, jb = (int)blockIdx.x >> 3;                  \
    const int npx = (N) > xcd ? ((N) - xcd + 7) >> 3 : 0
#define SW_PATCH_ORDER(N)                                                                                      \
    SW_XCD_DEAL(N);                                                                                            \
    const int npw = npx > jb ? (npx - jb + G8 - 1) / G8 : 0;                                                   \
    auto patch_of = [&](int i) __attribute__((always_inline)) { return 8 * (jb + (i < npw ? i : npw - 1) * G8) + xcd; }

inline unsigned sweep_grid(const alq_ctx *ctx, long long items, int per_cu) {
    const long long g = std::min<long long>((long long)per_cu * ctx->num_cus, items);
    return (unsigned)std::max<long long>(8, (g + 7) / 8 * 8);
}

inline bool is_conv3_same(const int k[3], const int lo[3], const int s[3]) {
    return k[0] == 3 && k[1] == 3 && k[2] == 3 && s[0] == 1 && s[1] == 1 && s[2] == 1 && lo[0] == 1 && lo[1] == 1 && lo[2] == 1;
}

#define SWEEP_REQUIRE_PATCHES(N, name) ALQ_REQUIRE((N) < 4096, ALQ_EUNSUPPORTED, name ": 32-bit byte offsets hold fewer than 4096 patches per pass")

template <typename K, typename A>
inline int sweep_launch(alq_ctx *ctx, K kernel, unsigned grid, unsigned block, size_t lds, const A &args) {
    ALQ_HIP(hipFuncSetAttribute(reinterpret_cast<const void *>(kernel), hipFuncAttributeMaxDynamicSharedMemorySize, (int)lds));
    hipLaunchKernelGGL(kernel, dim3(grid), dim3(block), lds, ctx->stream, args);
    ALQ_HIP(hipGetLastError());
    return ALQ_OK;
}

}

#endif
```

nn-active-learning_amd/csrc/t3d8b.hip:

```cpp
#include "f16_pair.h"
#include "sweep_common.h"

#include <algorithm>
#include <cmath>
#include <cstdlib>
#include <cstring>
#include <vector>

namespace alq {

struct T8BwdArgs {
    const float *dout;
    float *din;
    const unsigned short *W;
    const unsigned char *mask_bits;
    float *dsum;
    float scale, scale11, inv;
    int N;
};

constexpr int T8B_KG = 17 * 16;
constexpr int T8B_PIECE = 2 * T8B_KG;
constexpr int T8B_ROW = 2 * T8B_PIECE + 16;
constexpr int T8B_PLANE = 18 * T8B_ROW + 32;
constexpr int T8B_RING = 3 * T8B_PLANE;
constexpr int T8B_XCH = 4 * 16 * 4;
constexpr int T8B_LDS = T8B_RING + T8B_XCH;

__device__ __host__ inline int t8b_row(int y) { return y * T8B_ROW + ((y >> 1) & 1) * 16; }

__global__ __launch_bounds__(256, 2) void t3d8_bwd_kernel(const T8BwdArgs a) {
    extern __shared__ __attribute__((aligned(16))) char t8lds[];
    const int lane = threadIdx.x & 63, wave = __builtin_amdgcn_readfirstlane((int)(threadIdx.x >> 6));
    const int cb = wave & 1, tp = wave >> 1;
    char *ring = t8lds;
    float *xch = reinterpret_cast<float *>(t8lds + T8B_RING);
    for (int i = threadIdx.x; i < T8B_LDS / 16; i += 256) reinterpret_cast<i32x4 *>(t8lds)[i] = i32x4{0, 0, 0, 0};
    __syncthreads();
    const int n = lane & 15, kg = lane >> 4;
    f16x8 wh[15], wl[15];
#pragma unroll
    for (int c = 0; c < 15; ++c) {
        wh[c] = *reinterpret_cast<const f16x8 *>(a.W + ((size_t)((0 * 2 + cb) * 15 + c) * 64 + lane) * 8);
        wl[c] = *reinterpret_cast<const f16x8 *>(a.W + ((size_t)((1 * 2 + cb) * 15 + c) * 64 + lane) * 8);
    }
#pragma unroll
    for (int c = 0; c < 15; ++c) asm volatile("" : "+v"(wh[c]), "+v"(wl[c]));

    const __amdgpu_buffer_rsrc_t i_rsrc = sw_rsrc(a.dout, (unsigned long long)a.N * 4096 * 64);
    const __amdgpu_buffer_rsrc_t o_rsrc = sw_rsrc(a.din, (unsigned long long)a.N * 512 * 128);
    const __amdgpu_buffer_rsrc_t m_rsrc = sw_rsrc(a.mask_bits, a.mask_bits ? (unsigned long long)a.N * 512 * 8 : 0ull);
    const __amdgpu_buffer_rsrc_t u_rsrc = sw_rsrc(a.dsum, a.dsum ? (unsigned long long)a.N * 512 * 4 : 0ull);

    const int sx = lane >> 2, cq = lane & 3;
    const int w_off = (cq >> 1) * T8B_KG + sx * 16 + (cq & 1) * 8;
    const unsigned ldA = (unsigned)lane * 16u;
    int f01[2][3], f22[2][2];
#pragma unroll
    for (int j = 0; j < 2; ++j) {
        const int qy = 2 * (tp + 2 * j) + (n >> 3), qx = n & 7, h = kg >> 1;
#pragma unroll
        for (int ty = 0; ty < 3; ++ty) f01[j][ty] = t8b_row(2 * qy + ty) + (kg & 1) * T8B_KG + (2 * qx + h) * 16;
        f22[j][0] = t8b_row(2 * qy + h) + (kg & 1) * T8B_KG + (2 * qx + 2) * 16;
        f22[j][1] = t8b_row(2 * qy + 2 + h) + (kg & 1) * T8B_KG + (2 * qx + 2) * 16;
    }
    const unsigned e_out = (unsigned)(cb * 64 + kg * 16), e_msk = (unsigned)(cb * 4 + kg);

    SW_PATCH_ORDER(a.N);

    f32x4 RA[8];
    auto fetch = [&](int p, int pa) __attribute__((always_inline)) {
#pragma unroll
        for (int j = 0; j < 8; ++j) {
            const int k = 8 * wave + j;
            const int pz = pa + (k >> 4);
            const unsigned row = ((unsigned)p * 16u + (unsigned)(pz < 16 ? pz : 15)) * 16u + (unsigned)(k & 15);
            RA[j] = __builtin_bit_cast(f32x4, __builtin_amdgcn_raw_buffer_load_b128(i_rsrc, (int)ldA, sw_s(row * 1024u), 0));
        }
    };
    auto stage = [&](int pa, bool on) __attribute__((always_inline)) {
#pragma unroll
        for (int j = 0; j < 8; ++j) {
            const int k = 8 * wave + j;
            const int pz = pa + (k >> 4), y = k & 15;
            const bool rv = on && pz < 16;
            const float sc = rv ? a.scale : 0.f, sc11 = rv ? a.scale11 : 0.f;
            char *dst = ring + (pz % 3) * T8B_PLANE + t8b_row(y) + w_off;
            const f32x4 g = RA[j];
            const f16x2 h01 = __builtin_convertvector(f32x2{g.x * sc, g.y * sc}, f16x2), h23 = __builtin_convertvector(f32x2{g.z * sc, g.w * sc}, f16x2);
            const f16x2 l01 = __builtin_convertvector(f32x2{__builtin_fmaf((float)h01.x, -2048.f, g.x * sc11), __builtin_fmaf((float)h01.y, -2048.f, g.y * sc11)}, f16x2);
            const f16x2 l23 = __builtin_convertvector(f32x2{__builtin_fmaf((float)h23.x, -2048.f, g.z * sc11), __builtin_fmaf((float)h23.y, -2048.f, g.w * sc11)}, f16x2);
            *reinterpret_cast<i32x2 *>(dst) = i32x2{__builtin_bit_cast(int, h01), __builtin_bit_cast(int, h23)};
            *reinterpret_cast<i32x2 *>(dst + T8B_PIECE) = i32x2{__builtin_bit_cast(int, l01), __builtin_bit_cast(int, l23)};
        }
    };

    const int total = 8 * npw;
    if (total > 0) fetch(patch_of(0), 1);
    for (int g = 0; g < total; ++g) {
        const int i = g >> 3, zq = g & 7;
        const int p = patch_of(i);
        if (zq == 0) {
            f32x4 R0[4];
#pragma unroll
            for (int j = 0; j < 4; ++j)
                R0[j] = __builtin_bit_cast(f32x4, __builtin_amdgcn_raw_buffer_load_b128(i_rsrc, (int)ldA, sw_s((((unsigned)p * 16u) * 16u + (unsigned)(4 * wave + j)) * 1024u), 0));
#pragma unroll
            for (int j = 0; j < 4; ++j) {
                char *dst = ring + t8b_row(4 * wave + j) + w_off;
                const f32x4 gq = R0[j];
                const float sc = a.scale, sc11 = a.scale11;
                const f16x2 h01 = __builtin_convertvector(f32x2{gq.x * sc, gq.y * sc}, f16x2), h23 = __builtin_convertvector(f32x2{gq.z * sc, gq.w * sc}, f16x2);
                const f16x2 l01 = __builtin_convertvector(f32x2{__builtin_fmaf((float)h01.x, -2048.f, gq.x * sc11), __builtin_fmaf((float)h01.y, -2048.f, gq.y * sc11)}, f16x2);
                const f16x2 l23 = __builtin_convertvector(f32x2{__builtin_fmaf((float)h23.x, -2048.f, gq.z * sc11), __builtin_fmaf((float)h23.y, -2048.f, gq.w * sc11)}, f16x2);
                *reinterpret_cast<i32x2 *>(dst) = i32x2{__builtin_bit_cast(int, h01), __builtin_bit_cast(int, h23)};
                *reinterpret_cast<i32x2 *>(dst + T8B_PIECE) = i32x2{__builtin_bit_cast(int, l01), __builtin_bit_cast(int, l23)};
            }
        }
        stage(2 * zq + 1, true);
        unsigned mb[2];
#pragma unroll
        for (int j = 0; j < 2; ++j) {
            const unsigned vox = ((unsigned)p * 8u + (unsigned)zq) * 64u + (unsigned)(tp + 2 * j) * 16u;
            mb[j] = a.mask_bits ? (unsigned)(unsigned char)__builtin_amdgcn_raw_buffer_load_b8(m_rsrc, (int)((unsigned)n * 8u + e_msk), sw_s(vox * 8u), 0) : 0xfu;
        }
        __syncthreads();
        if (g + 1 < total) fetch(patch_of((g + 1) >> 3), 2 * ((g + 1) & 7) + 1);
        f32x4 c[2], cx[2];
#pragma unroll
        for (int j = 0; j < 2; ++j) { c[j] = f32x4{0.f, 0.f, 0.f, 0.f}; cx[j] = f32x4{0.f, 0.f, 0.f, 0.f}; }
#pragma unroll
        for (int tz = 0; tz < 3; ++tz) {
            const char *pl = ring + ((2 * zq + tz) % 3) * T8B_PLANE;
#pragma unroll
            for (int j = 0; j < 2; ++j)
#pragma unroll
                for (int pi = 0; pi < 5; ++pi) {
                    const char *src = pl + (pi < 3 ? f01[j][pi] : f22[j][pi - 3]);
                    const f16x8 xh = *reinterpret_cast<const f16x8 *>(src);
                    const f16x8 xl = *reinterpret_cast<const f16x8 *>(src + T8B_PIECE);
                    cx[j] = __builtin_amdgcn_mfma_f32_16x16x32_f16(wl[tz * 5 + pi], xh, cx[j], 0, 0, 0);
                    c[j] = __builtin_amdgcn_mfma_f32_16x16x32_f16(wh[tz * 5 + pi], xh, c[j], 0, 0, 0);
                    cx[j] = __builtin_amdgcn_mfma_f32_16x16x32_f16(wh[tz * 5 + pi], xl, cx[j], 0, 0, 0);
                }
        }
        float part[2];
#pragma unroll
        for (int j = 0; j < 2; ++j) {
            const unsigned vox = (unsigned)sw_s((((unsigned)p * 8u + (unsigned)zq) * 64u + (unsigned)(tp + 2 * j) * 16u));
            const unsigned m = mb[j];
            const float v0 = (m & 1u) ? __builtin_fmaf(cx[j].x, 0x1p-11f, c[j].x) * a.inv : 0.f, v1 = (m & 2u) ? __builtin_fmaf(cx[j].y, 0x1p-11f, c[j].y) * a.inv : 0.f;
            const float v2 = (m & 4u) ? __builtin_fmaf(cx[j].z, 0x1p-11f, c[j].z) * a.inv : 0.f, v3 = (m & 8u) ? __builtin_fmaf(cx[j].w, 0x1p-11f, c[j].w) * a.inv : 0.f;
            const f32x4 o = f32x4{v0, v1, v2, v3};
            __builtin_amdgcn_raw_buffer_store_b128(__builtin_bit_cast(i32x4, o), o_rsrc, (int)((unsigned)n * 128u + e_out), (int)(vox * 128u), 0);
            float s_ = (v0 + v1) + (v2 + v3);
            s_ += __shfl_xor(s_, 16, 64);
            s_ += __shfl_xor(s_, 32, 64);
            part[j] = s_;
            if (cb == 1 && kg == 0) xch[(tp + 2 * j) * 16 + n] = s_;
            asm volatile("s_nop 3" :: "v"(o) : "memory");
        }
        __syncthreads();
        if (cb == 0 && a.dsum) {
#pragma unroll
            for (int j = 0; j < 2; ++j) {
                const unsigned vox = (unsigned)sw_s((((unsigned)p * 8u + (unsigned)zq) * 64u + (unsigned)(tp + 2 * j) * 16u));
                const float s_ = part[j] + xch[(tp + 2 * j) * 16 + n];
                __builtin_amdgcn_raw_buffer_store_b32(__builtin_bit_cast(int, s_), u_rsrc, (int)(kg == 0 ? (unsigned)n * 4u : SW_OOB), (int)(vox * 4u), 0);
            }
        }
    }
}

void t3d8_bwd_pack(T3dPlan *plan, const float *W) {
    plan->w_exp = f16_pair_exp(W, (size_t)27 * 16 * 32);
    plan->h_W.assign((size_t)2 * 2 * 15 * 64 * 8, 0);
    for (int cb = 0; cb < 2; ++cb)
        for (int tz = 0; tz < 3; ++tz)
            for (int pi = 0; pi < 5; ++pi)
                for (int lane = 0; lane < 64; ++lane) {
                    const int r = lane & 15, kg = lane >> 4, h = kg >> 1;
                    int ty, tx;
                    bool any = true;
                    if (pi < 3) { ty = pi; tx = h; } else if (pi == 3) { ty = h; tx = 2; } else { ty = 2; tx = 2; any = h == 0; }
                    for (int c = 0; c < 8; ++c) {
                        const int co = 8 * (kg & 1) + c, ci = 16 * cb + r;
                        const float w = any ? W[((size_t)((tz * 3 + ty) * 3 + tx) * 16 + co) * 32 + ci] : 0.f;
                        const size_t f = (size_t)(cb * 15 + tz * 5 + pi);
                        f16_pair_split(w, plan->w_exp, 11, &plan->h_W[(((size_t)0 * 30 + f) * 64 + lane) * 8 + c], &plan->h_W[(((size_t)1 * 30 + f) * 64 + lane) * 8 + c]);
                    }
                }
}

int t3d8_bwd_launch(alq_ctx *ctx, const T3dPlan &plan, const View &dout, const View &din, int N, float in_bound, const unsigned char *mask_bits, float *dsum) {
    ALQ_REQUIRE(plan.ok && plan.d_W && plan.kind == 8, ALQ_EINVAL, "t3d8: backward weights not set");
    ALQ_REQUIRE(dout.cs == 16 && dout.c0 == 0 && dout.split == 0 && dout.D == 16 && din.cs == 32 && din.c0 == 0 && din.split == 0 && din.D == 8 && in_bound > 0.f,
                ALQ_EINVAL, "t3d8: view mismatch");
    SWEEP_REQUIRE_PATCHES(N, "t3d8");
    if (N <= 0) return ALQ_OK;
    const int e_in = f16_pair_exp(&in_bound, 1);
    T8BwdArgs a;
    a.dout = dout.p; a.din = din.p; a.W = reinterpret_cast<const unsigned short *>(plan.d_W); a.mask_bits = mask_bits; a.dsum = dsum;
    a.scale = std::ldexp(1.f, e_in); a.scale11 = std::ldexp(1.f, e_in + 11); a.inv = std::ldexp(1.f, -(e_in + plan.w_exp)); a.N = N;
    ProfScope ps(ctx, PROF_IGEMM_F16, plan.flops_per_patch * N);
    return sweep_launch(ctx, t3d8_bwd_kernel, sweep_grid(ctx, N, 2), 256, T8B_LDS, a);
}

}
```

Measured before the change: 287,000.

## Add alternate LDS layouts for d3d/t3d8 backward and hold e3d low weights in registers

```diff
diff --git a/include/alq.h b/include/alq.h
--- a/include/alq.h
+++ b/include/alq.h
@@ -270,7 +270,8 @@
     ALQ_INFO_HOST_PACK_ELEMS = 14,
     ALQ_INFO_LSUM = 15,
     ALQ_INFO_DCP_FORM = 16,
-    ALQ_INFO_E3D_BWD_FORM = 17
+    ALQ_INFO_E3D_BWD_FORM = 17,
+    ALQ_INFO_LDS_LAYOUT = 19
 };
 int alq_model_engine_info(alq_model *m, int what);
 
diff --git a/nn-active-learning_amd/csrc/alq_internal.h b/nn-active-learning_amd/csrc/alq_internal.h
--- a/nn-active-learning_amd/csrc/alq_internal.h
+++ b/nn-active-learning_amd/csrc/alq_internal.h
@@ -248,6 +248,7 @@
 extern int g_no_f16x2;
 extern int g_no_fixed;
 extern int g_no_xcd_order;
+extern int g_lds_layout;
 int igemm2_build_plan(const IgemmPlan &p1, Igemm2Plan *p2);
 void igemm2_pack_weights(Igemm2Plan *p2, const std::vector<float> &Bmat);
 int igemm2_launch(alq_ctx *ctx, const Igemm2Plan &plan, const View &in, const View &out, const float *bias,
diff --git a/nn-active-learning_amd/csrc/d3d.hip b/nn-active-learning_amd/csrc/d3d.hip
--- a/nn-active-learning_amd/csrc/d3d.hip
+++ b/nn-active-learning_amd/csrc/d3d.hip
@@ -1,4 +1,5 @@
 #include "f16_pair.h"
+#include "lds_layout.h"
 #include "sweep_common.h"
 
 #include <algorithm>
@@ -23,11 +24,7 @@
     int N;
 };
 
-constexpr int D3_KG = 18 * 16;
-constexpr int D3_ROWB = 4 * D3_KG;
-constexpr int D3_SLOT = 2 * D3_ROWB;
-constexpr int D3_PLANE = 18 * D3_SLOT;
-constexpr int D3_STRIP = 2 * D3_PLANE;
+static_assert(lds::D3F<lds::OLD>::STRIP <= 160 * 1024 && lds::D3F<lds::NEW>::STRIP <= 160 * 1024, "d3d_fwd: LDS layout");
 
 #ifndef D3_PIPE
 #define D3_PIPE 2
@@ -38,11 +35,13 @@
 
 struct D3Row { f32x4 a, b; };
 
+template <int FAM>
 __global__ __launch_bounds__(256) __attribute__((amdgpu_waves_per_eu(1, 1))) void d3d_fwd_kernel(const D3Args a) {
+    typedef lds::D3F<FAM> L;
     extern __shared__ __attribute__((aligned(16))) char d3lds[];
     const int lane = threadIdx.x & 63, wave = __builtin_amdgcn_readfirstlane((int)(threadIdx.x >> 6));
     char *strip = d3lds;
-    for (int i = threadIdx.x; i < D3_STRIP / 16; i += 256) reinterpret_cast<i32x4 *>(strip)[i] = i32x4{0, 0, 0, 0};
+    for (int i = threadIdx.x; i < L::STRIP / 16; i += 256) reinterpret_cast<i32x4 *>(strip)[i] = i32x4{0, 0, 0, 0};
     __syncthreads();
     const int n = lane & 15, kg = lane >> 4;
     f16x8 wh[27], wl[27];
@@ -70,10 +69,9 @@
     const __amdgpu_buffer_rsrc_t s_rsrc = sw_rsrc(a.sg, a.sg ? (unsigned long long)a.N * 4096 * 4 : 0ull);
     const __amdgpu_buffer_rsrc_t u_rsrc = sw_rsrc(a.osum, a.osum ? (unsigned long long)a.N * 4096 * 4 : 0ull);
 
-    const int sx = lane >> 2, cq = lane & 3;
-    char *const w_base = strip + (4 * wave + 1) * D3_SLOT + (cq >> 1) * D3_KG + (sx + 1) * 16 + (cq & 1) * 8;
+    char *const w_base = strip + L::write(wave, lane, 0, 0);
     const unsigned ldA = (unsigned)lane * 16u;
-    const char *const f_base = strip + 4 * wave * D3_SLOT + kg * D3_KG + n * 16;
+    const char *const f_base = strip + L::read(wave, lane, 0, 0, 0);
     const unsigned e_out = (unsigned)n * 64u + (unsigned)kg * 16u, e_sg = (unsigned)n * 4u + (unsigned)kg;
     const unsigned e_sum = kg == 0 ? (unsigned)n * 4u : SW_OOB;
 
@@ -90,13 +88,13 @@
     };
     auto stage_unit = [&](auto U, int img, float sc, float sc11) __attribute__((always_inline)) {
         constexpr int u = decltype(U)::value, r = u >> 1, h = u & 1;
-        char *dst = w_base + img * D3_PLANE + r * D3_SLOT + h * 2 * D3_KG;
+        char *dst = w_base + img * L::PLANE + L::wstep(u, 0);
         const f32x4 g = h ? RA[r].b : RA[r].a;
         const f16x2 h01 = __builtin_convertvector(f32x2{g.x * sc, g.y * sc}, f16x2), h23 = __builtin_convertvector(f32x2{g.z * sc, g.w * sc}, f16x2);
         const f16x2 l01 = __builtin_convertvector(f32x2{__builtin_fmaf((float)h01.x, -2048.f, g.x * sc11), __builtin_fmaf((float)h01.y, -2048.f, g.y * sc11)}, f16x2);
         const f16x2 l23 = __builtin_convertvector(f32x2{__builtin_fmaf((float)h23.x, -2048.f, g.z * sc11), __builtin_fmaf((float)h23.y, -2048.f, g.w * sc11)}, f16x2);
         *reinterpret_cast<i32x2 *>(dst) = i32x2{__builtin_bit_cast(int, h01), __builtin_bit_cast(int, h23)};
-        *reinterpret_cast<i32x2 *>(dst + D3_ROWB) = i32x2{__builtin_bit_cast(int, l01), __builtin_bit_cast(int, l23)};
+        *reinterpret_cast<i32x2 *>(dst + (L::wstep(u, 1) - L::wstep(u, 0))) = i32x2{__builtin_bit_cast(int, l01), __builtin_bit_cast(int, l23)};
     };
 
     f32x4 acc[3][4], acx[3][4];
@@ -141,14 +139,14 @@
         const float sc = nv ? __builtin_ldexpf(1.f, cen) : 0.f, sc11 = nv ? __builtin_ldexpf(1.f, cen + 11) : 0.f;
         const int img = q & 1;
         asm volatile("s_waitcnt lgkmcnt(0)\n\ts_barrier" ::: "memory");
-        const char *fb = f_base + img * D3_PLANE;
+        const char *fb = f_base + img * L::PLANE;
         f16x8 Fh[2][3], Fl[2][3];
         auto frag = [&](auto R, f16x8 *fh, f16x8 *fl) __attribute__((always_inline)) {
             constexpr int r = decltype(R)::value;
 #pragma unroll
             for (int dx = 0; dx < 3; ++dx) {
-                fh[dx] = *reinterpret_cast<const f16x8 *>(fb + r * D3_SLOT + dx * 16);
-                fl[dx] = *reinterpret_cast<const f16x8 *>(fb + r * D3_SLOT + dx * 16 + D3_ROWB);
+                fh[dx] = *reinterpret_cast<const f16x8 *>(fb + L::step(r, dx, 0));
+                fl[dx] = *reinterpret_cast<const f16x8 *>(fb + L::step(r, dx, 1));
             }
         };
         frag(IC<0>{}, Fh[0], Fl[0]);
@@ -241,18 +239,16 @@
     float scale, scale11, inv;
     int N;
 };
-constexpr int DB_KG = 18 * 16;
-constexpr int DB_ROWB = 2 * DB_KG;
-constexpr int DB_SLOT = 2 * DB_ROWB;
-constexpr int DB_PLANE = 19 * DB_SLOT;
-constexpr int DB_STRIP = 2 * DB_PLANE;
-
+static_assert(lds::D3B<lds::OLD>::STRIP <= 160 * 1024 && lds::D3B<lds::NEW>::STRIP <= 160 * 1024, "d3d_bwd: LDS layout");
+
+template <int FAM>
 __global__ __launch_bounds__(256) __attribute__((amdgpu_waves_per_eu(1, 1))) void d3d_bwd_kernel(const D3BArgs a) {
+    typedef lds::D3B<FAM> L;
     extern __shared__ __attribute__((aligned(16))) char d3lds[];
     const int lane = threadIdx.x & 63, wave = __builtin_amdgcn_readfirstlane((int)(threadIdx.x >> 6));
     const int cb = wave & 1, rg = wave >> 1;
     char *strip = d3lds;
-    for (int i = threadIdx.x; i < DB_STRIP / 16; i += 256) reinterpret_cast<i32x4 *>(strip)[i] = i32x4{0, 0, 0, 0};
+    for (int i = threadIdx.x; i < L::STRIP / 16; i += 256) reinterpret_cast<i32x4 *>(strip)[i] = i32x4{0, 0, 0, 0};
     __syncthreads();
     const int n = lane & 15, kg = lane >> 4;
     f16x8 wh[15], wl[15];
@@ -268,11 +264,10 @@
     const __amdgpu_buffer_rsrc_t o_rsrc = sw_rsrc(cb ? a.dinB : a.dinA, (unsigned long long)a.N * 4096 * 64);
     const __amdgpu_buffer_rsrc_t u_rsrc = sw_rsrc(a.sumB, a.sumB ? (unsigned long long)a.N * 4096 * 4 : 0ull);
 
-    const int sx = lane >> 2, cq = lane & 3;
-    char *const w_base = strip + (4 * wave + 1) * DB_SLOT + (cq >> 1) * DB_KG + (sx + 1) * 16 + (cq & 1) * 8;
+    char *const w_base = strip + L::write(wave, lane, 0, 0);
     const unsigned ldA = (unsigned)lane * 16u;
-    const char *const f01 = strip + 8 * rg * DB_SLOT + (kg & 1) * DB_KG + (n + (kg >> 1)) * 16;
-    const char *const f22 = strip + 8 * rg * DB_SLOT + (kg >> 1) * DB_SLOT + (kg & 1) * DB_KG + (n + 2) * 16;
+    const char *const f01 = strip + L::read(wave, lane, 0, 0, 0);
+    const char *const f22 = strip + L::read(wave, lane, 0, 1, 0);
     const unsigned e_out = (unsigned)n * 64u + (unsigned)kg * 16u;
     const unsigned e_sum = (kg == 0 && cb == 1) ? (unsigned)n * 4u : SW_OOB;
 
@@ -287,13 +282,13 @@
     };
     auto stage_unit = [&](auto U, int img, float sc, float sc11) __attribute__((always_inline)) {
         constexpr int r = decltype(U)::value;
-        char *dst = w_base + img * DB_PLANE + r * DB_SLOT;
+        char *dst = w_base + img * L::PLANE + L::wstep(r, 0);
         const f32x4 g = RA[r];
         const f16x2 h01 = __builtin_convertvector(f32x2{g.x * sc, g.y * sc}, f16x2), h23 = __builtin_convertvector(f32x2{g.z * sc, g.w * sc}, f16x2);
         const f16x2 l01 = __builtin_convertvector(f32x2{__builtin_fmaf((float)h01.x, -2048.f, g.x * sc11), __builtin_fmaf((float)h01.y, -2048.f, g.y * sc11)}, f16x2);
         const f16x2 l23 = __builtin_convertvector(f32x2{__builtin_fmaf((float)h23.x, -2048.f, g.z * sc11), __builtin_fmaf((float)h23.y, -2048.f, g.w * sc11)}, f16x2);
         *reinterpret_cast<i32x2 *>(dst) = i32x2{__builtin_bit_cast(int, h01), __builtin_bit_cast(int, h23)};
-        *reinterpret_cast<i32x2 *>(dst + DB_ROWB) = i32x2{__builtin_bit_cast(int, l01), __builtin_bit_cast(int, l23)};
+        *reinterpret_cast<i32x2 *>(dst + L::PIECE) = i32x2{__builtin_bit_cast(int, l01), __builtin_bit_cast(int, l23)};
     };
 
     f32x4 acc[3][8], acx[3][8];
@@ -331,14 +326,14 @@
         const float sc = nv ? a.scale : 0.f, sc11 = nv ? a.scale11 : 0.f;
         const int img = q & 1;
         asm volatile("s_waitcnt lgkmcnt(0)\n\ts_barrier" ::: "memory");
-        const char *fa = f01 + img * DB_PLANE, *fb = f22 + img * DB_PLANE;
+        const char *fa = f01 + img * L::PLANE, *fb = f22 + img * L::PLANE;
         f16x8 Fh[2][2], Fl[2][2];
         auto frag = [&](auto R, f16x8 *fh, f16x8 *fl) __attribute__((always_inline)) {
             constexpr int r = decltype(R)::value;
-            fh[0] = *reinterpret_cast<const f16x8 *>(fa + r * DB_SLOT);
-            fl[0] = *reinterpret_cast<const f16x8 *>(fa + r * DB_SLOT + DB_ROWB);
-            fh[1] = *reinterpret_cast<const f16x8 *>(fb + r * DB_SLOT);
-            fl[1] = *reinterpret_cast<const f16x8 *>(fb + r * DB_SLOT + DB_ROWB);
+            fh[0] = *reinterpret_cast<const f16x8 *>(fa + L::step(r, 0));
+            fl[0] = *reinterpret_cast<const f16x8 *>(fa + L::step(r, 1));
+            fh[1] = *reinterpret_cast<const f16x8 *>(fb + L::step(r, 0));
+            fl[1] = *reinterpret_cast<const f16x8 *>(fb + L::step(r, 1));
         };
         frag(IC<0>{}, Fh[0], Fl[0]);
         auto mm = [&](auto ST, auto RY, auto KS, const f16x8 &xh, const f16x8 &xl) __attribute__((always_inline)) {
@@ -470,7 +465,8 @@
     a.dinA = dinA; a.dinB = dinB; a.sumB = sumB;
     a.scale = std::ldexp(1.f, e_in); a.scale11 = std::ldexp(1.f, e_in + 11); a.inv = std::ldexp(1.f, -(e_in + plan.w_exp)); a.N = N;
     ProfScope ps(ctx, PROF_IGEMM_F16, plan.flops_per_patch * N);
-    return sweep_launch(ctx, d3d_bwd_kernel, sweep_grid(ctx, N, 1), 256, DB_STRIP, a);
+    if (lds::pick(g_lds_layout, lds::D3B_DEFAULT) == lds::OLD) return sweep_launch(ctx, d3d_bwd_kernel<lds::OLD>, sweep_grid(ctx, N, 1), 256, lds::D3B<lds::OLD>::STRIP, a);
+    return sweep_launch(ctx, d3d_bwd_kernel<lds::NEW>, sweep_grid(ctx, N, 1), 256, lds::D3B<lds::NEW>::STRIP, a);
 }
 
 int d3d_fwd_launch(alq_ctx *ctx, const D3dPlan &plan, int N, const float *inA, const float *inB, const unsigned *amaxA, const unsigned *amaxB,
@@ -484,7 +480,8 @@
     a.Whi = reinterpret_cast<const unsigned short *>(plan.d_Whi); a.Wlo = reinterpret_cast<const unsigned short *>(plan.d_Wlo);
     a.bias = bias; a.out = out; a.sg = sg; a.osum = osum; a.e_w = plan.w_exp; a.relu = relu; a.N = N;
     ProfScope ps(ctx, PROF_IGEMM_F16, plan.flops_per_patch * N);
-    return sweep_launch(ctx, d3d_fwd_kernel, sweep_grid(ctx, N, 1), 256, D3_STRIP, a);
-}
-
-}
+    if (lds::pick(g_lds_layout, lds::D3F_DEFAULT) == lds::OLD) return sweep_launch(ctx, d3d_fwd_kernel<lds::OLD>, sweep_grid(ctx, N, 1), 256, lds::D3F<lds::OLD>::STRIP, a);
+    return sweep_launch(ctx, d3d_fwd_kernel<lds::NEW>, sweep_grid(ctx, N, 1), 256, lds::D3F<lds::NEW>::STRIP, a);
+}
+
+}
diff --git a/nn-active-learning_amd/csrc/e3d.hip b/nn-active-learning_amd/csrc/e3d.hip
--- a/nn-active-learning_amd/csrc/e3d.hip
+++ b/nn-active-learning_amd/csrc/e3d.hip
@@ -237,33 +237,30 @@
 constexpr int E3Z_IMG = 18 * E3_SLOT;
 constexpr int E3Z_ZERO = 4 * E3Z_IMG;
 constexpr int E3Z_SINK = 5 * E3Z_IMG;
-constexpr int E3Z_LDS = E3_WLO + E3Z_SINK + E3_SLOT;
+constexpr int E3Z_LDS = E3Z_SINK + E3_SLOT;
 static_assert(E3Z_IMG % 16 == 0 && E3Z_LDS <= 160 * 1024, "e3d plane sweep: LDS layout");
 
 struct E3ZRowB { f32x4 dp; unsigned am; };
 
 __global__ __launch_bounds__(512) void e3d_bwdz_kernel(const E3Args a) {
     extern __shared__ __attribute__((aligned(16))) char e3lds[];
-    {
-        const i32x4 *src = reinterpret_cast<const i32x4 *>(a.Wlo);
-        i32x4 *dst = reinterpret_cast<i32x4 *>(e3lds);
-        for (int i = threadIdx.x; i < E3_WLO / 16; i += 512) dst[i] = src[i];
-        for (int i = threadIdx.x; i < (E3Z_LDS - E3_WLO) / 16; i += 512) dst[E3_WLO / 16 + i] = i32x4{0, 0, 0, 0};
-    }
+    for (int i = threadIdx.x; i < E3Z_LDS / 16; i += 512) reinterpret_cast<i32x4 *>(e3lds)[i] = i32x4{0, 0, 0, 0};
     __syncthreads();
     const int lane = threadIdx.x & 63, wave = __builtin_amdgcn_readfirstlane((int)(threadIdx.x >> 6));
-    char *strip = e3lds + E3_WLO;
+    char *strip = e3lds;
     const int n = lane & 15, kg = lane >> 4, ry = n >> 3, j = n & 7;
-    f16x8 wh[9][2];
+    f16x8 wh[9][2], wlr[9][2];
 #pragma unroll
     for (int c = 0; c < 9; ++c)
 #pragma unroll
-        for (int s = 0; s < 2; ++s) wh[c][s] = *reinterpret_cast<const f16x8 *>(a.Whi + ((size_t)(c * 2 + s) * 64 + lane) * 8);
+        for (int s = 0; s < 2; ++s) {
+            wh[c][s] = *reinterpret_cast<const f16x8 *>(a.Whi + ((size_t)(c * 2 + s) * 64 + lane) * 8);
+            wlr[c][s] = *reinterpret_cast<const f16x8 *>(a.Wlo + ((size_t)(c * 2 + s) * 64 + lane) * 8);
+        }
 #pragma unroll
     for (int c = 0; c < 9; ++c)
 #pragma unroll
-        for (int s = 0; s < 2; ++s) asm volatile("" : "+v"(wh[c][s]));
-    const char *wl = e3lds + lane * 16;
+        for (int s = 0; s < 2; ++s) asm volatile("" : "+v"(wh[c][s]), "+v"(wlr[c][s]));
 
     const __amdgpu_buffer_rsrc_t sk_rsrc = sw_rsrc(a.skip, (unsigned long long)a.N * 4096 * 64);
     const __amdgpu_buffer_rsrc_t dp_rsrc = sw_rsrc(a.dpool, (unsigned long long)a.N * 512 * 64);
@@ -386,7 +383,7 @@
                     for (int s2 = 0; s2 < 2; ++s2) {
                         const f16x8 xh = *reinterpret_cast<const f16x8 *>(src + s2 * 64);
                         const f16x8 xl = *reinterpret_cast<const f16x8 *>(src + s2 * 64 + E3_ROWB);
-                        const f16x8 wlo = *reinterpret_cast<const f16x8 *>(wl + ((dz * 3 + dy) * 2 + s2) * 1024);
+                        const f16x8 wlo = wlr[dz * 3 + dy][s2];
                         const f16x8 whi = wh[dz * 3 + dy][s2];
                         cl = __builtin_amdgcn_mfma_f32_16x16x32_f16(wlo, xh, cl, 0, 0, 0);
                         cl = __builtin_amdgcn_mfma_f32_16x16x32_f16(whi, xl, cl, 0, 0, 0);
diff --git a/nn-active-learning_amd/csrc/engine_switches.h b/nn-active-learning_amd/csrc/engine_switches.h
--- a/nn-active-learning_amd/csrc/engine_switches.h
+++ b/nn-active-learning_amd/csrc/engine_switches.h
@@ -16,11 +16,12 @@
     KNOB_NO_CONV_POOL = 7,
     KNOB_DCP_NARROW = 8,
     KNOB_E3D_GRID_CAP = 9,
-    ALQ_NKNOBS = 10
+    KNOB_SWEEP_GRID_CAP = 10,
+    ALQ_NKNOBS = 11
 };
 
 struct EngineSwitches {
-    int knobs[ALQ_NKNOBS] = {0, 0, 0, 0, 0, 0, 0, 0, 0, 0};
+    int knobs[ALQ_NKNOBS] = {0, 0, 0, 0, 0, 0, 0, 0, 0, 0, 0};
     int disable_v2 = 0;
     int disable_v3 = 0;
     int disable_v4 = 0;
@@ -57,6 +58,7 @@
     int no_d3b = 0;
     int no_f3d = 0;
     int no_t3d = 0;
+    int lds_layout = 0;
 };
 
 enum SwitchRule {
@@ -144,6 +146,7 @@
             case SW_ROWS:       dst = (v && std::atoi(v) == 4) ? 4 : ((v && std::atoi(v) == 8) ? 8 : 7); break;
         }
     }
+    if (const char *v = std::getenv("ALQ_LDS_OLD_LAYOUT")) sw.lds_layout = std::atoi(v) == 1 ? 1 : 2;
     return sw;
 }
 
diff --git a/nn-active-learning_amd/csrc/igemm2.hip b/nn-active-learning_amd/csrc/igemm2.hip
--- a/nn-active-learning_amd/csrc/igemm2.hip
+++ b/nn-active-learning_amd/csrc/igemm2.hip
@@ -506,8 +506,9 @@
 unsigned long long *g_igemm2_dbg = nullptr;
 int g_no_f16x2 = 0;
 int g_no_xcd_order = 0;
+int g_lds_layout = 0;
 int g_no_fixed = 0;
-int g_dbg_knobs[ALQ_NKNOBS] = {0, 0, 0, 0, 0, 0, 0, 0, 0, 0};
+int g_dbg_knobs[ALQ_NKNOBS] = {0, 0, 0, 0, 0, 0, 0, 0, 0, 0, 0};
 
 template <int NTW, bool WRES, int GEO, bool SUMS>
 static int launch2_s(alq_ctx *ctx, const Igemm2Plan &plan, const Igemm2Args &a, unsigned grid) {
diff --git a/nn-active-learning_amd/csrc/lds_layout.h b/nn-active-learning_amd/csrc/lds_layout.h
--- /dev/null
+++ b/nn-active-learning_amd/csrc/lds_layout.h
@@ -0,0 +1,69 @@
+#ifndef ALQ_LDS_LAYOUT_H
+#define ALQ_LDS_LAYOUT_H
+
+namespace alq {
+namespace lds {
+
+enum Family { OLD = 1, NEW = 2 };
+
+constexpr int D3F_DEFAULT = OLD, D3B_DEFAULT = NEW, T8B_DEFAULT = NEW;
+constexpr int pick(int forced, int dflt) { return forced == OLD || forced == NEW ? forced : dflt; }
+
+template <int F> struct D3F {
+    static constexpr int KG = 18 * 16;
+    static constexpr int PIECE = F == OLD ? 4 * KG : 768 + 2 * KG;
+    static constexpr int SLOT = 2 * PIECE;
+    static constexpr int ROWS = 18;
+    static constexpr int PLANE = ROWS * SLOT;
+    static constexpr int STRIP = 2 * PLANE;
+    static constexpr int kg_off(int kg) { return F == OLD ? kg * KG : (kg & 1) * 768 + (kg >> 1) * KG; }
+    static constexpr int cell(int row, int slot, int kg, int piece) { return row * SLOT + piece * PIECE + kg_off(kg) + slot * 16; }
+    static constexpr int write(int wave, int lane, int unit, int piece) {
+        return cell(4 * wave + 1 + (unit >> 1), (lane >> 2) + 1, 2 * (unit & 1) + ((lane & 3) >> 1), piece) + (lane & 1) * 8;
+    }
+    static constexpr int read(int wave, int lane, int block, int dx, int piece) { return cell(4 * wave + block, (lane & 15) + dx, lane >> 4, piece); }
+    static constexpr int step(int block, int dx, int piece) { return cell(block, dx, 0, piece); }
+    static constexpr int wstep(int unit, int piece) { return cell(unit >> 1, 0, 2 * (unit & 1), piece); }
+};
+
+template <int F> struct D3B {
+    static constexpr int KG = 18 * 16;
+    static constexpr int PIECE = F == OLD ? 2 * KG : KG;
+    static constexpr int HALF = F == OLD ? KG : 768;
+    static constexpr int SLOT = F == OLD ? 4 * KG : 768 + 2 * KG;
+    static constexpr int ROWS = 19;
+    static constexpr int PLANE = ROWS * SLOT;
+    static constexpr int STRIP = 2 * PLANE;
+    static constexpr int cell(int row, int slot, int half, int piece) { return row * SLOT + piece * PIECE + half * HALF + slot * 16; }
+    static constexpr int write(int wave, int lane, int unit, int piece) {
+        return cell(4 * wave + 1 + unit, (lane >> 2) + 1, (lane & 3) >> 1, piece) + (lane & 1) * 8;
+    }
+    static constexpr int read(int wave, int lane, int block, int kind, int piece) {
+        const int n = lane & 15, kg = lane >> 4, row = 8 * (wave >> 1) + block;
+        return kind == 0 ? cell(row, n + (kg >> 1), kg & 1, piece) : cell(row + (kg >> 1), n + 2, kg & 1, piece);
+    }
+    static constexpr int step(int block, int piece) { return cell(block, 0, 0, piece); }
+    static constexpr int wstep(int unit, int piece) { return cell(unit, 0, 0, piece); }
+};
+
+template <int F> struct T8B {
+    static constexpr int KG = 17 * 16;
+    static constexpr int PIECE = 2 * KG;
+    static constexpr int ROW = F == OLD ? 2 * PIECE + 16 : 1152;
+    static constexpr int ROWS = 18;
+    static constexpr int PLANE = F == OLD ? ROWS * ROW + 32 : ROWS * ROW;
+    static constexpr int RING = 3 * PLANE;
+    static constexpr int XCH = 4 * 16 * 4;
+    static constexpr int LDS = RING + XCH;
+    static constexpr int row(int y) { return y * ROW + (F == OLD ? ((y >> 1) & 1) * 16 : 0); }
+    static constexpr int cell(int y, int slot, int half, int piece) { return row(y) + piece * PIECE + half * KG + slot * 16; }
+    static constexpr int write(int lane, int y, int piece) { return cell(y, lane >> 2, (lane & 3) >> 1, piece) + (lane & 1) * 8; }
+    static constexpr int read(int wave, int lane, int j, int pi, int piece) {
+        const int n = lane & 15, kg = lane >> 4, h = kg >> 1, qy = 2 * ((wave >> 1) + 2 * j) + (n >> 3), qx = n & 7;
+        return pi < 3 ? cell(2 * qy + pi, 2 * qx + h, kg & 1, piece) : cell(2 * qy + (pi == 3 ? 0 : 2) + h, 2 * qx + 2, kg & 1, piece);
+    }
+};
+
+}
+}
+#endif
diff --git a/nn-active-learning_amd/csrc/model.hip b/nn-active-learning_amd/csrc/model.hip
--- a/nn-active-learning_amd/csrc/model.hip
+++ b/nn-active-learning_amd/csrc/model.hip
@@ -3,6 +3,7 @@
 #include <cstring>
 #include <string>
 
+#include "lds_layout.h"
 #include "model_types.h"
 
 namespace alq {
@@ -18,13 +19,14 @@
 
 using namespace alq;
 
-static int g_knob_override[ALQ_NKNOBS] = {-1, -1, -1, -1, -1, -1, -1, -1, -1, -1};
+static int g_knob_override[ALQ_NKNOBS] = {-1, -1, -1, -1, -1, -1, -1, -1, -1, -1, -1};
 
 static void apply_knobs(const alq_model *m) {
     for (int k = 0; k < ALQ_NKNOBS; ++k) g_dbg_knobs[k] = g_knob_override[k] >= 0 ? g_knob_override[k] : m->sw.knobs[k];
     g_no_f16x2 = m->sw.no_f16x2;
     g_no_xcd_order = m->sw.no_xcd_order;
     g_no_fixed = m->sw.no_fixed;
+    g_lds_layout = m->sw.lds_layout;
 }
 
 static int gemm_build(const EngineSwitches &sw, const ConvDesc &d, int max_batch, Gemm *g, const G4Geom *g4 = nullptr) {
@@ -602,6 +604,7 @@
     bool fc_head_fused = false;
     bool c3_head = false;
     m->last.fwd = {};
+    m->last.lds_layout = 0;
     const bool no16 = g_no_f16x2 != 0;
     std::vector<char> prod(nl, 0), cons(nl, 0);
     const bool light = !with_sums && !keep_all;
@@ -744,6 +747,7 @@
                     ly.signs_ready = sgd;
                     fused = true;
                     m->last.fwd.d3f = 1;
+                    m->last.lds_layout |= lds::pick(m->sw.lds_layout, lds::D3F_DEFAULT);
                     break;
                 }
                 if (f3d_fwd_applies(m, i, in, fuse, prod, cons, with_sums, light, drop)) {
@@ -1122,10 +1126,12 @@
                     ALQ_TRY(t3d_bwd_launch(ctx, ly.t3b, ly.dout, ly.din, N, fz.in_bound, fz.mask ? fz.mask_bits : nullptr, fz.osumA));
                     fused = true;
                     m->last.bwd.t3b += 1;
+                    if (ly.t3b.kind == 8) m->last.lds_layout |= lds::pick(m->sw.lds_layout, lds::T8B_DEFAULT);
                 } else if (d3d_bwd_applies(m, ly, fuse, acc, hand)) {
                     ALQ_TRY(d3d_bwd_launch(ctx, ly.d3f, N, ly.dout.p, fz.in_bound, ly.din.p, ly.din.p + ly.din.delta, fz.osumB));
                     fused = true;
                     m->last.bwd.d3b = 1;
+                    m->last.lds_layout |= lds::pick(m->sw.lds_layout, lds::D3B_DEFAULT);
                 } else
                 ALQ_TRY(gemm_launch(ctx, ly.bwd, ly.dout, ly.din, nullptr, 0, acc, N, PROF_IGEMM_BWD, fuse, &fused));
                 if (hand) {
@@ -1445,6 +1451,7 @@
         case ALQ_INFO_LSUM: return m->last.lsum;
         case ALQ_INFO_DCP_FORM: return m->last.fwd.dcp;
         case ALQ_INFO_E3D_BWD_FORM: return m->last.bwd.e3b_form;
+        case ALQ_INFO_LDS_LAYOUT: return m->last.lds_layout;
         default: break;
     }
     set_error("alq_model_engine_info: bad argument");
diff --git a/nn-active-learning_amd/csrc/model_types.h b/nn-active-learning_amd/csrc/model_types.h
--- a/nn-active-learning_amd/csrc/model_types.h
+++ b/nn-active-learning_amd/csrc/model_types.h
@@ -89,6 +89,7 @@
         int e3b_form = 0;
         int d3b = 0;
     } bwd;
+    int lds_layout = 0;
     int lsum = 0;
     bool call_fisher = false;
 };
diff --git a/nn-active-learning_amd/csrc/sweep_common.h b/nn-active-learning_amd/csrc/sweep_common.h
--- a/nn-active-learning_amd/csrc/sweep_common.h
+++ b/nn-active-learning_amd/csrc/sweep_common.h
@@ -42,7 +42,10 @@
 
 inline unsigned sweep_grid(const alq_ctx *ctx, long long items, int per_cu) {
     const long long g = std::min<long long>((long long)per_cu * ctx->num_cus, items);
-    return (unsigned)std::max<long long>(8, (g + 7) / 8 * 8);
+    long long g8 = std::max<long long>(8, (g + 7) / 8 * 8);
+    const int cap = g_dbg_knobs[KNOB_SWEEP_GRID_CAP];
+    if (cap > 0) g8 = std::min<long long>(g8, std::max(8, cap / 8 * 8));
+    return (unsigned)g8;
 }
 
 inline bool is_conv3_same(const int k[3], const int lo[3], const int s[3]) {
diff --git a/nn-active-learning_amd/csrc/t3d8b.hip b/nn-active-learning_amd/csrc/t3d8b.hip
--- a/nn-active-learning_amd/csrc/t3d8b.hip
+++ b/nn-active-learning_amd/csrc/t3d8b.hip
@@ -1,4 +1,5 @@
 #include "f16_pair.h"
+#include "lds_layout.h"
 #include "sweep_common.h"
 
 #include <algorithm>
@@ -19,23 +20,17 @@
     int N;
 };
 
-constexpr int T8B_KG = 17 * 16;
-constexpr int T8B_PIECE = 2 * T8B_KG;
-constexpr int T8B_ROW = 2 * T8B_PIECE + 16;
-constexpr int T8B_PLANE = 18 * T8B_ROW + 32;
-constexpr int T8B_RING = 3 * T8B_PLANE;
-constexpr int T8B_XCH = 4 * 16 * 4;
-constexpr int T8B_LDS = T8B_RING + T8B_XCH;
-
-__device__ __host__ inline int t8b_row(int y) { return y * T8B_ROW + ((y >> 1) & 1) * 16; }
-
+static_assert(2 * lds::T8B<lds::OLD>::LDS <= 160 * 1024 && 2 * lds::T8B<lds::NEW>::LDS <= 160 * 1024, "t3d8_bwd: LDS layout");
+
+template <int FAM>
 __global__ __launch_bounds__(256, 2) void t3d8_bwd_kernel(const T8BwdArgs a) {
+    typedef lds::T8B<FAM> L;
     extern __shared__ __attribute__((aligned(16))) char t8lds[];
     const int lane = threadIdx.x & 63, wave = __builtin_amdgcn_readfirstlane((int)(threadIdx.x >> 6));
     const int cb = wave & 1, tp = wave >> 1;
     char *ring = t8lds;
-    float *xch = reinterpret_cast<float *>(t8lds + T8B_RING);
-    for (int i = threadIdx.x; i < T8B_LDS / 16; i += 256) reinterpret_cast<i32x4 *>(t8lds)[i] = i32x4{0, 0, 0, 0};
+    float *xch = reinterpret_cast<float *>(t8lds + L::RING);
+    for (int i = threadIdx.x; i < L::LDS / 16; i += 256) reinterpret_cast<i32x4 *>(t8lds)[i] = i32x4{0, 0, 0, 0};
     __syncthreads();
     const int n = lane & 15, kg = lane >> 4;
     f16x8 wh[15], wl[15];
@@ -52,17 +47,15 @@
     const __amdgpu_buffer_rsrc_t m_rsrc = sw_rsrc(a.mask_bits, a.mask_bits ? (unsigned long long)a.N * 512 * 8 : 0ull);
     const __amdgpu_buffer_rsrc_t u_rsrc = sw_rsrc(a.dsum, a.dsum ? (unsigned long long)a.N * 512 * 4 : 0ull);
 
-    const int sx = lane >> 2, cq = lane & 3;
-    const int w_off = (cq >> 1) * T8B_KG + sx * 16 + (cq & 1) * 8;
+    const int w_off = L::write(lane, 0, 0);
     const unsigned ldA = (unsigned)lane * 16u;
     int f01[2][3], f22[2][2];
 #pragma unroll
     for (int j = 0; j < 2; ++j) {
-        const int qy = 2 * (tp + 2 * j) + (n >> 3), qx = n & 7, h = kg >> 1;
-#pragma unroll
-        for (int ty = 0; ty < 3; ++ty) f01[j][ty] = t8b_row(2 * qy + ty) + (kg & 1) * T8B_KG + (2 * qx + h) * 16;
-        f22[j][0] = t8b_row(2 * qy + h) + (kg & 1) * T8B_KG + (2 * qx + 2) * 16;
-        f22[j][1] = t8b_row(2 * qy + 2 + h) + (kg & 1) * T8B_KG + (2 * qx + 2) * 16;
+#pragma unroll
+        for (int ty = 0; ty < 3; ++ty) f01[j][ty] = L::read(wave, lane, j, ty, 0);
+        f22[j][0] = L::read(wave, lane, j, 3, 0);
+        f22[j][1] = L::read(wave, lane, j, 4, 0);
     }
     const unsigned e_out = (unsigned)(cb * 64 + kg * 16), e_msk = (unsigned)(cb * 4 + kg);
 
@@ -85,13 +78,13 @@
             const int pz = pa + (k >> 4), y = k & 15;
             const bool rv = on && pz < 16;
             const float sc = rv ? a.scale : 0.f, sc11 = rv ? a.scale11 : 0.f;
-            char *dst = ring + (pz % 3) * T8B_PLANE + t8b_row(y) + w_off;
+            char *dst = ring + (pz % 3) * L::PLANE + L::row(y) + w_off;
             const f32x4 g = RA[j];
             const f16x2 h01 = __builtin_convertvector(f32x2{g.x * sc, g.y * sc}, f16x2), h23 = __builtin_convertvector(f32x2{g.z * sc, g.w * sc}, f16x2);
             const f16x2 l01 = __builtin_convertvector(f32x2{__builtin_fmaf((float)h01.x, -2048.f, g.x * sc11), __builtin_fmaf((float)h01.y, -2048.f, g.y * sc11)}, f16x2);
             const f16x2 l23 = __builtin_convertvector(f32x2{__builtin_fmaf((float)h23.x, -2048.f, g.z * sc11), __builtin_fmaf((float)h23.y, -2048.f, g.w * sc11)}, f16x2);
             *reinterpret_cast<i32x2 *>(dst) = i32x2{__builtin_bit_cast(int, h01), __builtin_bit_cast(int, h23)};
-            *reinterpret_cast<i32x2 *>(dst + T8B_PIECE) = i32x2{__builtin_bit_cast(int, l01), __builtin_bit_cast(int, l23)};
+            *reinterpret_cast<i32x2 *>(dst + L::PIECE) = i32x2{__builtin_bit_cast(int, l01), __builtin_bit_cast(int, l23)};
         }
     };
 
@@ -107,14 +100,14 @@
                 R0[j] = __builtin_bit_cast(f32x4, __builtin_amdgcn_raw_buffer_load_b128(i_rsrc, (int)ldA, sw_s((((unsigned)p * 16u) * 16u + (unsigned)(4 * wave + j)) * 1024u), 0));
 #pragma unroll
             for (int j = 0; j < 4; ++j) {
-                char *dst = ring + t8b_row(4 * wave + j) + w_off;
+                char *dst = ring + L::row(4 * wave + j) + w_off;
                 const f32x4 gq = R0[j];
                 const float sc = a.scale, sc11 = a.scale11;
                 const f16x2 h01 = __builtin_convertvector(f32x2{gq.x * sc, gq.y * sc}, f16x2), h23 = __builtin_convertvector(f32x2{gq.z * sc, gq.w * sc}, f16x2);
                 const f16x2 l01 = __builtin_convertvector(f32x2{__builtin_fmaf((float)h01.x, -2048.f, gq.x * sc11), __builtin_fmaf((float)h01.y, -2048.f, gq.y * sc11)}, f16x2);
                 const f16x2 l23 = __builtin_convertvector(f32x2{__builtin_fmaf((float)h23.x, -2048.f, gq.z * sc11), __builtin_fmaf((float)h23.y, -2048.f, gq.w * sc11)}, f16x2);
                 *reinterpret_cast<i32x2 *>(dst) = i32x2{__builtin_bit_cast(int, h01), __builtin_bit_cast(int, h23)};
-                *reinterpret_cast<i32x2 *>(dst + T8B_PIECE) = i32x2{__builtin_bit_cast(int, l01), __builtin_bit_cast(int, l23)};
+                *reinterpret_cast<i32x2 *>(dst + L::PIECE) = i32x2{__builtin_bit_cast(int, l01), __builtin_bit_cast(int, l23)};
             }
         }
         stage(2 * zq + 1, true);
@@ -131,14 +124,14 @@
         for (int j = 0; j < 2; ++j) { c[j] = f32x4{0.f, 0.f, 0.f, 0.f}; cx[j] = f32x4{0.f, 0.f, 0.f, 0.f}; }
 #pragma unroll
         for (int tz = 0; tz < 3; ++tz) {
-            const char *pl = ring + ((2 * zq + tz) % 3) * T8B_PLANE;
+            const char *pl = ring + ((2 * zq + tz) % 3) * L::PLANE;
 #pragma unroll
             for (int j = 0; j < 2; ++j)
 #pragma unroll
                 for (int pi = 0; pi < 5; ++pi) {
                     const char *src = pl + (pi < 3 ? f01[j][pi] : f22[j][pi - 3]);
                     const f16x8 xh = *reinterpret_cast<const f16x8 *>(src);
-                    const f16x8 xl = *reinterpret_cast<const f16x8 *>(src + T8B_PIECE);
+                    const f16x8 xl = *reinterpret_cast<const f16x8 *>(src + L::PIECE);
                     cx[j] = __builtin_amdgcn_mfma_f32_16x16x32_f16(wl[tz * 5 + pi], xh, cx[j], 0, 0, 0);
                     c[j] = __builtin_amdgcn_mfma_f32_16x16x32_f16(wh[tz * 5 + pi], xh, c[j], 0, 0, 0);
                     cx[j] = __builtin_amdgcn_mfma_f32_16x16x32_f16(wh[tz * 5 + pi], xl, cx[j], 0, 0, 0);
@@ -203,7 +196,8 @@
     a.dout = dout.p; a.din = din.p; a.W = reinterpret_cast<const unsigned short *>(plan.d_W); a.mask_bits = mask_bits; a.dsum = dsum;
     a.scale = std::ldexp(1.f, e_in); a.scale11 = std::ldexp(1.f, e_in + 11); a.inv = std::ldexp(1.f, -(e_in + plan.w_exp)); a.N = N;
     ProfScope ps(ctx, PROF_IGEMM_F16, plan.flops_per_patch * N);
-    return sweep_launch(ctx, t3d8_bwd_kernel, sweep_grid(ctx, N, 2), 256, T8B_LDS, a);
-}
-
-}
+    if (lds::pick(g_lds_layout, lds::T8B_DEFAULT) == lds::OLD) return sweep_launch(ctx, t3d8_bwd_kernel<lds::OLD>, sweep_grid(ctx, N, 2), 256, lds::T8B<lds::OLD>::LDS, a);
+    return sweep_launch(ctx, t3d8_bwd_kernel<lds::NEW>, sweep_grid(ctx, N, 2), 256, lds::T8B<lds::NEW>::LDS, a);
+}
+
+}
```

After: 285,900. Within noise of the previous version (-0.4%).
